# the-professor510/RSMCRT

Hardware: AMD Instinct MI355X
Metric: photon packets/sec (128^3 jmean grid, path-length deposition) (higher is better)
Workload: dtype f64

## Files before the change

include/smcrt.h:

```cpp
#ifndef SMCRT_H
#define SMCRT_H

#include <stddef.h>
#include <stdint.h>

#ifdef __cplusplus
extern "C" {
#endif

#define SMCRT_ABI_VERSION 5

typedef enum smcrt_status {
  SMCRT_OK = 0,
  SMCRT_ERR_INVALID_ARG = -1,
  SMCRT_ERR_HIP = -2,
  SMCRT_ERR_RCCL = -3,
  SMCRT_ERR_DEVICE_FAULT = -4,
  SMCRT_ERR_NO_DEVICE = -5,
  SMCRT_ERR_OOM = -6,
  SMCRT_ERR_UNSUPPORTED = -7
} smcrt_status;

typedef enum smcrt_sdf_kind {
  SMCRT_SDF_SPHERE = 1,
// ... 236 lines not shown
  const double* mua;
  const double* hgg;
  const double* n;
  const double* flux;
} smcrt_spectral;

typedef enum smcrt_spectral_mode {
  SMCRT_SPECTRAL_INIT = 0,
  SMCRT_SPECTRAL_UPDATE = 1,
  SMCRT_SPECTRAL_INIT_AS_WRITTEN = 2
} smcrt_spectral_mode;

typedef struct smcrt_optprops {
  double mus, mua, hgg, g2, n, kappa, albedo;
  double wavelength;
  int32_t node_flags;
  int32_t reserved;
} smcrt_optprops;

int smcrt_spectral_sample(const smcrt_spectral* sp, int32_t mode, uint64_t seed, uint64_t* draw,
                          smcrt_optprops* out);

int smcrt_scene_set_spectral(smcrt_scene* scene, int32_t top_index, const smcrt_spectral* sp, int32_t mode,
                             uint64_t seed, uint64_t* draw, smcrt_optprops* out);

int smcrt_run(smcrt_scene* scene, const smcrt_source* src, const smcrt_run_config* cfg,
              smcrt_tallies* io);

typedef struct smcrt_path_config {
  uint64_t range_first, range_count;
  int32_t max_vertices;
  int32_t reserved;
  int64_t max_paths;
} smcrt_path_config;

typedef struct smcrt_path {
  uint64_t photon;
  int32_t detector;
  uint32_t hit;
  uint32_t n_vertices;
  uint32_t n_stored;
  uint32_t status;
  int32_t layer;
  int64_t offset;
  double start[3], dir[3], point_sep, weight;
} smcrt_path;

int smcrt_scene_set_path_tracking(smcrt_scene* scene, const smcrt_path_config* cfg);
int smcrt_scene_path_counts(smcrt_scene* scene, int64_t* n_paths, int64_t* n_vertices, int64_t* n_dropped,
                            int64_t* n_truncated);
int smcrt_scene_read_paths(smcrt_scene* scene, smcrt_path* paths, double* vertices );

#define SMCRT_PPATH_MAX_MEDIA 16

typedef struct smcrt_ppath_config {
  uint64_t range_first, range_count;
  int64_t max_records;
  int64_t reserved;
} smcrt_ppath_config;

typedef struct smcrt_ppath {
  uint64_t photon;
  int32_t detector;
  uint32_t hit;
  uint32_t status;
  int32_t layer;
  uint32_t nscatt;
  int32_t reserved;
  double start[3], dir[3], point_sep, weight;
} smcrt_ppath;

int smcrt_scene_set_partial_paths(smcrt_scene* scene, const smcrt_ppath_config* cfg);
int smcrt_scene_partial_path_counts(smcrt_scene* scene, int64_t* n_records, int64_t* n_dropped);
int smcrt_scene_read_partial_paths(smcrt_scene* scene, smcrt_ppath* headers, double* lengths);

typedef struct smcrt_phasor_config {
  int32_t fixed_k;
  int32_t reserved;
  double wavenumber;
} smcrt_phasor_config;
#define SMCRT_PHASOR_OPTICAL_PATH 1

int smcrt_scene_set_phasor(smcrt_scene* scene, const smcrt_phasor_config* cfg);
int smcrt_scene_read_phasor(smcrt_scene* scene, double* out);
int smcrt_scene_reset_phasor(smcrt_scene* scene);

typedef struct smcrt_screen {
  double origin[3];
  double eu[3], ev[3];
  int32_t nu, nv;
  int32_t sides;
  int32_t reserved;
} smcrt_screen;

int smcrt_scene_set_screens(smcrt_scene* scene, const smcrt_screen* screens, int32_t n);
int smcrt_scene_screen_info(const smcrt_scene* scene, int32_t* n, int64_t* n_doubles);
int smcrt_scene_read_screens(smcrt_scene* scene, double* out);
int smcrt_scene_reset_screens(smcrt_scene* scene);
int smcrt_screen_hit(const smcrt_screen* screen, const double start[3], const double dir[3], double sep,
                     double* t, int32_t* pixel);


int smcrt_scene_set_volume_source(smcrt_scene* scene, const double* weights);
int smcrt_scene_volume_source_info(const smcrt_scene* scene, int64_t* n_positive, int64_t* n_reachable, double* total);
int smcrt_volume_sample(const double* weights, const smcrt_grid* g, uint64_t seed, uint64_t first, int64_t n,
                        double* pos, double* dir, int64_t* voxel);
int smcrt_volume_pick(const double* weights, int64_t nvox, const double* u, int64_t m, int64_t* voxel);

typedef struct smcrt_device_tallies {
  double* jmean;
  double* absorb;
  double* emission;
  double* det_bins;
  double* nscatt;
  double* moments;
  uint64_t* counters;
  smcrt_photon_record* records;
} smcrt_device_tallies;

int smcrt_run_device(smcrt_scene* scene, const smcrt_source* src, const smcrt_run_config* cfg,
                     smcrt_device_tallies* dev, void* stream);

int smcrt_run_origins(smcrt_scene* scene, const smcrt_source* src, const double* origins, int64_t n_origins,
                      const smcrt_run_config* cfg, double* det_totals, smcrt_tallies* io);

int smcrt_scene_classify(smcrt_scene* scene, const double* points, int64_t n, int32_t* layer, double* kappa);

int smcrt_scene_fence(smcrt_scene* scene, void* stream);

int smcrt_scene_check(smcrt_scene* scene);

typedef struct smcrt_kernel_times {
  double transport_ms;
  double deposit_ms;
  int64_t launches;
  int64_t lean_launches;
  int64_t far_steps;
  double fold_cu_ms;
  int64_t lean_hazards;
} smcrt_kernel_times;

int smcrt_scene_set_timing(smcrt_scene* scene, int32_t enable);
int smcrt_scene_kernel_times(smcrt_scene* scene, smcrt_kernel_times* out);

enum {
  SMCRT_DEPOSIT_ATOMIC = 0,
  SMCRT_DEPOSIT_SORTED = 1,
  SMCRT_DEPOSIT_BUCKETS = 2
};
int smcrt_scene_deposit_regime(const smcrt_scene* scene, int32_t* regime);

int smcrt_scene_invoxel_segments(smcrt_scene* scene, int64_t* out);

int smcrt_normalise_fluence(float* grid, const smcrt_grid* g, uint64_t nphotons);

typedef enum smcrt_symmetry {
  SMCRT_SYM_NONE = 0,
  SMCRT_SYM_PRISM = 1,
  SMCRT_SYM_FLIPPED = 2,
  SMCRT_SYM_UNIFORM_SLAB = 3,
  SMCRT_SYM_NONE_ROTATIONAL = 4,
  SMCRT_SYM_ROTATIONAL_360 = 5
} smcrt_symmetry;

typedef struct smcrt_escape_config {
  int32_t symmetry;
  int32_t n[3];
  double max[3];
  double pos[3];
  double dir[3];
  double rotation;
} smcrt_escape_config;

int smcrt_escape_sym_dims(const smcrt_escape_config* cfg, int32_t dims[3]);

int smcrt_escape_cells(const smcrt_escape_config* cfg, int64_t* n_cells, int32_t* cells, double* positions);

int smcrt_escape_map(const smcrt_escape_config* cfg, const smcrt_grid* grid, int32_t n_dets, const float* escape_sym,
                     float* escape);

int smcrt_escape_run(smcrt_scene* scene, const smcrt_source* src, const smcrt_escape_config* cfg,
                     const smcrt_run_config* run, float* escape_sym, float* escape, smcrt_tallies* io);

enum {
  SMCRT_INVERSE_FIND_MUS = 1u << 0,
  SMCRT_INVERSE_FIND_MUA = 1u << 1,
  SMCRT_INVERSE_FIND_G = 1u << 2,
  SMCRT_INVERSE_FIND_N = 1u << 3,
  SMCRT_INVERSE_APPLY_TRIAL = 1u << 4
};

typedef struct smcrt_inverse_config {
  int32_t layer;
  int32_t flags;
  int32_t max_steps;
  int32_t reserved;
  double max_step_size, grad_step_size, accuracy;
  uint64_t seed;
} smcrt_inverse_config;

int smcrt_scene_get_optprops(const smcrt_scene* scene, int32_t top_index, int32_t* layer, double* mus, double* mua,
                             double* hgg, double* n);

int smcrt_inverse_run(smcrt_scene* scene, const smcrt_source* src, const smcrt_inverse_config* cfg,
                      const smcrt_run_config* run, const double* targets, double* steps, smcrt_tallies* io);

enum {
  SMCRT_PACK_JMEAN = 1u << 0,
  SMCRT_PACK_ABSORB = 1u << 1,
  SMCRT_PACK_EMISSION = 1u << 2,
  SMCRT_PACK_DET_BINS = 1u << 3
};
typedef struct smcrt_pack_layout {
  int64_t n_voxels;
  int64_t n_det_bins;
  uint32_t fields;
  int32_t reserved;
} smcrt_pack_layout;

int smcrt_pack_size(const smcrt_pack_layout* layout, int64_t* n_doubles);
int smcrt_pack_host(const smcrt_pack_layout* layout, const smcrt_tallies* t, double* buf);
int smcrt_unpack_host(const smcrt_pack_layout* layout, const double* buf, smcrt_tallies* t);

#define SMCRT_UNIQUE_ID_BYTES 128
typedef struct smcrt_comm smcrt_comm;
int smcrt_comm_unique_id(uint8_t* id );
int smcrt_comm_init_rank(const uint8_t* id, int32_t n_ranks, int32_t rank, int32_t device, smcrt_comm** out);
void smcrt_comm_destroy(smcrt_comm* comm);
int smcrt_comm_info(const smcrt_comm* comm, int32_t* n_ranks, int32_t* rank, int32_t* device);
int smcrt_reduce_device_tallies(smcrt_scene* scene, smcrt_comm* comm, smcrt_device_tallies* dev, int32_t root,
                                void* stream);

typedef struct smcrt_multi smcrt_multi;
int smcrt_multi_create(const smcrt_sdf_node* nodes, int32_t n_nodes, const int32_t* top, int32_t n_top,
                       const smcrt_grid* grid, const smcrt_detector* dets, int32_t n_dets,
                       const int32_t* devices, int32_t n_devices, smcrt_multi** out);
int smcrt_multi_info(const smcrt_multi* multi, int32_t* n_devices);
smcrt_scene* smcrt_multi_scene(smcrt_multi* multi, int32_t i);
int smcrt_multi_run(smcrt_multi* multi, const smcrt_source* src, const smcrt_run_config* cfg, smcrt_tallies* io);
int smcrt_multi_accumulate(smcrt_multi* multi, const smcrt_source* src, const smcrt_run_config* cfg);
int smcrt_multi_collect(smcrt_multi* multi, smcrt_tallies* io);
int smcrt_multi_device_photons(const smcrt_multi* multi, uint64_t* photons);
void smcrt_multi_destroy(smcrt_multi* multi);


int smcrt_write_data_f32(const char* filename, const float* array, int32_t nx, int32_t ny, int32_t nz,
                         const char* metadata, const char* dect_id, int32_t overwrite,
                         char* written_path, int32_t path_cap);
int smcrt_write_data_f64(const char* filename, const double* array, int32_t nx, int32_t ny, int32_t nz,
                         const char* metadata, const char* dect_id, int32_t overwrite,
                         char* written_path, int32_t path_cap);

int smcrt_write_detector(const char* filename, const smcrt_detector* d, const double* data,
                         const char* id, int64_t nphotons);

int smcrt_write_paths(const char* filename, const smcrt_path* paths, int64_t n_paths, const double* vertices);

int smcrt_write_checkpoint(const char* filename, const char* toml_filename, int64_t photons_run,
                           const float* jmean, const smcrt_grid* g, int32_t overwrite,
                           char* written_path, int32_t path_cap);

typedef struct smcrt_job smcrt_job;

typedef struct smcrt_job_desc {
  int64_t n_photons;
  int64_t seed;
  int32_t flags;
  int32_t n_nodes, n_top, n_dets;
  int32_t overwrite;
  smcrt_grid grid;
  smcrt_source source;
  char experiment[64];
  char source_name[32];
} smcrt_job_desc;

int smcrt_job_load(const char* toml_path, smcrt_job** out);
enum { SMCRT_JOB_DEFAULT = 0, SMCRT_JOB_ESCAPE = 1, SMCRT_JOB_INVERSE = 2 };
int smcrt_job_load_mode(const char* toml_path, int32_t mode, smcrt_job** out);
void smcrt_job_destroy(smcrt_job* job);
int smcrt_job_info(const smcrt_job* job, smcrt_job_desc* desc);
int smcrt_job_scene(const smcrt_job* job, smcrt_sdf_node* nodes, int32_t* top, smcrt_detector* dets);
int smcrt_job_metadata(const smcrt_job* job, char* buf, int32_t cap);
int smcrt_job_history_filename(const smcrt_job* job, char* buf, int32_t cap);
#define SMCRT_ALL_DEVICES (-1)
int smcrt_job_run(smcrt_job* job, int32_t device, const char* outdir, double* nscatt);
int smcrt_job_run_devices(smcrt_job* job, const int32_t* devices, int32_t n_devices, const char* outdir,
                          double* nscatt);

int smcrt_job_escape_config(const smcrt_job* job, smcrt_escape_config* out);
int smcrt_job_inverse_config(const smcrt_job* job, smcrt_inverse_config* out);
int smcrt_job_targets(const smcrt_job* job, double* targets);
int smcrt_job_run_escape(smcrt_job* job, int32_t device, const char* outdir);
int smcrt_job_run_inverse(smcrt_job* job, int32_t device, int32_t apply_trial, double* steps);

#ifdef __cplusplus
}
#endif
#endif
```

rsmcrt_amd/abi.py:

```python
import ctypes as C

SMCRT_ABI_VERSION = 5

OK = 0
ERR_INVALID_ARG = -1
ERR_HIP = -2
ERR_RCCL = -3
ERR_DEVICE_FAULT = -4
ERR_NO_DEVICE = -5
ERR_OOM = -6
ERR_UNSUPPORTED = -7

STATUS_NAMES = {
    OK: "OK", ERR_INVALID_ARG: "INVALID_ARG", ERR_HIP: "HIP_ERROR", ERR_RCCL: "RCCL_ERROR",
    ERR_DEVICE_FAULT: "DEVICE_FAULT", ERR_NO_DEVICE: "NO_DEVICE", ERR_OOM: "OUT_OF_MEMORY",
    ERR_UNSUPPORTED: "UNSUPPORTED",
}

SDF_SPHERE, SDF_BOX, SDF_TORUS, SDF_CYLINDER, SDF_TRIPRISM = 1, 2, 3, 4, 5
SDF_SEGMENT, SDF_CAPSULE, SDF_CONE, SDF_EGG, SDF_PLANE, SDF_MODEL = 6, 7, 8, 9, 10, 11
SDF_REVOLUTION, SDF_EXTRUDE, SDF_ONION, SDF_TWIST, SDF_BEND, SDF_ELONGATE, SDF_DISPLACEMENT = 12, 13, 14, 15, 16, 17, 18
DISP_SINE, DISP_EXPR = 1, 2

OP_UNION, OP_SMOOTH_UNION, OP_SUBTRACTION, OP_INTERSECTION = 0, 1, 2, 3
# ... 99 lines not shown


class Detector(C.Structure):
    _fields_ = [
        ("kind", C.c_int32), ("nbins", C.c_int32), ("layer", C.c_int32), ("reserved", C.c_int32),
        ("pos", C.c_double * 3), ("dir", C.c_double * 3), ("e1", C.c_double * 3), ("e2", C.c_double * 3),
        ("radius", C.c_double), ("r1", C.c_double), ("r2", C.c_double),
        ("width", C.c_double), ("height", C.c_double),
        ("bin_wid", C.c_double), ("bin_wid_y", C.c_double), ("fibre", C.c_double * 11),
    ]


class RunConfig(C.Structure):
    _fields_ = [("n_photons", C.c_uint64), ("first_photon", C.c_uint64), ("seed", C.c_uint64),
                ("flags", C.c_uint32), ("reserved", C.c_int32)]


class PhotonRecord(C.Structure):
    _fields_ = [("pos", C.c_double * 3), ("dir", C.c_double * 3), ("weight", C.c_double),
                ("cell", C.c_int32 * 3), ("layer", C.c_int32), ("nscatt", C.c_uint32),
                ("bounces", C.c_uint32), ("draws", C.c_uint32), ("status", C.c_uint32)]


class Tallies(C.Structure):
    _fields_ = [
        ("jmean", C.POINTER(C.c_float)), ("absorb", C.POINTER(C.c_float)),
        ("emission", C.POINTER(C.c_float)),
        ("jmean_f64", C.POINTER(C.c_double)), ("absorb_f64", C.POINTER(C.c_double)),
        ("emission_f64", C.POINTER(C.c_double)),
        ("det_bins", C.POINTER(C.c_double)), ("nscatt", C.POINTER(C.c_double)),
        ("moments", C.POINTER(C.c_double)), ("counters", C.POINTER(C.c_uint64)),
        ("records", C.POINTER(PhotonRecord)),
    ]


class DeviceTallies(C.Structure):
    _fields_ = [
        ("jmean", C.c_void_p), ("absorb", C.c_void_p), ("emission", C.c_void_p),
        ("det_bins", C.c_void_p), ("nscatt", C.c_void_p), ("moments", C.c_void_p),
        ("counters", C.c_void_p), ("records", C.c_void_p),
    ]


class PathConfig(C.Structure):
    _fields_ = [("range_first", C.c_uint64), ("range_count", C.c_uint64), ("max_vertices", C.c_int32),
                ("reserved", C.c_int32), ("max_paths", C.c_int64)]


class Path(C.Structure):
    _fields_ = [("photon", C.c_uint64), ("detector", C.c_int32), ("hit", C.c_uint32), ("n_vertices", C.c_uint32),
                ("n_stored", C.c_uint32), ("status", C.c_uint32), ("layer", C.c_int32), ("offset", C.c_int64),
                ("start", C.c_double * 3), ("dir", C.c_double * 3), ("point_sep", C.c_double), ("weight", C.c_double)]


class PPathConfig(C.Structure):
    _fields_ = [("range_first", C.c_uint64), ("range_count", C.c_uint64), ("max_records", C.c_int64),
                ("reserved", C.c_int64)]


class PPath(C.Structure):
    _fields_ = [("photon", C.c_uint64), ("detector", C.c_int32), ("hit", C.c_uint32), ("status", C.c_uint32),
                ("layer", C.c_int32), ("nscatt", C.c_uint32), ("reserved", C.c_int32),
                ("start", C.c_double * 3), ("dir", C.c_double * 3), ("point_sep", C.c_double), ("weight", C.c_double)]


class PhasorConfig(C.Structure):
    _fields_ = [("fixed_k", C.c_int32), ("reserved", C.c_int32), ("wavenumber", C.c_double)]


class Screen(C.Structure):
    _fields_ = [("origin", C.c_double * 3), ("eu", C.c_double * 3), ("ev", C.c_double * 3),
                ("nu", C.c_int32), ("nv", C.c_int32), ("sides", C.c_int32), ("reserved", C.c_int32)]


def path_dtype():
    import numpy as np
    return np.dtype([("photon", "<u8"), ("detector", "<i4"), ("hit", "<u4"), ("n_vertices", "<u4"),
                     ("n_stored", "<u4"), ("status", "<u4"), ("layer", "<i4"), ("offset", "<i8"),
                     ("start", "<f8", 3), ("dir", "<f8", 3), ("point_sep", "<f8"), ("weight", "<f8")])


def ppath_dtype():
    import numpy as np
    return np.dtype([("photon", "<u8"), ("detector", "<i4"), ("hit", "<u4"), ("status", "<u4"), ("layer", "<i4"),
                     ("nscatt", "<u4"), ("reserved", "<i4"), ("start", "<f8", 3), ("dir", "<f8", 3),
                     ("point_sep", "<f8"), ("weight", "<f8")])


def record_dtype():
    import numpy as np
    return np.dtype([("pos", "<f8", 3), ("dir", "<f8", 3), ("weight", "<f8"), ("cell", "<i4", 3),
                     ("layer", "<i4"), ("nscatt", "<u4"), ("bounces", "<u4"), ("draws", "<u4"),
                     ("status", "<u4")])


SYM_NONE, SYM_PRISM, SYM_FLIPPED, SYM_UNIFORM_SLAB, SYM_NONE_ROTATIONAL, SYM_ROTATIONAL_360 = 0, 1, 2, 3, 4, 5
SYMMETRY_KINDS = {"none": SYM_NONE, "prism": SYM_PRISM, "flipped": SYM_FLIPPED, "uniformSlab": SYM_UNIFORM_SLAB,
                  "noneRotational": SYM_NONE_ROTATIONAL, "360rotational": SYM_ROTATIONAL_360}


class EscapeConfig(C.Structure):
    _fields_ = [("symmetry", C.c_int32), ("n", C.c_int32 * 3), ("max", C.c_double * 3), ("pos", C.c_double * 3),
                ("dir", C.c_double * 3), ("rotation", C.c_double)]


INVERSE_FIND_MUS, INVERSE_FIND_MUA, INVERSE_FIND_G, INVERSE_FIND_N, INVERSE_APPLY_TRIAL = 1, 2, 4, 8, 16


class InverseConfig(C.Structure):
    _fields_ = [("layer", C.c_int32), ("flags", C.c_int32), ("max_steps", C.c_int32), ("reserved", C.c_int32),
                ("max_step_size", C.c_double), ("grad_step_size", C.c_double), ("accuracy", C.c_double),
                ("seed", C.c_uint64)]


JOB_DEFAULT, JOB_ESCAPE, JOB_INVERSE = 0, 1, 2


class JobDesc(C.Structure):
    _fields_ = [("n_photons", C.c_int64), ("seed", C.c_int64), ("flags", C.c_int32), ("n_nodes", C.c_int32),
                ("n_top", C.c_int32), ("n_dets", C.c_int32), ("overwrite", C.c_int32), ("grid", Grid),
                ("source", Source), ("experiment", C.c_char * 64), ("source_name", C.c_char * 32)]


PACK_JMEAN, PACK_ABSORB, PACK_EMISSION, PACK_DET_BINS = 1, 2, 4, 8
UNIQUE_ID_BYTES = 128
ALL_DEVICES = -1


class PackLayout(C.Structure):
    _fields_ = [("n_voxels", C.c_int64), ("n_det_bins", C.c_int64), ("fields", C.c_uint32), ("reserved", C.c_int32)]


class KernelTimes(C.Structure):
    _fields_ = [("transport_ms", C.c_double), ("deposit_ms", C.c_double), ("launches", C.c_int64),
                ("lean_launches", C.c_int64), ("far_steps", C.c_int64), ("fold_cu_ms", C.c_double),
                ("lean_hazards", C.c_int64)]


EXPORTED_SYMBOLS = [
    "smcrt_abi_version", "smcrt_device_count", "smcrt_last_error", "smcrt_scene_create",
    "smcrt_scene_destroy", "smcrt_scene_det_bins", "smcrt_scene_set_optprops", "smcrt_run",
    "smcrt_run_device", "smcrt_normalise_fluence", "smcrt_scene_set_timing", "smcrt_scene_kernel_times",
    "smcrt_write_data_f32", "smcrt_write_data_f64", "smcrt_write_detector", "smcrt_write_checkpoint",
    "smcrt_job_load", "smcrt_job_destroy", "smcrt_job_info", "smcrt_job_scene", "smcrt_job_metadata", "smcrt_job_run",
    "smcrt_scene_info", "smcrt_run_origins", "smcrt_scene_classify", "smcrt_escape_sym_dims", "smcrt_escape_cells",
    "smcrt_escape_map", "smcrt_escape_run", "smcrt_scene_get_optprops", "smcrt_inverse_run", "smcrt_job_load_mode",
    "smcrt_job_escape_config", "smcrt_job_inverse_config", "smcrt_job_targets", "smcrt_job_run_escape",
    "smcrt_job_run_inverse", "smcrt_scene_fence",
    "smcrt_pack_size", "smcrt_pack_host", "smcrt_unpack_host", "smcrt_comm_unique_id", "smcrt_comm_init_rank",
    "smcrt_comm_info", "smcrt_comm_destroy", "smcrt_reduce_device_tallies", "smcrt_multi_create", "smcrt_multi_info",
    "smcrt_multi_scene", "smcrt_multi_run", "smcrt_multi_accumulate", "smcrt_multi_collect",
    "smcrt_multi_device_photons", "smcrt_multi_destroy", "smcrt_job_run_devices",
    "smcrt_spectral_sample", "smcrt_scene_set_spectral", "smcrt_scene_check",
    "smcrt_scene_invoxel_segments",
    "smcrt_scene_set_path_tracking", "smcrt_scene_path_counts", "smcrt_scene_read_paths", "smcrt_write_paths",
    "smcrt_job_history_filename",
    "smcrt_scene_set_phasor", "smcrt_scene_read_phasor", "smcrt_scene_reset_phasor",
    "smcrt_scene_set_screens", "smcrt_scene_screen_info", "smcrt_scene_read_screens", "smcrt_scene_reset_screens",
    "smcrt_screen_hit",
    "smcrt_scene_set_volume_source", "smcrt_scene_volume_source_info", "smcrt_volume_sample", "smcrt_volume_pick",
    "smcrt_displacement_compile", "smcrt_displacement_eval", "smcrt_displacement_describe",
    "smcrt_voxel_scene_create", "smcrt_scene_deposit_regime",
    "smcrt_mesh_scene_create",
    "smcrt_scene_set_partial_paths", "smcrt_scene_partial_path_counts", "smcrt_scene_read_partial_paths",
]
```

rsmcrt_amd/csrc/sceneplan.cpp:

```cpp
#include "sceneplan.h"

#include <algorithm>
#include <cmath>
#include <cstdlib>
#include <cstring>
#include <functional>
#include <string>

#include "dispexpr.h"
#include "hosterr.h"

namespace smcrt {
namespace {

int fail(int code, const std::string& msg) { return set_error(code, msg); }
bool is(const char* v, const char* s) { return v && std::strcmp(v, s) == 0; }

}

Knobs read_knobs() {
  Knobs k;
  auto num = [](const char* v, double d) { return v ? std::atof(v) : d; };
  if (const char* cm = std::getenv("SMCRT_COOP_MIN_TOPS")) k.coop_min_tops = std::max(1, std::atoi(cm));
  if (const char* cl = std::getenv("SMCRT_COOP_LANES")) k.coop_lanes = std::max(1, std::min(64, std::atoi(cl)));
  k.coop_tab = !is(std::getenv("SMCRT_COOP_TAB"), "0");
  k.cull = !is(std::getenv("SMCRT_CULL"), "0");
  k.cull_grid.cells_per_top = num(std::getenv("SMCRT_CULL_CPT"), 512.0);
  k.cull_grid.max_cells = num(std::getenv("SMCRT_CULL_MAX_CELLS"), 1 << 18);
  k.cull_grid.max_list = (int32_t)num(std::getenv("SMCRT_CULL_MAX_LIST"), 64);
  k.cull_grid.k_nearest = (int32_t)num(std::getenv("SMCRT_CULL_K"), 8);
  k.cull_grid.u_frac = num(std::getenv("SMCRT_CULL_UFRAC"), 1.0);
  k.cull_log = std::getenv("SMCRT_CULL_LOG") != nullptr;
  k.far_march = !is(std::getenv("SMCRT_FAR_MARCH"), "0");
  const char* dm = std::getenv("SMCRT_DEPOSIT");
  k.deposit_atomic = is(dm, "atomic");
  k.deposit_sorted = is(dm, "sorted");
  if (const char* pc = std::getenv("SMCRT_POOL_CAP"))
    k.pool_cap_chunks = std::max<uint64_t>(1, std::strtoull(pc, nullptr, 10) / CHUNK_RECORDS);
  const char* fp = std::getenv("SMCRT_FOLD_PRIO");
  k.fold_prio = !(fp && fp[0] == '0');
  k.fused_hist = !is(std::getenv("SMCRT_FUSED_HIST"), "0");
  const char* wsl = std::getenv("SMCRT_WS_SLOTS");
  k.ws_two_slots = wsl && wsl[0] == '2';
  const char* wi = std::getenv("SMCRT_WS_INVOXEL");
  k.ws_invoxel = wi ? (is(wi, "0") ? 0 : 1) : -1;
  const char* le = std::getenv("SMCRT_LEAN");
  k.lean_mode = le ? (is(le, "0") ? 0 : 1) : -1;
  const char* lm = std::getenv("SMCRT_DEBUG_LEAN_MARGIN");
  k.lean_debug = is(lm, "all") ? 2u : (is(lm, "0") ? 1u : 0u);
  k.verbose = std::getenv("SMCRT_VERBOSE") != nullptr;
  return k;
}

LaunchKnobs read_launch_knobs() {
  LaunchKnobs k;
#ifdef SMCRT_DIAG
  const char* dd = std::getenv("SMCRT_DIAG_DONE");
  k.diag_done = dd && dd[0] == '1';
#endif
  if (const char* wm = std::getenv("SMCRT_WATCHDOG_MS")) k.watchdog_ms = std::strtod(wm, nullptr);
  if (const char* cd = std::getenv("SMCRT_DEBUG_CLAIM_DELAY")) k.claim_delay = (uint32_t)std::strtoul(cd, nullptr, 10);
  const char* de = std::getenv("SMCRT_DEBUG_DROP_EVENT");
  k.drop_event = de && de[0] == '1';
  if (const char* pv = std::getenv("SMCRT_PATH_VERTICES")) k.path_vertices = (int32_t)std::strtol(pv, nullptr, 10);
  if (const char* pm = std::getenv("SMCRT_PATH_MAX")) k.path_max = (int64_t)std::strtoll(pm, nullptr, 10);
  return k;
}

void job_path_knobs(int32_t* max_vertices, int64_t* max_paths) {
  const LaunchKnobs k = read_launch_knobs();
  *max_vertices = k.path_vertices;
  *max_paths = k.path_max;
}

PoolKnobs read_pool_knobs() {
  PoolKnobs k;
  if (const char* ns = std::getenv("SMCRT_SLOTS")) k.slots = std::max(2, std::min(MAX_SLOTS, std::atoi(ns)));
  if (const char* dg = std::getenv("SMCRT_DEEP_SLOT_GIB")) {
    k.deep_set = true;
    k.deep_bytes = (uint64_t)std::strtoull(dg, nullptr, 10) << 30;
  }
  return k;
}

bool pool_log_knob() {
  static const bool on = std::getenv("SMCRT_POOL_LOG") != nullptr;
  return on;
}

TopProps make_props(const smcrt_sdf_node& nd) {
  TopProps p;
  p.kappa = nd.mus + nd.mua;
  if (nd.flags & SMCRT_NODE_ALBEDO_UNGUARDED) p.albedo = nd.mus / p.kappa;
  else p.albedo = (nd.mua < 1e-9) ? 1.0 : nd.mus / p.kappa;
  p.hgg = nd.hgg;
  p.n = nd.n;
  return p;
}

namespace {

int validate(const smcrt_sdf_node* nodes, int32_t n_nodes, const int32_t* top, int32_t n_top, const smcrt_grid* grid,
             const smcrt_detector* dets, int32_t n_dets) {
  if (!nodes || n_nodes < 1 || !top || n_top < 1 || !grid || n_dets < 0 || (n_dets > 0 && !dets))
    return fail(SMCRT_ERR_INVALID_ARG, "bad scene arguments");
  if (grid->nx < 1 || grid->ny < 1 || grid->nz < 1 || !(grid->xmax > 0) || !(grid->ymax > 0) ||
      !(grid->zmax > 0))
    return fail(SMCRT_ERR_INVALID_ARG, "grid dimensions must be positive");
  if ((uint64_t)grid->nx * (uint64_t)grid->ny * (uint64_t)grid->nz >= (1ull << 32))
    return fail(SMCRT_ERR_UNSUPPORTED, "grids of 2^32 or more voxels are not supported");
  for (int32_t i = 0; i < n_nodes; ++i) {
    const smcrt_sdf_node& nd = nodes[i];
    if (nd.kind < SMCRT_SDF_SPHERE || nd.kind > SMCRT_SDF_DISPLACEMENT)
      return fail(SMCRT_ERR_INVALID_ARG, "node " + std::to_string(i) + ": unknown SDF kind");
    if (nd.kind == SMCRT_SDF_MODEL) {
      if (nd.n_children < 1 || nd.first_child < 0 || nd.first_child + nd.n_children > n_nodes)
        return fail(SMCRT_ERR_INVALID_ARG, "model node " + std::to_string(i) + ": bad child range");
      if (nd.op < SMCRT_OP_UNION || nd.op > SMCRT_OP_INTERSECTION)
        return fail(SMCRT_ERR_INVALID_ARG, "model node " + std::to_string(i) + ": bad CSG op");
    } else if (composite_kind(nd.kind)) {
      if (nd.n_children != 1 || nd.first_child < 0 || nd.first_child >= n_nodes)
        return fail(SMCRT_ERR_INVALID_ARG, "modifier node " + std::to_string(i) + ": needs exactly one child");
      if (nd.kind == SMCRT_SDF_DISPLACEMENT && nd.param[0] == (double)SMCRT_DISP_EXPR) {
        std::string why;
        if (!disp_expr_verify(nd, &why))
          return fail(SMCRT_ERR_INVALID_ARG, "displacement node " + std::to_string(i) + ": bad expression program: " + why);
      } else if (nd.kind == SMCRT_SDF_DISPLACEMENT && nd.param[0] != (double)SMCRT_DISP_SINE) {
        return fail(SMCRT_ERR_INVALID_ARG, "displacement node " + std::to_string(i) + ": unknown function");
      }
    }
  }
  std::function<int(int32_t, int)> depth_ok = [&](int32_t idx, int lvl) -> int {
    const smcrt_sdf_node& nd = nodes[idx];
    if (!composite_kind(nd.kind)) return 1;
    if (lvl >= PROG_MAX_DEPTH) return 0;
    for (int32_t c = 0; c < nd.n_children; ++c)
      if (!depth_ok(nd.first_child + c, lvl + 1)) return 0;
    return 1;
  };
  for (int32_t i = 0; i < n_top; ++i)
    if (top[i] >= 0 && top[i] < n_nodes && !depth_ok(top[i], 0))
      return fail(SMCRT_ERR_UNSUPPORTED, "top " + std::to_string(i) + ": models/modifiers nested more than " +
                                             std::to_string(PROG_MAX_DEPTH) + " levels deep are not supported");
  for (int32_t i = 0; i < n_top; ++i)
    if (top[i] < 0 || top[i] >= n_nodes) return fail(SMCRT_ERR_INVALID_ARG, "top index out of range");
  for (int32_t i = 0; i < n_dets; ++i) {
    if (dets[i].kind < SMCRT_DET_CIRCLE || dets[i].kind > SMCRT_DET_FIBRE || dets[i].nbins < 1)
      return fail(SMCRT_ERR_INVALID_ARG, "bad detector " + std::to_string(i));
  }
  return SMCRT_OK;
}

bool translate_only(const smcrt_sdf_node& nd) {
  const double* t = nd.transform;
  return t[0] == 1.0 && t[1] == 0.0 && t[2] == 0.0 && t[4] == 0.0 && t[5] == 1.0 && t[6] == 0.0 &&
         t[8] == 0.0 && t[9] == 0.0 && t[10] == 1.0;
}

void flatten(const smcrt_sdf_node* nodes, const int32_t* top, int32_t n_top, ScenePlan& p) {
  std::vector<ProgOp>& prog = p.prog;
  p.top_first.assign((size_t)n_top + 1, 0);
  for (int32_t i = 0; i < n_top; ++i) {
    const smcrt_sdf_node& nd = nodes[top[i]];
    p.top_first[i] = (int32_t)prog.size();
    if (!composite_kind(nd.kind)) {
      prog.push_back(ProgOp{top[i], PROG_TOP, i + 1, 0, 0.0, translate_only(nd), 0});
    } else if (nd.kind != SMCRT_SDF_MODEL) {
      prog.push_back(ProgOp{top[i], PROG_TOP | PROG_SUB, i + 1, 0, 0.0, 0, 0});
    } else {
      for (int32_t c = 0; c < nd.n_children; ++c) {
        const int32_t ci = nd.first_child + c;
        const bool sub = composite_kind(nodes[ci].kind);
        prog.push_back(ProgOp{ci, (c == 0 ? PROG_CHILD_FIRST : PROG_CHILD) | (sub ? PROG_SUB : 0),
                              c == nd.n_children - 1 ? i + 1 : 0, nd.op, nd.k, sub ? 0 : translate_only(nodes[ci]), 0});
      }
    }
  }
  p.n_prog = (int)prog.size();
  p.top_first[n_top] = p.n_prog;
  for (int32_t i = 0; i <= n_top; ++i)
    prog.push_back(ProgOp{p.top_first[i], PROG_TOP, 0, 0, 0.0, 0, 0});
  for (const ProgOp& op : prog) p.nested = p.nested || (op.action & PROG_SUB) != 0;
}

void plan_far_march(const smcrt_sdf_node* nodes, const int32_t* top, int32_t n_top, const smcrt_grid* grid, bool fm,
                    ScenePlan& p) {
  double ext = grid->xmax + grid->ymax + grid->zmax + 1.0;
  double scale = 0.0;
  std::function<bool(int32_t, int, double&)> far_ok = [&](int32_t idx, int lvl, double& m) -> bool {
    const smcrt_sdf_node& nd = nodes[idx];
    if (nd.kind == SMCRT_SDF_MODEL) {
      const bool op_ok = nd.op == SMCRT_OP_UNION || nd.op == SMCRT_OP_INTERSECTION || nd.op == SMCRT_OP_SUBTRACTION ||
                         (nd.op == SMCRT_OP_SMOOTH_UNION && nd.k > 0.0 && std::isfinite(nd.k));
      if (lvl >= 4 || !op_ok || nd.n_children < 1) return false;
      if (nd.op == SMCRT_OP_SMOOTH_UNION) m = std::max(m, nd.k);
      for (int32_t c = 0; c < nd.n_children; ++c)
        if (!far_ok(nd.first_child + c, lvl + 1, m)) return false;
      return true;
    }
    const int32_t kd = nd.kind;
    if (!translate_only(nd) || !(kd == SMCRT_SDF_SPHERE || kd == SMCRT_SDF_BOX || kd == SMCRT_SDF_TORUS ||
                                 kd == SMCRT_SDF_SEGMENT || kd == SMCRT_SDF_CAPSULE))
      return false;
    double mm = std::fabs(nd.transform[3]) + std::fabs(nd.transform[7]) + std::fabs(nd.transform[11]);
    for (int r = 0; r < 8; ++r) mm += std::fabs(nd.param[r]);
    if (!std::isfinite(mm)) return false;
    m = std::max(m, mm);
    return true;
  };
  for (int32_t i = 0; fm && i < n_top; ++i) {
    double m = 0.0;
    fm = far_ok(top[i], 0, m);
    scale = std::max(scale, m);
  }
  fm = fm && std::isfinite(ext);
  if (fm) {
// ... 447 lines not shown
```

rsmcrt_amd/csrc/sceneplan.h:

```cpp
#pragma once
#include <stdint.h>

#include <algorithm>
#include <vector>

#include "../../include/smcrt.h"
#include "transport.h"
#include "cull.h"
#include "deposit.h"
#include "launchchoice.h"

namespace smcrt {

constexpr int MAX_SLOTS = 4;
#ifndef SMCRT_DEEP_SLOT_GIB
#define SMCRT_DEEP_SLOT_GIB 24
#endif
constexpr uint64_t DEEP_SLOT_BYTES = (uint64_t)SMCRT_DEEP_SLOT_GIB << 30;

enum QueueWord : int {
  Q_STREAM0 = 0,
  Q_CALLER = MAX_SLOTS,
  Q_FAR_STEPS,
  Q_FOLD_TICKS,
  Q_LEAN_HAZARDS,
  Q_WATCHDOG,
  Q_INVOXEL,
  Q_COUNT
};
constexpr int N_QUEUES = Q_CALLER + 1;

constexpr size_t LDS_BYTES = 163840;
constexpr size_t MAX_FACE_BYTES = 40960;
constexpr uint32_t MAX_FUSED_HIST_TILES = 512;
constexpr uint64_t MAX_POOL_RECORDS = (1ull << 32) - (1ull << 28);
constexpr double POOL_SLACK = 1.15;
constexpr double DEFAULT_WATCHDOG_MS = 2000.0;

struct Knobs {
  int32_t coop_min_tops = 8;
  int32_t coop_lanes = 0;
  bool coop_tab = true;
  bool cull = true;
  CullKnobs cull_grid;
  bool cull_log = false;
  bool far_march = true;
  bool deposit_atomic = false, deposit_sorted = false;
  uint64_t pool_cap_chunks = 0;
  bool fold_prio = true;
  bool fused_hist = true;
  bool ws_two_slots = false;
  int ws_invoxel = -1;
  int lean_mode = -1;
  uint32_t lean_debug = 0;
  bool verbose = false;
};
struct LaunchKnobs {
  int32_t path_vertices = 64;
  int64_t path_max = 65536;
  double watchdog_ms = DEFAULT_WATCHDOG_MS;
  uint32_t claim_delay = 0;
  bool drop_event = false;
  bool diag_done = false;
};
struct PoolKnobs {
  int slots = 0;
  bool deep_set = false;
  uint64_t deep_bytes = 0;
};
Knobs read_knobs();
LaunchKnobs read_launch_knobs();
PoolKnobs read_pool_knobs();
bool pool_log_knob();

struct PlanLimits {
  size_t ws_shared2 = 0, ws_shared3 = 0;
};

struct ScenePlan {
  int n_nodes = 0, n_top = 0, n_dets = 0;
  smcrt_grid grid{};
  int64_t det_total = 0;
  std::vector<smcrt_sdf_node> h_nodes;
  std::vector<int32_t> h_top;
  std::vector<TopProps> h_props;
  std::vector<smcrt_detector> h_dets;
  std::vector<int64_t> h_det_off;
  std::vector<double> faces;
  std::vector<ProgOp> prog;
  std::vector<int32_t> top_first;
  int n_prog = 0;
  bool nested = false;
  int coop_lanes = 0;
  std::vector<double> ctab;
  CullHost cull;
  double fm_err = 0.0, fm_step = 0.0;
  double inv2[3] = {0.0, 0.0, 0.0};
  int grid_mode = 0;
  int32_t fe[3] = {0, 0, 0};
  uint32_t n_tiles = 0;
  bool force_atomic = false;
  uint64_t pool_cap_chunks = 0;
  bool bucketed = false;
  uint32_t hist_tiles = 0;
  size_t face_bytes = 0;
  bool lds_faces = false;
  bool fresnel = false;
  int ws_slots = 3;
  int lean_mode = -1;
  uint32_t lean_debug = 0;
  int ws_invoxel = -1;
  bool lean_candidate = false;
  bool fold_prio = true, cull_log = false, verbose = false;
  bool voxel = false;
  std::vector<uint8_t> labels;
  bool mesh = false;
  int32_t mesh_ambient = 0;
  std::vector<MeshNode> mesh_nodes;
  std::vector<MeshTri> mesh_tris;
  std::vector<MeshFace> mesh_faces;
};

int plan_scene(const smcrt_sdf_node* nodes, int32_t n_nodes, const int32_t* top, int32_t n_top, const smcrt_grid* grid,
               const smcrt_detector* dets, int32_t n_dets, const Knobs& knobs, const PlanLimits& lim, ScenePlan* out);

TopProps make_props(const smcrt_sdf_node& nd);

int plan_voxel_scene(const uint8_t* labels, const smcrt_medium* media, int32_t n_media, const smcrt_grid* grid,
                     const smcrt_detector* dets, int32_t n_dets, const Knobs& knobs, ScenePlan* out);
int32_t host_vox_of(double p, int32_t n, double max);

int plan_mesh_scene(const double* verts, int32_t nv, const int32_t* tris, const uint8_t* tri_media, int32_t nt,
                    const smcrt_medium* media, int32_t n_media, int32_t ambient, const smcrt_grid* grid,
                    const smcrt_detector* dets, int32_t n_dets, const Knobs& knobs, ScenePlan* out);
int32_t mesh_medium_at(const ScenePlan& p, const double pt[3]);

int plan_screens(const smcrt_screen* screens, int32_t n, std::vector<ScreenDev>* out, int64_t* n_doubles);

int plan_volume_source(const double* w, int64_t nvox, std::vector<double>* cdf, int64_t* last, int64_t* n_positive,
                       int64_t* n_reachable);

std::vector<double> grid_faces(const smcrt_grid* grid);

inline size_t lean_lds(const ScenePlan& p) {
  return (p.lds_faces ? p.face_bytes : 0) + (size_t)2 * p.n_tiles * sizeof(uint32_t);
}
inline uint32_t dep_words(const ScenePlan& p) { return p.bucketed ? 2 * p.n_tiles : 4 * p.hist_tiles; }
inline size_t transport_lds(const ScenePlan& p, uint32_t dep_words, bool xsrc, bool hist = false, bool screens = false) {
  const bool ctab = !p.ctab.empty() && p.coop_lanes > 0;
  const bool faces = p.lds_faces && !(xsrc && p.coop_lanes > 0) && !hist;
  const size_t start_rows = screens ? 4 : p.n_dets ? 3 : 0;
  return (faces ? p.face_bytes : 0) + start_rows * 256 * sizeof(double) +
         (size_t)dep_words * sizeof(uint32_t) + (ctab ? CTAB_DOUBLES * sizeof(double) : 0);
}
inline double pool_slack_records(const ScenePlan& p, int blocks) {
  const double waves = (double)blocks * 4.0;
  return p.bucketed ? (waves / 4.0 * 2.0 * p.n_tiles + waves * BUCKET_BATCH) * BUCKET_RECORDS
                    : waves * CHUNK_RECORDS;
}
inline uint64_t pool_records_for(const ScenePlan& p, int blocks, uint64_t n, double rpp) {
  const double want = (double)n * rpp * POOL_SLACK + pool_slack_records(p, blocks);
  return (uint64_t)std::min(want, (double)MAX_POOL_RECORDS);
}
inline int slot_depth(const PoolKnobs& k, bool lean_or_far, uint64_t cap_bytes, uint64_t total_mem) {
  const int want = k.slots ? k.slots : (lean_or_far ? 2 : MAX_SLOTS);
  uint64_t deep = std::max<uint64_t>(DEEP_SLOT_BYTES, (uint64_t)(0.6 * (double)total_mem) / MAX_SLOTS);
  if (k.deep_set) deep = k.deep_bytes;
  return cap_bytes <= deep ? want : 2;
}
inline bool launch_binned(const ScenePlan& p, bool has_jmean, uint32_t flags) {
  return has_jmean && (flags & SMCRT_FLAG_PATHLENGTH) && !(flags & SMCRT_FLAG_SURVIVAL_BIAS) && p.n_tiles > 0 &&
         !p.force_atomic;
}
inline bool launch_lean(bool lean_ok, bool xsrc, uint32_t bucket_tiles, uint32_t flags) {
  return !xsrc && lean_ok && bucket_tiles && (flags & SMCRT_FLAG_PATHLENGTH) &&
         !(flags & (SMCRT_FLAG_SURVIVAL_BIAS | SMCRT_FLAG_TRACK_PATHS | SMCRT_FLAG_PHASOR));
}
inline bool ws_invoxel_on(int knob, bool xf) { return knob < 0 ? !xf : knob != 0; }
inline bool plan_xf(const ScenePlan& p) { return p.fresnel || p.n_dets > 0; }

constexpr int32_t PPL_MAX_MEDIA = SMCRT_PPATH_MAX_MEDIA;
inline size_t ppl_lds_bytes(const ScenePlan& p) { return (size_t)p.n_top * 256 * sizeof(double); }
constexpr size_t SDFLESS_STATIC_LDS = sizeof(LaneCounters);

inline LaunchChoice launch_choice(const ScenePlan& p, bool lean_ok, bool xsrc, uint32_t bucket_tiles, uint32_t flags,
                                  bool path_on, bool phasor_on, size_t n_screens, size_t ppl_lds = 0) {
  LaunchChoice c;
  c.gm = p.grid_mode;
  if (p.voxel || p.mesh) {
    c.family = p.mesh ? KF_MESH : KF_VOXEL;
    c.xsrc = xsrc;
    c.lds = p.face_bytes + (size_t)dep_words(p) * sizeof(uint32_t);
    c.ppl = (flags & SMCRT_FLAG_PARTIAL_PATHS) && ppl_lds > 0;
    if (c.ppl) c.lds += ppl_lds;
  } else if (launch_lean(lean_ok, xsrc, bucket_tiles, flags)) {
    c.family = KF_WS;
    c.lds_faces = p.lds_faces;
    c.xf = plan_xf(p);
    c.slots = p.ws_slots;
    c.iv = ws_invoxel_on(p.ws_invoxel, c.xf);
    c.tk = (flags & SMCRT_FLAG_TEST_KERNEL) != 0;
    c.lds = lean_lds(p);
  } else {
    c.xsrc = xsrc;
    c.coop = p.coop_lanes > 0;
    c.hist = (flags & SMCRT_FLAG_TRACK_PATHS) && path_on;
    c.phas = (flags & SMCRT_FLAG_PHASOR) && phasor_on && !c.hist;
    c.scr = c.phas && n_screens > 0;
    c.lds_faces = p.lds_faces && !((xsrc && c.coop) || c.hist || c.phas);
    c.lds = transport_lds(p, dep_words(p), xsrc, c.hist || c.phas, c.scr);
  }
  return c;
}
inline void lean_margins(uint32_t lean_debug, const smcrt_grid& g, double lo[3], double hi[3]) {
  const double eps = 1e-8, mf = (lean_debug & 3u) ? 0.0 : 2.0 * eps;
// ... 7 lines not shown
```

rsmcrt_amd/csrc/smcrt.hip:

```cpp
#include <hip/hip_runtime.h>

#include <algorithm>
#include <cmath>
#include <cstdio>
#include <cstring>
#include <memory>
#include <mutex>
#include <string>
#include <vector>

#define SMCRT_FOLD_KERNELS
#include "../../include/smcrt.h"
#include "scene_internal.h"
#include "transport.h"
#include "deposit.h"
#include "devmem.h"
#include "hosterr.h"
#include "hostrng.h"
#include "sceneplan.h"

using namespace smcrt;

#include "kernel_ptrs.h"

// ... 525 lines not shown
  uint64_t chunks = (records + CHUNK_RECORDS - 1) / CHUNK_RECORDS;
  if (s->pool_cap_chunks) chunks = std::min(chunks, s->pool_cap_chunks);
  if (chunks <= s->pool_chunks) return true;
  chunks = std::min<uint64_t>(chunks + chunks / 4, MAX_POOL_RECORDS / CHUNK_RECORDS);
  if (s->pool_cap_chunks) chunks = std::min(chunks, s->pool_cap_chunks);
  (void)hipDeviceSynchronize();
  (void)drain_folds(s);
  auto release = [&]() {
    s->d_sorted.reset(); s->d_pieces.reset(); s->d_order.reset();
    for (int i = 0; i < MAX_SLOTS; ++i) { s->d_pool[i].reset(); s->d_chunk_fill[i].reset(); s->d_bucket_tile[i].reset(); }
    s->pool_chunks = 0;
  };
  release();
  const uint64_t cap = chunks * CHUNK_RECORDS;
  size_t mfree = 0, mtotal = 0;
  if (hipMemGetInfo(&mfree, &mtotal) != hipSuccess) mtotal = 0;
  s->n_slots = slot_depth(read_pool_knobs(), s->lean_ok || s->fm_err > 0.0, cap * 8, mtotal);
  s->slot = 0;
  s->lturn = 0;
  s->last_slot = -1;
  const uint64_t pieces = std::min<uint64_t>(cap / MIN_PIECE_RECORDS, REDUCE_PIECES + 1) + s->n_tiles + 1;
  const uint64_t buckets = cap / BUCKET_RECORDS;
  bool ok = s->d_pieces.alloc(pieces) == hipSuccess;
  for (int i = 0; ok && i < s->n_slots; ++i) {
    ok = s->d_pool[i].alloc(cap) == hipSuccess;
    if (ok && s->bucketed)
      ok = s->d_chunk_fill[i].alloc(buckets) == hipSuccess && s->d_bucket_tile[i].alloc(buckets) == hipSuccess;
    else if (ok)
      ok = s->d_chunk_fill[i].alloc(chunks) == hipSuccess;
  }
  if (ok && s->bucketed)
    ok = s->d_order.alloc(buckets) == hipSuccess;
  else if (ok)
    ok = s->d_sorted.alloc(cap) == hipSuccess;
  if (!ok) {
    (void)hipGetLastError();
    release();
    return false;
  }
  s->pool_chunks = chunks;
  s->max_pieces = pieces;
  return true;
}


static int next_timing_events(smcrt_scene* s, Event** ev) {
  *ev = nullptr;
  if (!s->timing) return SMCRT_OK;
  if (s->tev_used == MAX_TIMED) HIPCHK(harvest_times(s));
  while (4 * (s->tev_used + 1) > s->tev.size()) {
    Event e;
    HIPCHK(hipEventCreate(e.out()));
    s->tev.push_back(std::move(e));
  }
  *ev = &s->tev[4 * s->tev_used++];
  return SMCRT_OK;
}

static int enqueue_transport(smcrt_scene* s, const KParams& K, KCold Ch, const LaunchChoice& c, hipStream_t stream,
                             int sl, int qi, Event** ev_out) {
  const bool binned = K.rec_pool != nullptr;
  if (binned && s->f_pending[sl]) HIPCHK(hipStreamWaitEvent(stream, s->ev_f[sl], 0));
  Ch.queue = s->d_queue + qi;
  Ch.lane_scratch = s->d_lscratch ? (double*)(s->d_lscratch + (size_t)qi * s->lscratch_stride) : nullptr;
  HIPCHK(hipMemsetAsync(Ch.queue, 0, sizeof(unsigned long long), stream));
  const KCold* C = s->d_cold + (size_t)qi * COLD_PER_STREAM + (s->cold_seq[qi]++ % COLD_PER_STREAM);
  HIPCHK(hipMemcpyAsync((void*)C, &Ch, sizeof(KCold), hipMemcpyHostToDevice, stream));
  if (binned) {
    HIPCHK(hipMemsetAsync(s->d_dep_ctl[sl], 0, 8 * sizeof(uint32_t), stream));
    if (K.bucket_tiles)
      HIPCHK(hipMemsetAsync(s->d_bin_counts[sl], 0, (size_t)s->n_tiles * sizeof(uint32_t), stream));
    else if (K.hist_tiles)
      HIPCHK(hipMemsetAsync(s->d_bin_counts[sl], 0, (size_t)s->n_tiles * BIN_BLOCKS * sizeof(uint32_t), stream));
  }
  if (const int st = next_timing_events(s, ev_out)) return st;
  Event* ev = *ev_out;
  if (ev) HIPCHK(hipEventRecord(ev[0], stream));
  const bool ws = c.family == KF_WS;
  const uint64_t per_block = ws ? (uint64_t)kinst_ws_photon_lanes() : 256;
  const int blocks = (int)std::min<uint64_t>((uint64_t)blocks_for(s, c),
                                             std::max<uint64_t>(1, (Ch.n_photons + per_block - 1) / per_block));
  if (ws) ++s->lean_launches;
  const smcrt_sdf_node* a_nodes = K.nodes;
  const ProgOp* a_prog = K.prog;
  const smcrt_detector* a_dets = K.dets;
  const int64_t* a_off = K.det_off;
  void* args_ws[] = {(void*)&K, (void*)&a_nodes, (void*)&a_prog, (void*)&C};
  void* args[] = {(void*)&K, (void*)&a_nodes, (void*)&a_prog, (void*)&a_dets, (void*)&a_off, (void*)&C};
  HIPCHK(hipLaunchKernel(kernel_ptr(c), dim3(blocks), dim3(kernel_threads(c)), ws ? args_ws : args, c.lds, stream));
  HIPCHK(hipGetLastError());
  if (ev) HIPCHK(hipEventRecord(ev[1], stream));
  return SMCRT_OK;
}

static int enqueue_fold(smcrt_scene* s, const KParams& K, double* jmean, hipStream_t stream, int sl, Event* ev) {
  if (!K.rec_pool) {
    if (ev) {
      HIPCHK(hipEventRecord(ev[2], stream));
      HIPCHK(hipEventRecord(ev[3], stream));
    }
    return SMCRT_OK;
  }
  hipStream_t fs = s->fstream;
  HIPCHK(hipEventRecord(s->ev_t, stream));
  HIPCHK(hipStreamWaitEvent(fs, s->ev_t, 0));
  if (ev) HIPCHK(hipEventRecord(ev[2], fs));
  const uint32_t nch = (uint32_t)s->pool_chunks;
  const uint64_t nv = (uint64_t)s->grid.nx * s->grid.ny * s->grid.nz;
  if (K.bucket_tiles) {
    hipLaunchKernelGGL(bk_scan, dim3(1), dim3(1024), 0, fs, s->d_bin_counts[sl], s->n_tiles, s->d_tile_start,
                       s->d_tile_count, s->d_pieces, s->d_dep_ctl[sl]);
    hipLaunchKernelGGL(bk_place, dim3(BIN_BLOCKS), dim3(BIN_THREADS), 0, fs, s->d_bucket_tile[sl], s->d_chunk_fill[sl],
                       s->d_dep_ctl[sl], K.n_buckets, s->n_tiles, s->d_tile_count, s->d_order);
#ifndef SMCRT_ABL_NO_FOLD
    hipLaunchKernelGGL(bk_reduce, dim3(1024), dim3(RED_THREADS), 0, fs, s->d_pool[sl], s->d_order, s->d_pieces,
                       s->d_dep_ctl[sl], nv, jmean, s->d_queue + Q_FOLD_TICKS);
#endif
  } else {
    if (!K.hist_tiles)
      hipLaunchKernelGGL(bin_hist, dim3(BIN_BLOCKS), dim3(BIN_THREADS), 0, fs, s->d_pool[sl], s->d_chunk_fill[sl],
                         s->d_dep_ctl[sl], nch, s->n_tiles, s->d_bin_counts[sl]);
    hipLaunchKernelGGL(bin_rowscan, dim3(s->n_tiles), dim3(BIN_BLOCKS), 0, fs, s->d_bin_counts[sl],
                       s->d_tile_count);
    hipLaunchKernelGGL(bin_scan, dim3(1), dim3(1024), 0, fs, s->d_tile_count, s->n_tiles, s->d_tile_start,
                       s->d_pieces, s->d_dep_ctl[sl]);
    hipLaunchKernelGGL(bin_scatter, dim3(BIN_BLOCKS), dim3(BIN_THREADS), s->scatter_lds, fs, s->d_pool[sl],
                       s->d_chunk_fill[sl], s->d_dep_ctl[sl], nch, s->n_tiles, s->d_tile_start, s->d_bin_counts[sl],
                       s->d_sorted, (uint64_t)s->pool_chunks * CHUNK_RECORDS);
    hipLaunchKernelGGL(bin_reduce, dim3(1024), dim3(1024), 0, fs, s->d_sorted, s->d_pieces, s->d_dep_ctl[sl], nv,
                       jmean);
  }
  HIPCHK(hipGetLastError());
  HIPCHK(hipMemcpyAsync(s->h_ctl + 8 * sl, s->d_dep_ctl[sl], 4 * sizeof(uint32_t), hipMemcpyDeviceToHost, fs));
  HIPCHK(hipMemcpyAsync(s->h_ctl + 8 * sl + 5, s->d_dep_ctl[sl] + 5, 2 * sizeof(uint32_t), hipMemcpyDeviceToHost, fs));
  HIPCHK(hipEventRecord(s->ctl_ev[sl], fs));
  s->ctl_pending[sl] = true;
  if (ev) HIPCHK(hipEventRecord(ev[3], fs));
  HIPCHK(hipEventRecord(s->ev_f[sl], fs));
  s->f_pending[sl] = true;
  s->last_slot = sl;
  return SMCRT_OK;
}

#ifdef SMCRT_DIAG
static int diag_report(hipStream_t stream, bool lean) {
  unsigned long long h[72], ht[9], hc[6];
  HIPCHK(hipStreamSynchronize(stream));
  kinst_diag_gather(h, ht, hc);
  if (lean) {
    const double wi = (double)std::max(1ull, h[20]), pt = (double)std::max(1ull, h[24]);
    std::fprintf(stderr, "[diag-ws] walker iters %llu: idle %.3f, busy lanes/iter %.1f, pending lanes/iter %.1f | "
                 "photon trips %llu: sleep %.3f, idle lanes %.1f, sync-waiting %.2f, slot-blocked %.2f, EVAL lanes "
                 "%.1f, pushes %.2f, P7 runs %.3f (lanes/run %.1f), event-waiting %.2f | producer waits %llu | event "
                 "iters %llu, lanes/iter %.1f | emissions waiting for a slot %llu lane-trips\n",
                 h[20], h[21] / wi, h[22] / wi, h[23] / wi, h[24], h[25] / pt, h[30] / pt, h[27] / pt, h[26] / pt,
                 h[31] / pt, h[32] / pt, h[28] / pt, (double)h[29] / (double)std::max(1ull, h[28]), h[36] / pt, h[33],
                 h[34], (double)h[35] / (double)std::max(1ull, h[34]), h[51]);
    const char* np[8] = {"fetch", "poll", "eval", "p3p4", "handout", "p5p6", "p7", "p8"};
    double tp = 0, tw = 0, te = 0;
    for (int i = 0; i < 8; ++i) tp += (double)h[37 + i];
    for (int i = 0; i < 4; ++i) tw += (double)h[45 + i];
    te = (double)h[49] + (double)h[50];
    std::fprintf(stderr, "[diag-ws-time] photon:");
    for (int i = 0; i < 8; ++i) std::fprintf(stderr, " %s=%.3f", np[i], (double)h[37 + i] / std::max(1.0, tp));
    std::fprintf(stderr, " | walker: claim=%.3f idle=%.3f walk=%.3f finish=%.3f | event: run=%.3f idle=%.3f | "
                 "ticks photon/walker/event %.3g/%.3g/%.3g\n", h[45] / std::max(1.0, tw), h[46] / std::max(1.0, tw),
                 h[47] / std::max(1.0, tw), h[48] / std::max(1.0, tw), h[49] / std::max(1.0, te),
                 h[50] / std::max(1.0, te), tp, tw, te);
  }
  unsigned long long lt = 0;
  for (int i = 0; i < 64; ++i) lt += h[i];
  std::fprintf(stderr, "[diag] waves %llu, longest wave %llu trips %llu ticks\n", h[70], h[68], h[69]);
  std::fprintf(stderr, "[diag] trips %llu dda %llu eval %llu p7 %llu | lane-trips %llu:", h[64], h[65], h[66],
               h[67], lt);
  for (int i = 0; i < 64; ++i)
    if (h[i]) std::fprintf(stderr, " %s%d=%.3f", i >= 32 ? "seg:" : "", i & 31, (double)h[i] / (double)lt);
  std::fprintf(stderr, "\n");

  double tt = 0;
  for (int i = 1; i < 9; ++i) tt += (double)ht[i];
  const char* nm_t[9] = {"", "fetch", "eval", "p3", "p4", "dda", "p5p6", "p7", "p8"};
  const char* nm_l[9] = {"", "fetch", "eval", "p3p4", "push", "walk", "p5p6", "p7", "p8"};
  const char* const* nm = lean ? nm_l : nm_t;
  std::fprintf(stderr, "[diag-time]");
  for (int i = 1; i < 9; ++i) std::fprintf(stderr, " %s=%.3f", nm[i], (double)ht[i] / tt);
  std::fprintf(stderr, "\n");

  if (hc[0] + hc[2])
    std::fprintf(stderr, "[diag-cull] culled lane-EVALs %llu, bound fallbacks %llu (%.4f), capture/outside %llu, "
                 "mean list %.1f, wave-EVALs %llu with a full fallback %.3f\n", hc[0], hc[1],
                 (double)hc[1] / (double)std::max(1ull, hc[0]), hc[2], (double)hc[3] / (double)std::max(1ull, hc[0]),
                 hc[4], (double)hc[5] / (double)std::max(1ull, hc[4]));
  return SMCRT_OK;
}
#endif

static int launch_one(smcrt_scene* s, const KParams& K, const KCold& Ch, bool xsrc, hipStream_t stream, int sl, int qi) {
  const LaunchChoice c = launch_choice(*s, s->lean_ok, xsrc, K.bucket_tiles, K.flags, s->path_on, s->phasor_on, s->screens.size(),
                                       ppl_lds_of(s));
  Event* ev = nullptr;
  int st = enqueue_transport(s, K, Ch, c, stream, sl, qi, &ev);
  if (!st) st = enqueue_fold(s, K, Ch.jmean, stream, sl, ev);
#ifdef SMCRT_DIAG
  if (!st) st = diag_report(stream, c.family == KF_WS);
#endif
  return st;
}

struct OriginRun {
  const double* d_origins;
  double* d_totals;
  uint64_t per_origin, first;
};

static int fill_params(smcrt_scene* s, const smcrt_source* src, const smcrt_run_config* cfg,
                       const smcrt_device_tallies& dt, const SrcPlan& plan, hipStream_t stream, bool diag_done_ok,
                       const LaunchChoice& run, KParams& K, KCold& Ch) {
  const LaunchKnobs knobs = read_launch_knobs();
  K.nodes = s->d_nodes;
  K.prog = s->d_prog;
  K.n_prog = s->n_prog;
  K.coop_lanes = s->coop_lanes;
  K.cull = s->d_cull;
  K.ctab = s->d_ctab;
  const bool far = s->fm_err > 0.0 && (cfg->flags & SMCRT_FLAG_PATHLENGTH);
  K.fm_err = far ? s->fm_err : 0.0;
  K.fm_step = s->fm_step;
  K.inv2x = s->inv2[0]; K.inv2y = s->inv2[1]; K.inv2z = s->inv2[2];
  K.fex = s->fe[0]; K.fey = s->fe[1]; K.fez = s->fe[2];
  K.props = s->d_props;
  K.xface = s->d_faces;
  K.yface = s->d_faces + (s->grid.nx + 1);
  K.zface = s->d_faces + (s->grid.nx + 1) + (s->grid.ny + 1);
  K.dets = s->d_dets;
  K.det_off = s->d_det_off;
  K.n_top = s->n_top;
  K.n_dets = s->n_dets;
  K.nx = s->grid.nx; K.ny = s->grid.ny; K.nz = s->grid.nz;
  K.xmax = s->grid.xmax; K.ymax = s->grid.ymax; K.zmax = s->grid.zmax;
  K.flags = cfg->flags;
  Ch.src = *src;
  Ch.plan = plan;
  K.key0 = (uint32_t)cfg->seed;
  K.key1 = (uint32_t)(cfg->seed >> 32);
  Ch.jmean = dt.jmean; Ch.absorb = dt.absorb; Ch.emission = dt.emission;
  Ch.chunk_fill = nullptr; Ch.dep_ctl = nullptr; Ch.bin_counts = nullptr;
  Ch.bucket_tile = nullptr; Ch.bucket_fill = nullptr; Ch.tile_nb = nullptr;
  Ch.det_bins = dt.det_bins; Ch.nscatt = dt.nscatt; Ch.moments = dt.moments;
  Ch.counters = (unsigned long long*)dt.counters;
  Ch.queue = nullptr;
  Ch.far_steps = s->d_queue + Q_FAR_STEPS;
  Ch.lean_hazards = s->d_queue + Q_LEAN_HAZARDS;
  Ch.invoxel_segs = s->d_queue + Q_INVOXEL;
  Ch.lane_scratch = nullptr;
  Ch.watchdog = watchdog_word(s);
  const bool hist = run.hist, phas = run.phas, scr = run.scr;
  Ch.hist_scratch = hist ? (double*)s->d_hist_scratch : nullptr;
  Ch.path_vertices = hist ? (double*)s->d_path_vertices : nullptr;
  Ch.path_headers = hist ? (smcrt_path*)s->d_path_headers : nullptr;
  Ch.path_ctl = hist ? (unsigned long long*)s->d_path_ctl : nullptr;
  Ch.hist_lanes = hist ? s->hist_lanes : 0;
  Ch.path_max = hist ? (uint64_t)s->path_cfg.max_paths : 0;
  const bool ppl = run.ppl;
  Ch.range_first = hist ? s->path_cfg.range_first : ppl ? s->ppath_cfg.range_first : 0;
  Ch.range_count = hist ? s->path_cfg.range_count : ppl ? s->ppath_cfg.range_count : 0;
  Ch.ppl_lengths = ppl ? (double*)s->d_ppl_lengths : nullptr;
  Ch.ppl_headers = ppl ? (smcrt_ppath*)s->d_ppl_headers : nullptr;
  Ch.ppl_ctl = ppl ? (unsigned long long*)s->d_ppl_ctl : nullptr;
  Ch.ppl_max = ppl ? (uint64_t)s->ppath_cfg.max_records : 0;
  Ch.ppl_lds_off = ppl ? (uint32_t)((s->face_bytes + (size_t)dep_words(*s) * sizeof(uint32_t)) / sizeof(double)) : 0u;
  Ch.ppl_n_media = ppl ? (uint32_t)s->n_top : 0u;
  Ch.hist_max_vertices = hist ? (uint32_t)s->path_cfg.max_vertices : 0;
  Ch.phasor = phas ? (double*)s->d_phasor : nullptr;
  Ch.phasor_fixed = phas && s->phasor_cfg.fixed_k ? 1u : 0u;
  Ch.phasor_k = !phas ? 0.0
                : s->phasor_cfg.fixed_k ? s->phasor_cfg.wavenumber
                                        : 6.283185307179586 / (src->spectrum ? src->spectrum->wavelength : 500.0);
  Ch.screens = scr ? (const ScreenDev*)s->d_screens : nullptr;
  Ch.screen_field = scr ? (double*)s->d_screen_field : nullptr;
  Ch.n_screens = scr ? (uint32_t)s->screens.size() : 0u;
  Ch.phasor_optical = phas && (s->phasor_cfg.reserved & SMCRT_PHASOR_OPTICAL_PATH) ? 1u : 0u;
  const bool vsrc = src->kind == SMCRT_SRC_VOLUME && s->d_vs_cdf;
  Ch.vs_cdf = vsrc ? (const double*)s->d_vs_cdf : nullptr;
  Ch.vs_xface = vsrc ? K.xface : nullptr;
  Ch.vs_yface = vsrc ? K.yface : nullptr;
  Ch.vs_zface = vsrc ? K.zface : nullptr;
  Ch.vs_total = vsrc ? s->vs_total : 0.0;
  Ch.vs_nvox = vsrc ? (uint32_t)((int64_t)s->grid.nx * s->grid.ny * s->grid.nz) : 0u;
  Ch.vs_last = vsrc ? (uint32_t)s->vs_last : 0u;
  Ch.vox_labels = s->d_labels;
  Ch.vox_n_media = s->voxel ? (uint32_t)s->n_top : 0u;
  Ch.vox_reserved = 0;
  Ch.mesh_nodes = s->d_mesh_nodes;
  Ch.mesh_tris = s->d_mesh_tris;
  Ch.mesh_faces = s->d_mesh_faces;
  Ch.mesh_n_nodes = (uint32_t)s->mesh_nodes.size();
  Ch.mesh_ambient = (uint32_t)s->mesh_ambient;
#ifdef SMCRT_DIAG
  Ch.done_time = nullptr;
  Ch.done_base = cfg->first_photon;
  if (knobs.diag_done && diag_done_ok) {
    s->n_done = cfg->n_photons;
    HIPCHK(s->d_done.alloc(s->n_done));
    HIPCHK(hipMemsetAsync(s->d_done, 0, sizeof(unsigned long long) * s->n_done, stream));
    Ch.done_time = s->d_done;
  }
#else
  (void)stream; (void)diag_done_ok;
#endif
  Ch.watchdog_ticks = knobs.watchdog_ms > 0.0 ? (uint64_t)(knobs.watchdog_ms * (double)s->wall_khz) : 0ull;
  K.rec_pool = nullptr; K.n_chunks = 0; K.hist_tiles = 0; K.bucket_tiles = 0; K.n_buckets = 0;
  K.claim_delay = knobs.claim_delay;
  K.lean_debug = s->lean_debug | (knobs.drop_event ? 4u : 0u);
  K.ws_invoxel = ws_invoxel_on(s->ws_invoxel, plan_xf(*s)) ? 1u : 0u;
  lean_margins(K.lean_debug, s->grid, K.lean_lo, K.lean_hi);
  return SMCRT_OK;
}

static int launch(smcrt_scene* s, const smcrt_source* src, const smcrt_run_config* cfg,
                  const smcrt_device_tallies& dt, hipStream_t stream, const OriginRun* orun = nullptr) {
  if (src->kind < SMCRT_SRC_POINT || src->kind > SMCRT_SRC_VOLUME) return fail(SMCRT_ERR_INVALID_ARG, "bad source kind");
  if (src->kind == SMCRT_SRC_VOLUME) {
    if (orun) return fail(SMCRT_ERR_UNSUPPORTED, "smcrt_run_origins: a volume source has no origin to batch");
    if (!s->d_vs_cdf)
      return fail(SMCRT_ERR_INVALID_ARG, "a volume source needs smcrt_scene_set_volume_source first (the scene holds no table)");
  }
  if (const int pst = ppl_flag_scene_ok(s, cfg->flags)) return pst;
  if (cfg->n_photons == 0) return SMCRT_OK;
  const bool xsrc = src_needs_plan(src) || orun || s->nested;
  SrcPlan plan;
  std::memset(&plan, 0, sizeof plan);
  if (xsrc) {
    std::vector<double> px, py, pc;
    const char* perr = "";
    const int pst = build_src_plan(src, &s->grid, &plan, px, py, pc, &perr);
    if (pst) return fail(pst, perr);
    std::vector<double> tab;
    tab.reserve(px.size() + py.size() + pc.size());
    tab.insert(tab.end(), px.begin(), px.end());
    tab.insert(tab.end(), py.begin(), py.end());
    tab.insert(tab.end(), pc.begin(), pc.end());
    if (!tab.empty()) {
      if (tab != s->h_spec) {
        HIPCHK(hipStreamSynchronize(stream));
        if (s->stream != stream) HIPCHK(hipStreamSynchronize(s->stream));
        if (tab.size() > s->spec_cap) {
          s->spec_cap = 0;
          HIPCHK(s->d_spec.alloc(tab.size()));
          s->spec_cap = tab.size();
        }
        HIPCHK(hipMemcpy(s->d_spec, tab.data(), tab.size() * sizeof(double), hipMemcpyHostToDevice));
        s->h_spec = tab;
      }
      plan.spec_x = px.empty() ? nullptr : s->d_spec;
      plan.spec_y = py.empty() ? nullptr : s->d_spec + px.size();
      plan.cdf = s->d_spec + px.size() + py.size();
    }
    if (orun) {
      plan.origins = orun->d_origins;
      plan.det_totals = orun->d_totals;
      plan.per_origin = orun->per_origin;
      plan.first = orun->first;
    }
  }
  KParams K;
  KCold Ch;
  const LaunchChoice run = launch_choice(*s, false, xsrc, 0, cfg->flags, s->path_on, s->phasor_on, s->screens.size(),
                                         ppl_lds_of(s));
  if (const int st = fill_params(s, src, cfg, dt, plan, stream, !orun, run, K, Ch)) return st;
  const bool binned = launch_binned(*s, dt.jmean != nullptr, cfg->flags);
  const bool overlap = (cfg->flags & SMCRT_FLAG_OVERLAP) != 0;
  if (overlap) {
    HIPCHK(hipEventRecord(s->ev_in, stream));
    for (int i = 0; i < MAX_SLOTS; ++i) HIPCHK(hipStreamWaitEvent(s->lstream[i], s->ev_in, 0));
  } else {
    for (int i = 0; i < MAX_SLOTS; ++i)
      if (s->lpending[i]) HIPCHK(hipStreamWaitEvent(stream, s->lev[i], 0));
  }
  for (int i = 0; i < MAX_SLOTS; ++i)
    if (s->lpending[i] && hipEventQuery(s->lev[i]) == hipSuccess) s->lpending[i] = false;
  for (uint64_t done = 0; done < cfg->n_photons;) {
    refine_rpp(s);
    uint64_t n = cfg->n_photons - done;
    K.rec_pool = nullptr; K.n_chunks = 0; K.hist_tiles = 0; K.bucket_tiles = 0; K.n_buckets = 0;
    bool calibrate = false;
    if (binned) {
      if (!s->rpp_measured && n > CALIB_PHOTONS) { n = CALIB_PHOTONS; calibrate = true; }
      const uint64_t want = pool_records_for(*s, transport_blocks(s), n, s->rpp_est);
      if (!ensure_pool(s, want)) (void)ensure_pool(s, want / 4);
      if (s->pool_chunks) {
        const double usable = (double)(s->pool_chunks * CHUNK_RECORDS) - pool_slack_records(*s, transport_blocks(s));
        n = std::min<uint64_t>(n, (uint64_t)std::max(65536.0, usable / (s->rpp_est * POOL_SLACK)));
        K.rec_pool = s->d_pool[s->slot];
        Ch.chunk_fill = s->d_chunk_fill[s->slot];
        Ch.dep_ctl = s->d_dep_ctl[s->slot];
        Ch.bin_counts = s->d_bin_counts[s->slot];
        K.n_chunks = (uint32_t)s->pool_chunks;
        K.hist_tiles = s->hist_tiles;
        if (s->bucketed) {
          Ch.bucket_fill = s->d_chunk_fill[s->slot];
          Ch.bucket_tile = s->d_bucket_tile[s->slot];
          Ch.tile_nb = s->d_bin_counts[s->slot];
          K.bucket_tiles = s->n_tiles;
          K.n_buckets = (uint32_t)(s->pool_chunks * (CHUNK_RECORDS / BUCKET_RECORDS));
        }
      }
    }
    Ch.n_photons = n;
    Ch.first_photon = orun ? done : cfg->first_photon + done;
    Ch.records = dt.records ? dt.records + done : nullptr;
    const int sl = s->slot;
    if (K.rec_pool) {
      if (s->ctl_pending[sl]) { HIPCHK(hipEventSynchronize(s->ctl_ev[sl])); refine_rpp(s); }
      s->h_ctl[8 * sl + 4] = (uint32_t)std::min<uint64_t>(n, 0xFFFFFFFFull);
    }
    int st;
    if (overlap) {
      const int q = s->lturn;
      s->lturn = (s->lturn + 1) % s->n_slots;
      st = launch_one(s, K, Ch, xsrc, s->lstream[q], sl, q);
      if (!st && hipEventRecord(s->lev[q], s->lstream[q]) != hipSuccess) st = fail(SMCRT_ERR_HIP, "event record failed");
      s->lpending[q] = true;
    } else {
      st = launch_one(s, K, Ch, xsrc, stream, sl, Q_CALLER);
    }
    if (st) return st;
    if (K.rec_pool) s->slot = (s->slot + 1) % s->n_slots;
    if (calibrate && K.rec_pool) {
      HIPCHK(hipEventSynchronize(s->ctl_ev[sl]));
      refine_rpp(s);
    }
    done += n;
  }
  if (!(cfg->flags & (SMCRT_FLAG_ASYNC_FOLD | SMCRT_FLAG_OVERLAP)) && s->last_slot >= 0 && s->f_pending[s->last_slot])
    HIPCHK(hipStreamWaitEvent(stream, s->ev_f[s->last_slot], 0));
  return SMCRT_OK;
}

int smcrt_run_device(smcrt_scene* s, const smcrt_source* src, const smcrt_run_config* cfg,
                     smcrt_device_tallies* dev, void* stream) {
  g_last_error.clear();
  if (!s || !src || !cfg || !dev) return fail(SMCRT_ERR_INVALID_ARG, "NULL argument");
  if (const int vst = sdfless_flags_ok(s, cfg->flags)) return vst;
  if (const int pst = ppl_flag_scene_ok(s, cfg->flags)) return pst;
  if (cfg->flags & SMCRT_FLAG_TRACK_PATHS)
    return fail(SMCRT_ERR_INVALID_ARG, "SMCRT_FLAG_TRACK_PATHS: paths are recorded by smcrt_run only");
  if (cfg->flags & SMCRT_FLAG_PHASOR)
    return fail(SMCRT_ERR_INVALID_ARG, "SMCRT_FLAG_PHASOR: the phasor grid is tallied by smcrt_run only");
  if (cfg->flags & SMCRT_FLAG_PARTIAL_PATHS)
    return fail(SMCRT_ERR_INVALID_ARG, "SMCRT_FLAG_PARTIAL_PATHS: partial path lengths are recorded by smcrt_run only");
  std::lock_guard<std::mutex> g(s->mu);
  HIPCHK(hipSetDevice(s->device));
  return launch(s, src, cfg, *dev, (hipStream_t)stream);
}

}

static int run_sync(smcrt_scene* s, const smcrt_source* src, const smcrt_run_config* cfg_in, smcrt_tallies* io,
                    const OriginRun* orun) {
  smcrt_run_config cfg_local = *cfg_in;
  cfg_local.flags &= ~(uint32_t)(SMCRT_FLAG_ASYNC_FOLD | SMCRT_FLAG_OVERLAP);
  const smcrt_run_config* cfg = &cfg_local;
  const int64_t nv = (int64_t)s->grid.nx * s->grid.ny * s->grid.nz;
  const bool want[3] = {io->jmean || io->jmean_f64, io->absorb || io->absorb_f64, io->emission || io->emission_f64};
  if (!s->d_grids && (want[0] || want[1] || want[2])) {
    int st = dalloc(s->d_grids, (size_t)nv * 3);
// ... 125 lines not shown
  unsigned long long hc[6];
  kinst_diag_gather(out, out + 72, hc);
  return SMCRT_OK;
}
int smcrt_diag_done_times(smcrt_scene* s, unsigned long long* out, uint64_t n, int32_t* khz) {
  if (!s || !out || !s->d_done || n > s->n_done) return fail(SMCRT_ERR_INVALID_ARG, "no completion times");
  HIPCHK(hipDeviceSynchronize());
  HIPCHK(hipMemcpy(out, s->d_done, sizeof(unsigned long long) * n, hipMemcpyDeviceToHost));
  if (khz) *khz = s->wall_khz;
  return SMCRT_OK;
}
#endif

int smcrt_scene_info(const smcrt_scene* s, smcrt_grid* grid, int32_t* n_top, int32_t* n_dets) {
  if (!s) return fail(SMCRT_ERR_INVALID_ARG, "scene is NULL");
  if (grid) *grid = s->grid;
  if (n_top) *n_top = s->n_top;
  if (n_dets) *n_dets = s->n_dets;
  return SMCRT_OK;
}

int smcrt_scene_classify(smcrt_scene* s, const double* points, int64_t n, int32_t* layer, double* kappa) {
  g_last_error.clear();
  if (!s || (n > 0 && (!points || !layer))) return fail(SMCRT_ERR_INVALID_ARG, "NULL argument");
  if (n <= 0) return SMCRT_OK;
  std::lock_guard<std::mutex> g(s->mu);
  if (s->voxel) {
    for (int64_t i = 0; i < n; ++i) {
      const int32_t ci = host_vox_of(points[3 * i], s->grid.nx, s->grid.xmax),
                    cj = host_vox_of(points[3 * i + 1], s->grid.ny, s->grid.ymax),
                    ck = host_vox_of(points[3 * i + 2], s->grid.nz, s->grid.zmax);
      layer[i] = (ci < 1 || cj < 1 || ck < 1)
                     ? 0
                     : 1 + (int32_t)s->labels[(size_t)(ci - 1) + (size_t)s->grid.nx * ((size_t)(cj - 1) + (size_t)s->grid.ny * (size_t)(ck - 1))];
      if (kappa) kappa[i] = layer[i] > 0 ? s->h_props[layer[i] - 1].kappa : 0.0;
    }
    return SMCRT_OK;
  }
  if (s->mesh) {
    for (int64_t i = 0; i < n; ++i) {
      const bool in = host_vox_of(points[3 * i], s->grid.nx, s->grid.xmax) >= 1 &&
                      host_vox_of(points[3 * i + 1], s->grid.ny, s->grid.ymax) >= 1 &&
                      host_vox_of(points[3 * i + 2], s->grid.nz, s->grid.zmax) >= 1;
      layer[i] = in ? 1 + mesh_medium_at(*s, points + 3 * i) : 0;
      if (kappa) kappa[i] = layer[i] > 0 ? s->h_props[layer[i] - 1].kappa : 0.0;
    }
    return SMCRT_OK;
  }
  HIPCHK(hipSetDevice(s->device));
  DevBuf<double> d_pts;
  DevBuf<int32_t> d_lay;
  int st = dalloc(d_pts, (size_t)n * 3);
  if (!st) st = dalloc(d_lay, (size_t)n);
  if (!st) {
    hipError_t e = hipMemcpy(d_pts, points, sizeof(double) * 3 * (size_t)n, hipMemcpyHostToDevice);
    if (e == hipSuccess) {
      const int blocks = (int)std::min<int64_t>((n + 255) / 256, 65535);
      hipLaunchKernelGGL(classify_kernel, dim3(blocks), dim3(256), 0, s->stream, (const smcrt_sdf_node*)s->d_nodes,
                         (const ProgOp*)s->d_prog, (int32_t)s->n_prog, (const double*)d_pts, n, d_lay);
      e = hipGetLastError();
    }
    if (e == hipSuccess) e = hipStreamSynchronize(s->stream);
    if (e == hipSuccess) e = hipMemcpy(layer, d_lay, sizeof(int32_t) * (size_t)n, hipMemcpyDeviceToHost);
    if (e != hipSuccess) st = fail(SMCRT_ERR_HIP, std::string("classify: ") + hipGetErrorString(e));
  }
  if (!st && kappa)
    for (int64_t i = 0; i < n; ++i) kappa[i] = layer[i] > 0 ? s->h_props[layer[i] - 1].kappa : 0.0;
  return st;
}

int smcrt_scene_fence(smcrt_scene* s, void* stream) {
  g_last_error.clear();
  if (!s) return fail(SMCRT_ERR_INVALID_ARG, "scene is NULL");
  std::lock_guard<std::mutex> g(s->mu);
  HIPCHK(hipSetDevice(s->device));
  for (int i = 0; i < MAX_SLOTS; ++i)
    if (s->lpending[i]) HIPCHK(hipStreamWaitEvent((hipStream_t)stream, s->lev[i], 0));
  if (s->last_slot >= 0 && s->f_pending[s->last_slot])
    HIPCHK(hipStreamWaitEvent((hipStream_t)stream, s->ev_f[s->last_slot], 0));
  return SMCRT_OK;
}

int smcrt_scene_check(smcrt_scene* s) {
  g_last_error.clear();
  if (!s) return fail(SMCRT_ERR_INVALID_ARG, "scene is NULL");
  std::lock_guard<std::mutex> g(s->mu);
  HIPCHK(hipSetDevice(s->device));
  for (int i = 0; i < MAX_SLOTS; ++i)
    if (s->lstream[i]) {
      const hipError_t e = hipStreamSynchronize(s->lstream[i]);
      if (e != hipSuccess) return fail(SMCRT_ERR_DEVICE_FAULT, std::string("transport kernel: ") + hipGetErrorString(e));
    }
  for (hipStream_t st : {(hipStream_t)s->stream, (hipStream_t)s->fstream})
    if (st) {
      const hipError_t e = hipStreamSynchronize(st);
      if (e != hipSuccess) return fail(SMCRT_ERR_DEVICE_FAULT, std::string("transport kernel: ") + hipGetErrorString(e));
    }
  return take_watchdog(s);
}

int smcrt_scene_set_timing(smcrt_scene* s, int32_t enable) {
  if (!s) return fail(SMCRT_ERR_INVALID_ARG, "scene is NULL");
  std::lock_guard<std::mutex> g(s->mu);
  s->timing = enable != 0;
  return SMCRT_OK;
}

int smcrt_scene_kernel_times(smcrt_scene* s, smcrt_kernel_times* out) {
  if (!s || !out) return fail(SMCRT_ERR_INVALID_ARG, "NULL argument");
  std::lock_guard<std::mutex> g(s->mu);
  HIPCHK(hipSetDevice(s->device));
  HIPCHK(harvest_times(s));
  out->transport_ms = s->t_transport;
  out->deposit_ms = s->t_deposit;
  out->launches = s->t_launches;
  out->lean_launches = s->lean_launches;
  s->lean_launches = 0;
  unsigned long long far = 0;
  HIPCHK(hipMemcpy(&far, s->d_queue + Q_FAR_STEPS, sizeof(far), hipMemcpyDeviceToHost));
  out->far_steps = (int64_t)(far - s->far_reported);
  s->far_reported = far;
  unsigned long long ticks = 0;
  HIPCHK(hipMemcpy(&ticks, s->d_queue + Q_FOLD_TICKS, sizeof(ticks), hipMemcpyDeviceToHost));
  out->fold_cu_ms = (double)(ticks - s->fold_ticks_reported) / (double)s->wall_khz / (double)s->n_cus;
  s->fold_ticks_reported = ticks;
  unsigned long long hz = 0;
  HIPCHK(hipMemcpy(&hz, s->d_queue + Q_LEAN_HAZARDS, sizeof(hz), hipMemcpyDeviceToHost));
  out->lean_hazards = (int64_t)(hz - s->hazards_reported);
  s->hazards_reported = hz;
  s->t_transport = s->t_deposit = 0.0;
  s->t_launches = 0;
  return SMCRT_OK;
}

int smcrt_scene_deposit_regime(const smcrt_scene* s, int32_t* regime) {
  if (!s || !regime) return fail(SMCRT_ERR_INVALID_ARG, "NULL argument");
  *regime = !launch_binned(*s, true, SMCRT_FLAG_PATHLENGTH) ? SMCRT_DEPOSIT_ATOMIC
            : s->bucketed                                   ? SMCRT_DEPOSIT_BUCKETS
                                                            : SMCRT_DEPOSIT_SORTED;
  return SMCRT_OK;
}

int smcrt_scene_invoxel_segments(smcrt_scene* s, int64_t* out) {
  if (!s || !out) return fail(SMCRT_ERR_INVALID_ARG, "NULL argument");
  if (const int vst = smcrt::scene_needs_sdf(s, "smcrt_scene_invoxel_segments")) return vst;
  std::lock_guard<std::mutex> g(s->mu);
  HIPCHK(hipSetDevice(s->device));
  unsigned long long n = 0;
  HIPCHK(hipMemcpy(&n, s->d_queue + Q_INVOXEL, sizeof(n), hipMemcpyDeviceToHost));
  *out = (int64_t)n;
  return SMCRT_OK;
}

static void release_paths(smcrt_scene* s) {
  s->path_on = false;
  s->d_hist_scratch.reset(); s->d_path_vertices.reset(); s->d_path_headers.reset(); s->d_path_ctl.reset();
  s->hist_lanes = 0;
}

int smcrt_scene_set_path_tracking(smcrt_scene* s, const smcrt_path_config* cfg) {
  g_last_error.clear();
  if (!s) return fail(SMCRT_ERR_INVALID_ARG, "scene is NULL");
  if (const int vst = smcrt::scene_needs_sdf(s, "path tracking")) return vst;
  if (cfg) {
    if (cfg->max_vertices < 2 || cfg->max_vertices > 1024)
      return fail(SMCRT_ERR_INVALID_ARG, "path tracking: max_vertices must lie in 2 .. 1024");
    if (cfg->max_paths < 1) return fail(SMCRT_ERR_INVALID_ARG, "path tracking: max_paths must be >= 1");
    if (cfg->range_count > UINT64_MAX - cfg->range_first)
      return fail(SMCRT_ERR_INVALID_ARG, "path tracking: the photon range overflows");
  }
  std::lock_guard<std::mutex> g(s->mu);
  HIPCHK(hipSetDevice(s->device));
  HIPCHK(hipStreamSynchronize(s->stream));
  release_paths(s);
  if (!cfg) return SMCRT_OK;
  int hist_blocks = 0;
  for (int x = 0; x < 2; ++x)
    hist_blocks = std::max(hist_blocks, blocks_for(s, launch_choice(*s, false, x == 1, 0, SMCRT_FLAG_TRACK_PATHS, true, false, 0)));
  const uint64_t lanes = (uint64_t)hist_blocks * 256ull;
  const uint64_t mv = (uint64_t)cfg->max_vertices, mp = (uint64_t)cfg->max_paths;
  if (mp > (1ull << 40) / mv) return fail(SMCRT_ERR_OOM, "path tracking: the arena does not fit");
  int st;
  if ((st = dalloc(s->d_hist_scratch, (size_t)(lanes * mv * 4))) || (st = dalloc(s->d_path_vertices, (size_t)(mp * mv * 4))) ||
      (st = dalloc(s->d_path_headers, (size_t)mp)) || (st = dalloc(s->d_path_ctl, 3))) {
    (void)hipGetLastError();
    release_paths(s);
    return st;
  }
  HIPCHK(hipMemset(s->d_path_ctl, 0, 3 * sizeof(unsigned long long)));
  s->path_cfg = *cfg;
  s->hist_lanes = lanes;
  s->path_on = true;
  return SMCRT_OK;
}

static int fetch_paths(smcrt_scene* s, unsigned long long ctl[3], std::vector<smcrt_path>& hdr) {
  if (!s->path_on) return fail(SMCRT_ERR_INVALID_ARG, "path tracking is not configured on this scene");
  HIPCHK(hipSetDevice(s->device));
  HIPCHK(hipStreamSynchronize(s->stream));
  HIPCHK(hipMemcpy(ctl, s->d_path_ctl, 3 * sizeof(unsigned long long), hipMemcpyDeviceToHost));
  const uint64_t n = std::min<uint64_t>(ctl[0], (uint64_t)s->path_cfg.max_paths);
  hdr.resize((size_t)n);
  if (n) HIPCHK(hipMemcpy(hdr.data(), s->d_path_headers, (size_t)n * sizeof(smcrt_path), hipMemcpyDeviceToHost));
  for (smcrt_path& p : hdr)
    p.n_stored = std::min<uint32_t>(p.n_stored, (uint32_t)s->path_cfg.max_vertices);
  return SMCRT_OK;
}

int smcrt_scene_path_counts(smcrt_scene* s, int64_t* n_paths, int64_t* n_vertices, int64_t* n_dropped,
                            int64_t* n_truncated) {
  g_last_error.clear();
  if (!s) return fail(SMCRT_ERR_INVALID_ARG, "scene is NULL");
  if (const int vst = smcrt::scene_needs_sdf(s, "path tracking")) return vst;
  std::lock_guard<std::mutex> g(s->mu);
  unsigned long long ctl[3];
  std::vector<smcrt_path> hdr;
  if (const int st = fetch_paths(s, ctl, hdr)) return st;
  int64_t nv = 0;
  for (const smcrt_path& p : hdr) nv += p.n_stored;
  if (n_paths) *n_paths = (int64_t)hdr.size();
  if (n_vertices) *n_vertices = nv;
  if (n_dropped) *n_dropped = (int64_t)ctl[1];
  if (n_truncated) *n_truncated = (int64_t)ctl[2];
  return SMCRT_OK;
}

int smcrt_scene_read_paths(smcrt_scene* s, smcrt_path* paths, double* vertices) {
  g_last_error.clear();
  if (!s) return fail(SMCRT_ERR_INVALID_ARG, "scene is NULL");
  if (const int vst = smcrt::scene_needs_sdf(s, "path tracking")) return vst;
  std::lock_guard<std::mutex> g(s->mu);
  unsigned long long ctl[3];
  std::vector<smcrt_path> hdr;
  if (const int st = fetch_paths(s, ctl, hdr)) return st;
  if (hdr.empty()) return SMCRT_OK;
  if (!paths || !vertices) return fail(SMCRT_ERR_INVALID_ARG, "NULL argument");
  std::vector<size_t> order(hdr.size());
  for (size_t i = 0; i < order.size(); ++i) order[i] = i;
  std::sort(order.begin(), order.end(), [&](size_t a, size_t b) {
    if (hdr[a].photon != hdr[b].photon) return hdr[a].photon < hdr[b].photon;
    if (hdr[a].hit != hdr[b].hit) return hdr[a].hit < hdr[b].hit;
    return a < b;
  });
  const size_t mv = (size_t)s->path_cfg.max_vertices;
  std::vector<double> arena(hdr.size() * mv * 4);
  HIPCHK(hipMemcpy(arena.data(), s->d_path_vertices, arena.size() * sizeof(double), hipMemcpyDeviceToHost));
  int64_t off = 0;
  for (size_t k = 0; k < order.size(); ++k) {
    const size_t slot = order[k];
    paths[k] = hdr[slot];
    paths[k].offset = off;
    std::memcpy(vertices + 4 * off, arena.data() + slot * mv * 4, (size_t)hdr[slot].n_stored * 4 * sizeof(double));
    off += hdr[slot].n_stored;
  }
  return SMCRT_OK;
}

static void release_ppaths(smcrt_scene* s) {
  s->ppath_on = false;
  s->d_ppl_lengths.reset(); s->d_ppl_headers.reset(); s->d_ppl_ctl.reset();
}

static int ppaths_scene_ok(const smcrt_scene* s) {
  if (s->voxel || s->mesh) return SMCRT_OK;
  return fail(SMCRT_ERR_UNSUPPORTED, "partial path lengths are not supported on SDF scenes (smcrt_scene_create): "
                                     "they are kept by voxel and mesh scenes only");
}

int smcrt_scene_set_partial_paths(smcrt_scene* s, const smcrt_ppath_config* cfg) {
  g_last_error.clear();
  if (!s) return fail(SMCRT_ERR_INVALID_ARG, "scene is NULL");
  if (const int vst = ppaths_scene_ok(s)) return vst;
  uint64_t mr = 0;
  const uint64_t nm = (uint64_t)s->n_top;
  if (cfg) {
    if (cfg->max_records < 1) return fail(SMCRT_ERR_INVALID_ARG, "partial path lengths: max_records must be >= 1");
    if (cfg->reserved != 0) return fail(SMCRT_ERR_INVALID_ARG, "partial path lengths: reserved must be 0");
    if (cfg->range_count > UINT64_MAX - cfg->range_first)
      return fail(SMCRT_ERR_INVALID_ARG, "partial path lengths: the photon range overflows");
    if (s->n_top > PPL_MAX_MEDIA)
      return fail(SMCRT_ERR_UNSUPPORTED, "partial path lengths: the scene has " + std::to_string(s->n_top) +
                                             " media, more than the cap of " + std::to_string(PPL_MAX_MEDIA) +
                                             " (SMCRT_PPATH_MAX_MEDIA: the lengths live in the kernels' LDS)");
    const size_t lds = launch_choice(*s, false, false, 0, SMCRT_FLAG_PATHLENGTH | SMCRT_FLAG_PARTIAL_PATHS, false, false, 0,
                                     ppl_lds_bytes(*s)).lds + SDFLESS_STATIC_LDS;
    if (lds > LDS_BYTES)
      return fail(SMCRT_ERR_UNSUPPORTED, "partial path lengths: a block would need " + std::to_string(lds) +
                                             " bytes of LDS, more than " + std::to_string(LDS_BYTES));
    mr = (uint64_t)cfg->max_records;
    if (mr > (1ull << 40) / (nm * sizeof(double) + sizeof(smcrt_ppath)))
      return fail(SMCRT_ERR_OOM, "partial path lengths: the arena does not fit");
  }
  std::lock_guard<std::mutex> g(s->mu);
  HIPCHK(hipSetDevice(s->device));
  HIPCHK(hipStreamSynchronize(s->stream));
  release_ppaths(s);
  if (!cfg) return SMCRT_OK;
  int st;
  if ((st = dalloc(s->d_ppl_lengths, (size_t)(mr * nm))) || (st = dalloc(s->d_ppl_headers, (size_t)mr)) ||
      (st = dalloc(s->d_ppl_ctl, 2))) {
    (void)hipGetLastError();
    release_ppaths(s);
    return st;
  }
  HIPCHK(hipMemset(s->d_ppl_ctl, 0, 2 * sizeof(unsigned long long)));
  s->ppath_cfg = *cfg;
// ... 282 lines not shown
```

rsmcrt_amd/csrc/transport.h:

```cpp
#pragma once
#include <hip/hip_runtime.h>
#include <stdint.h>

#include <type_traits>

#include "../../include/smcrt.h"
#include "detmath.h"
#include "geometry.h"
#include "srcplan.h"
#include "cull.h"
#include "meshcast.h"
#include "screen.h"
#include "volsrc.h"

namespace smcrt {

constexpr int64_t MAX_EMIT_TRIES = 100000;
constexpr int64_t MAX_HOP_ITERS = 1000000;
constexpr int64_t MAX_MARCH_ITERS = 10000000;
constexpr int64_t MAX_GLANCE_ITERS = 100000;
constexpr int64_t MAX_DDA_ITERS = 10000000;
constexpr int MAX_RENORM_ITERS = 64;
constexpr int64_t MAX_INTERACTIONS = 100000000;

#define SMCRT_DDA_PER_ITER 3
#define SMCRT_FETCH_CHUNK 64
#define SMCRT_EVENT_LANES 16

struct TopProps {
  double kappa, albedo, hgg, n;
};

struct KCold {
  smcrt_source src;
  uint64_t n_photons, first_photon;
  double* absorb;
  double* emission;
  double* det_bins;
  double* nscatt;
  double* moments;
  unsigned long long* counters;
  smcrt_photon_record* records;
  unsigned long long* queue;
  double* jmean;
  uint32_t* chunk_fill;
  uint32_t* dep_ctl;
  uint32_t* bin_counts;
  uint32_t* bucket_tile;
  uint32_t* bucket_fill;
  uint32_t* tile_nb;
  unsigned long long* far_steps;
  unsigned long long* lean_hazards;
  unsigned long long* invoxel_segs;
  double* lane_scratch;
  uint32_t* watchdog;
  uint64_t watchdog_ticks;
#ifdef SMCRT_DIAG
  unsigned long long* done_time;
  uint64_t done_base;
#endif
  SrcPlan plan;
  double* hist_scratch;
  double* path_vertices;
  smcrt_path* path_headers;
  unsigned long long* path_ctl;
  uint64_t hist_lanes;
  uint64_t path_max;
  uint64_t range_first, range_count;
  uint32_t hist_max_vertices;
  uint32_t phasor_fixed;
  double* phasor;
  double phasor_k;
  const uint8_t* vox_labels;
  uint32_t vox_n_media;
  uint32_t vox_reserved;
  const MeshNode* mesh_nodes;
  const MeshTri* mesh_tris;
  const MeshFace* mesh_faces;
  uint32_t mesh_n_nodes;
  uint32_t mesh_ambient;
  const ScreenDev* screens;
  double* screen_field;
  uint32_t n_screens;
  uint32_t phasor_optical;
  const double* vs_cdf;
  const double* vs_xface;
  const double* vs_yface;
  const double* vs_zface;
  double vs_total;
  uint32_t vs_nvox;
  uint32_t vs_last;
  double* ppl_lengths;
  smcrt_ppath* ppl_headers;
  unsigned long long* ppl_ctl;
  uint64_t ppl_max;
  uint32_t ppl_lds_off;
  uint32_t ppl_n_media;
};

enum : uint32_t {
  WDOG_PHOTON_WAVE = 1,
  WDOG_RING = 2,
  WDOG_EVENT_QUEUE = 3,
  WDOG_BUCKET = 4
};
__device__ __forceinline__ bool watchdog_expired(const KCold* __restrict__ C, uint64_t t0, uint32_t site) {
  const uint64_t budget = C->watchdog_ticks;
  if (budget == 0 || __builtin_amdgcn_s_memrealtime() - t0 <= budget) return false;
  atomicCAS(C->watchdog, 0u, site | ((blockIdx.x + 1u) << 8));
  return true;
}

struct KParams {
  const smcrt_sdf_node* __restrict__ nodes;
  const ProgOp* __restrict__ prog;
  const TopProps* __restrict__ props;
  const double* __restrict__ xface;
  const double* __restrict__ yface;
  const double* __restrict__ zface;
  const smcrt_detector* __restrict__ dets;
  const int64_t* __restrict__ det_off;
  int32_t n_prog, n_top, n_dets;
  int32_t coop_lanes;
  int32_t nx, ny, nz;
  uint32_t flags;
  double xmax, ymax, zmax;
  double inv2x, inv2y, inv2z;
  int32_t fex, fey, fez;
  uint32_t key0, key1;
  unsigned long long* rec_pool;
  uint32_t n_chunks;
  uint32_t hist_tiles;
  uint32_t bucket_tiles, n_buckets;
  uint32_t claim_delay;
  uint32_t lean_debug;
  uint32_t ws_invoxel;
  double lean_lo[3], lean_hi[3];
  const CullGrid* __restrict__ cull;
  const double* __restrict__ ctab;
  double fm_err, fm_step;
};

template <int GM>
__device__ __forceinline__ double cell_floor(double p, int32_t n, double max, double inv, int32_t fe) {
  if constexpr (GM == 2) return floor(ldexp(p, -fe));
  const double a = (double)n * p;
  return floor(GM >= 1 ? a * inv : (inv != 0.0 ? a * inv : a / (2.0 * max)));
}
__device__ __forceinline__ int32_t cvt_sat_i32(double f) {
  int32_t r;
  asm("v_cvt_i32_f64 %0, %1" : "=v"(r) : "v"(f));
  return r;
}
template <int GM>
__device__ __forceinline__ int32_t cell_of(double p, int32_t n, double max, double inv, int32_t fe) {
  const double f = cell_floor<GM>(p, n, max, inv, fe);
  if (!(f >= 0.0 && f < (double)n)) return -1;
  return (int32_t)f + 1;
}
template <int GM>
__device__ __forceinline__ int32_t vox_of(double p, int32_t n, double max, double inv, int32_t fe) {
  return cell_of<GM>(p + max, n, max, inv, fe);
}

template <int GM>
__device__ __forceinline__ double face(const double* __restrict__ f, int32_t k, int32_t ex) {
  if constexpr (GM == 2) return ldexp((double)k, ex);
  else return f[k];
}

__device__ __forceinline__ void atomic_add_nr(double* p, double v) {
  __hip_atomic_fetch_add(p, v, __ATOMIC_RELAXED, __HIP_MEMORY_SCOPE_AGENT);
}

__device__ __forceinline__ bool intersect_circle(V3 n, V3 p0, double radius, V3 l0, V3 l, double& t, double& d2) {
  t = 0.0;
  const double denom = dot(n, l);
  if (denom > 1e-6) {
    const V3 p0l0 = p0 - l0;
    double tt = dot(p0l0, n);
    tt = tt / denom;
    t = tt;
    if (tt > -1e-6) {
      const V3 p = l0 + mul(l, tt);
      const V3 v = p - p0;
      d2 = sqrt(dot(v, v));
      if (d2 <= radius) return true;
    }
  }
  return false;
}

__device__ __forceinline__ int64_t f_nint(double x) {
  if (!(fabs(x) < 4.0e18)) return x > 0 ? (int64_t)4e18 : -(int64_t)4e18;
  return (int64_t)round(x);
}
__device__ __forceinline__ int64_t f_int(double x) {
  if (!(fabs(x) < 4.0e18)) return x > 0 ? (int64_t)4e18 : -(int64_t)4e18;
  return (int64_t)x;
}

struct NoHitHook {
  __device__ __forceinline__ void operator()(int32_t, const smcrt_detector*) const {}
};
template <class OnHit = NoHitHook>
__device__ __forceinline__ uint32_t record_hits(const KParams& K, double* det_bins,
// ... 543 lines not shown
    uxx = sint * cosp; uyy = sint * sinp; uzz = -cost;
  } else {
    temp = sqrt(1.0 - nzp * nzp);
    uxx = sint * ((nxp * nzp * cosp - nyp * sinp) / temp) + nxp * cost;
    uyy = sint * ((nyp * nzp * cosp + nxp * sinp) / temp) + nyp * cost;
    uzz = -1.0 * sint * cosp * temp + nzp * cost;
  }
  temp = sqrt(uxx * uxx + uyy * uyy + uzz * uzz);
  int it = 0;
  while (fabs(temp - 1.0) > 1e-12) {
    if (++it > MAX_RENORM_ITERS) { L.fault = true; L.tflag = true; break; }
    uxx = uxx / temp; uyy = uyy / temp; uzz = uzz / temp;
    temp = sqrt(uxx * uxx + uyy * uyy + uzz * uzz);
  }
  L.dir = v3(uxx, uyy, uzz);
}

template <int GM>
__device__ __forceinline__ bool start_segment(const KParams& K, Lane& L, LaneCounters* sh, V3 p, double dlen) {
  LCTR(LC_UPD)++;
  V3 old = v3(p.x + K.xmax, p.y + K.ymax, p.z + K.zmax);
  int32_t ci = cell_of<GM>(old.x, K.nx, K.xmax, K.inv2x, K.fex), cj = cell_of<GM>(old.y, K.ny, K.ymax, K.inv2y, K.fey),
          ck = cell_of<GM>(old.z, K.nz, K.zmax, K.inv2z, K.fez);
  L.xcell = ci; L.ycell = cj; L.zcell = ck;
  if (!(K.flags & SMCRT_FLAG_PATHLENGTH)) {
    old.x = old.x + L.dir.x * dlen;
    old.y = old.y + L.dir.y * dlen;
    old.z = old.z + L.dir.z * dlen;
    ci = cell_of<GM>(old.x, K.nx, K.xmax, K.inv2x, K.fex); cj = cell_of<GM>(old.y, K.ny, K.ymax, K.inv2y, K.fey);
    ck = cell_of<GM>(old.z, K.nz, K.zmax, K.inv2z, K.fez);
    if (ci == -1 || cj == -1 || ck == -1) L.tflag = true;
    L.xcell = ci; L.ycell = cj; L.zcell = ck;
    return false;
  }
  if (ci == -1 || cj == -1 || ck == -1) { L.tflag = true; return false; }
  L.old = old; L.sd = 0.0; L.slen = dlen; L.dda_it = 0;
  L.seg = true;
  return true;
}

template <int GM, class S, class PC = NoDdaPiece>
__device__ __forceinline__ void dda_step_r(const KParams& K, S& L, const V3 dir, const V3 rcp,
                                           const double* __restrict__ xf, const double* __restrict__ yf,
                                           const double* __restrict__ zf, bool& dep, uint32_t& dep_vox,
                                           double& dep_val, double weight, PC* piece = nullptr);
template <int GM, class S, class PC = NoDdaPiece>
__device__ __forceinline__ void dda_step(const KParams& K, S& L, const V3 dir, const double* __restrict__ xf,
                                         const double* __restrict__ yf, const double* __restrict__ zf,
                                         bool& dep, uint32_t& dep_vox, double& dep_val, double weight,
                                         PC* piece = nullptr) {
  const V3 rcp = v3(ieee_rcp_f64(dir.x), ieee_rcp_f64(dir.y), ieee_rcp_f64(dir.z));
  dda_step_r<GM>(K, L, dir, rcp, xf, yf, zf, dep, dep_vox, dep_val, weight, piece);
}
template <int GM, class S, class PC>
__device__ __forceinline__ void dda_step_r(const KParams& K, S& L, const V3 dir, const V3 rcp3,
                                           const double* __restrict__ xf, const double* __restrict__ yf,
                                           const double* __restrict__ zf, bool& dep, uint32_t& dep_vox,
                                           double& dep_val, double weight, PC* piece) {
#ifdef SMCRT_ASM_MARKERS
  asm volatile("; @@DDA_BEGIN");
#endif
  const bool capped = ++L.dda_it > (uint32_t)MAX_DDA_ITERS;
  const double fx = face<GM>(xf, dir.x > 0.0 ? L.xcell : L.xcell - 1, K.fex);
  const double fy = face<GM>(yf, dir.y > 0.0 ? L.ycell : L.ycell - 1, K.fey);
  const double fz = face<GM>(zf, dir.z > 0.0 ? L.zcell : L.zcell - 1, K.fez);
  const double nx = fx - L.old.x;
  const double ny = fy - L.old.y;
  const double nz = fz - L.old.z;
  const double rx = rcp3.x, ry = rcp3.y, rz = rcp3.z;
  const double ax = nx * rx;
  const double ay = ny * ry;
  const double az = nz * rz;
  const double amin = fmin(fmin(ax, ay), az);
  const double thr = amin * (1.0 + 0x1.0p-16);
  const bool ux = ax > thr, uy = ay > thr, uz = az > thr;
  const bool two = ((ux ^ uy) ^ uz) == false && (ux || uy || uz);
  const bool fast0 = two && amin > 0.0 && fabs(dir.x) >= 0x1.0p-500 && fabs(dir.y) >= 0x1.0p-500 &&
                     fabs(dir.z) >= 0x1.0p-500;
  bool lx = !ux, ly = !uy, lz = !uz;
  const double num = lx ? nx : (ly ? ny : nz), den = lx ? dir.x : (ly ? dir.y : dir.z);
  const double rcp = lx ? rx : (ly ? ry : rz);
  const bool fast = fast0 && fabs(num) >= 0x1.0p-500;
  double dcell;
  if (fast) {
    dcell = ieee_div_tail_f64(num, den, rcp);
  } else {
    double dx = -999.0, dy = -999.0, dz = -999.0;
    if (dir.x > 0.0 || dir.x < 0.0) dx = nx / dir.x;
    else if (dir.x == 0.0) dx = 100000.0;
    if (dir.y > 0.0 || dir.y < 0.0) dy = ny / dir.y;
    else if (dir.y == 0.0) dy = 100000.0;
    if (dir.z > 0.0 || dir.z < 0.0) dz = nz / dir.z;
    else if (dir.z == 0.0) dz = 100000.0;
    dcell = dmin(dmin(dx, dy), dz);
    lx = (dcell == dx); ly = (dcell == dy); lz = (dcell == dz);
  }
  const bool neg = dcell < 0.0;
  const bool ok = !capped && !neg;
  const double sdn = L.sd + dcell;
  const bool last = sdn > L.slen;
  const double dc = last ? L.slen - L.sd : dcell;
  dep = ok;
  dep_vox = lin(K, L.xcell, L.ycell, L.zcell);
  dep_val = (double)(float)dc * weight;
  if constexpr (!std::is_empty_v<PC>) {
    piece->dc = dc;
    piece->wall = ok && !last;
  }
  const double delta = 1e-8;
  const double vx = L.old.x + dir.x * dc, vy = L.old.y + dir.y * dc, vz = L.old.z + dir.z * dc;
  const double sx = dir.x > 0.0 || dir.x < 0.0 ? fx + (dir.x > 0.0 ? delta : -delta) : L.old.x;
  const double sy = dir.y > 0.0 || dir.y < 0.0 ? fy + (dir.y > 0.0 ? delta : -delta) : L.old.y;
  const double sz = dir.z > 0.0 || dir.z < 0.0 ? fz + (dir.z > 0.0 ? delta : -delta) : L.old.z;
  const bool noaxis = !(lx || ly || lz);
  const bool snap = ok && !last && !noaxis;
  const bool snx = lx, sny = !lx && ly, snz = !lx && !ly;
  if constexpr (std::is_same_v<PC, DdaPieceAxis>) piece->axis = snap ? (snx ? 0 : (sny ? 1 : 2)) : -1;
  const double px = snx && (dir.x > 0.0 || dir.x < 0.0) ? sx : vx;
  const double py = sny && (dir.y > 0.0 || dir.y < 0.0) ? sy : vy;
  const double pz = snz && (dir.z > 0.0 || dir.z < 0.0) ? sz : vz;
  const int32_t gx = cvt_sat_i32(cell_floor<GM>(px, K.nx, K.xmax, K.inv2x, K.fex));
  const int32_t gy = cvt_sat_i32(cell_floor<GM>(py, K.ny, K.ymax, K.inv2y, K.fey));
  const int32_t gz = cvt_sat_i32(cell_floor<GM>(pz, K.nz, K.zmax, K.inv2z, K.fez));
  const bool inx = (uint32_t)gx < (uint32_t)K.nx, iny = (uint32_t)gy < (uint32_t)K.ny,
             inz = (uint32_t)gz < (uint32_t)K.nz;
  const bool left = snap && !(inx && iny && inz);
  L.old = v3(px, py, pz);
  L.sd = sdn;
  L.xcell = snap ? (inx ? gx + 1 : -1) : L.xcell;
  L.ycell = snap ? (iny ? gy + 1 : -1) : L.ycell;
  L.zcell = snap ? (inz ? gz + 1 : -1) : L.zcell;
  const bool bad = capped || neg || (ok && !last && noaxis);
  if (bad || left) {
    L.fault = L.fault || bad;
    L.tflag = true;
  }
  L.seg = !(bad || (ok && last) || left);
#ifdef SMCRT_ASM_MARKERS
  asm volatile("; @@DDA_END");
#endif
}

#ifndef SMCRT_EVAL_PAIRS
#define SMCRT_EVAL_PAIRS 1
#endif
struct EvalOut {
  double minabs, minv, va, vb;
  int32_t maxloc;
};

template <bool NEST = false, bool PAIRS = false>
__device__ __forceinline__ EvalOut eval_sdfs(const smcrt_sdf_node* __restrict__ nodes,
                                             const ProgOp* __restrict__ prog, int32_t n_prog, V3 q,
                                             bool mask_le, int32_t capi, int32_t capj) {
  EvalOut r;
  r.minabs = __builtin_inf();
  r.minv = __builtin_inf();
  r.va = 0.0; r.vb = 0.0;
  r.maxloc = 0;
  double best = -__builtin_inf();
  double acc = 0.0;
  for (int32_t ip = 0; ip < n_prog; ++ip) {
    const ProgOp op = prog[ip];
#if SMCRT_EVAL_PAIRS
    if (PAIRS && !NEST && ip + 1 < n_prog && op.action == PROG_TOP && op.top > 0) {
      const ProgOp op2 = prog[ip + 1];
      if (op2.action == PROG_TOP && op2.top > 0) {
        const smcrt_sdf_node* n1 = nodes + __builtin_amdgcn_readfirstlane(op.node);
        const smcrt_sdf_node* n2 = nodes + __builtin_amdgcn_readfirstlane(op2.node);
        const int32_t k1 = n1->kind, k2 = n2->kind;
        const bool t1 = op.translate_only != 0, t2 = op2.translate_only != 0;
        double v1 = 0.0, v2 = 0.0;
        bool pair = true;
        if (k1 == SMCRT_SDF_SPHERE && k2 == SMCRT_SDF_BOX) {
          v1 = sdf_prim_s<1>(SMCRT_SDF_SPHERE, n1->transform, n1->param, q, t1);
          v2 = sdf_prim_s<1>(SMCRT_SDF_BOX, n2->transform, n2->param, q, t2);
        } else if (k1 == SMCRT_SDF_BOX && k2 == SMCRT_SDF_BOX) {
          v1 = sdf_prim_s<1>(SMCRT_SDF_BOX, n1->transform, n1->param, q, t1);
          v2 = sdf_prim_s<1>(SMCRT_SDF_BOX, n2->transform, n2->param, q, t2);
        } else if (k1 == SMCRT_SDF_BOX && k2 == SMCRT_SDF_SPHERE) {
          v1 = sdf_prim_s<1>(SMCRT_SDF_BOX, n1->transform, n1->param, q, t1);
          v2 = sdf_prim_s<1>(SMCRT_SDF_SPHERE, n2->transform, n2->param, q, t2);
        } else if (k1 == SMCRT_SDF_SPHERE && k2 == SMCRT_SDF_SPHERE) {
          v1 = sdf_prim_s<1>(SMCRT_SDF_SPHERE, n1->transform, n1->param, q, t1);
          v2 = sdf_prim_s<1>(SMCRT_SDF_SPHERE, n2->transform, n2->param, q, t2);
        } else {
          pair = false;
        }
        if (pair) {
          const double dv[2] = {v1, v2};
          const int32_t tv[2] = {op.top, op2.top};
#pragma unroll
          for (int u = 0; u < 2; ++u) {
            const double d = dv[u];
            const int32_t i = tv[u];
            const double a = fabs(d);
            if (a < r.minabs) r.minabs = a;
            if (d < r.minv) r.minv = d;
            const bool neg = mask_le ? (d <= 0.0) : (d < 0.0);
            if (neg && (r.maxloc == 0 || d > best)) { best = d; r.maxloc = i; }
            if (i == capi) r.va = d;
            if (i == capj) r.vb = d;
          }
          ++ip;
          continue;
        }
      }
    }
#endif
    const int32_t node = __builtin_amdgcn_readfirstlane(op.node);
    const double v = prog_value<NEST>(nodes, node, op.action, op.translate_only != 0, q);
    if ((op.action & 3) == PROG_TOP) acc = v;
    else if ((op.action & 3) == PROG_CHILD_FIRST) acc = v;
    else acc = csg(op.op, acc, v, op.k);
    if (op.top > 0) {
      const double d = acc;
      const int32_t i = op.top;
      const double a = fabs(d);
      if (a < r.minabs) r.minabs = a;
      if (d < r.minv) r.minv = d;
      const bool neg = mask_le ? (d <= 0.0) : (d < 0.0);
      if (neg && (r.maxloc == 0 || d > best)) { best = d; r.maxloc = i; }
      if (i == capi) r.va = d;
      if (i == capj) r.vb = d;
    }
  }
  return r;
}

template <bool NEST = false>
__device__ __forceinline__ EvalOut eval_sdfs_coop(const smcrt_sdf_node* __restrict__ nodes,
                                                           const ProgOp* __restrict__ prog, int32_t n_prog,
                                                           int32_t n_top, V3 q, bool mask_le, int32_t capi,
                                                           int32_t capj) {
  const int32_t lane = (int32_t)(threadIdx.x & 63);
  double minabs = __builtin_inf(), minv = __builtin_inf(), best = -__builtin_inf();
  double va = 0.0, vb = 0.0;
  int32_t loc = 0;
  for (int32_t i = lane; i < n_top; i += 64) {
    const int32_t b = prog[n_prog + i].node, e = prog[n_prog + i + 1].node;
    if (b == e) continue;
    double acc = 0.0;
    for (int32_t ip = b; ip < e; ++ip) {
      const ProgOp op = prog[ip];
      const double v = prog_value<NEST>(nodes, op.node, op.action, op.translate_only != 0, q);
      if ((op.action & 3) == PROG_TOP || (op.action & 3) == PROG_CHILD_FIRST) acc = v;
      else acc = csg(op.op, acc, v, op.k);
    }
    const double d = acc;
    const int32_t t = i + 1;
    const double a = fabs(d);
    if (a < minabs) minabs = a;
    if (d < minv) minv = d;
    const bool neg = mask_le ? (d <= 0.0) : (d < 0.0);
    if (neg && (loc == 0 || d > best)) { best = d; loc = t; }
    if (t == capi) va = d;
    if (t == capj) vb = d;
  }
#pragma unroll
  for (int off = 32; off >= 1; off >>= 1) {
    const double m2 = __shfl_xor(minabs, off, 64);
    if (m2 < minabs) minabs = m2;
    const double v2 = __shfl_xor(minv, off, 64);
    if (v2 < minv) minv = v2;
    const double b2 = __shfl_xor(best, off, 64);
    const int32_t l2 = __shfl_xor(loc, off, 64);
    if (l2 != 0 && (loc == 0 || b2 > best || (b2 == best && l2 < loc))) { best = b2; loc = l2; }
  }
  EvalOut r;
  r.minabs = minabs;
  r.minv = minv;
  r.maxloc = loc;
  r.va = capi > 0 ? __shfl(va, (capi - 1) & 63, 64) : 0.0;
  r.vb = capj > 0 ? __shfl(vb, (capj - 1) & 63, 64) : 0.0;
  return r;
}

constexpr int CTAB_ROWS = 21;
constexpr int CTAB_DOUBLES = CTAB_ROWS * 64;

__device__ __forceinline__ double readlane_f64(double v, int l) {
  const uint64_t b = (uint64_t)__double_as_longlong(v);
  const uint32_t lo = (uint32_t)__builtin_amdgcn_readlane((int)(uint32_t)b, l);
  const uint32_t hi = (uint32_t)__builtin_amdgcn_readlane((int)(uint32_t)(b >> 32), l);
  return __longlong_as_double((long long)(((uint64_t)hi << 32) | lo));
}
template <int CTRL, int ROWS>
__device__ __forceinline__ double dpp_f64(double old, double v) {
  const uint64_t b = (uint64_t)__double_as_longlong(v), o = (uint64_t)__double_as_longlong(old);
  const uint32_t lo = (uint32_t)__builtin_amdgcn_update_dpp((int)(uint32_t)o, (int)(uint32_t)b, CTRL, ROWS, 0xf, false);
  const uint32_t hi =
      (uint32_t)__builtin_amdgcn_update_dpp((int)(uint32_t)(o >> 32), (int)(uint32_t)(b >> 32), CTRL, ROWS, 0xf, false);
  return __longlong_as_double((long long)(((uint64_t)hi << 32) | lo));
}
template <int CTRL, int ROWS>
__device__ __forceinline__ int32_t dpp_i32(int32_t old, int32_t v) {
  return __builtin_amdgcn_update_dpp(old, v, CTRL, ROWS, 0xf, false);
}
struct CoopAcc {
  double minabs, minv, best;
  int32_t loc;
};
__device__ __forceinline__ void coop_fold(CoopAcc& a, const CoopAcc& b) {
  if (b.minabs < a.minabs) a.minabs = b.minabs;
  if (b.minv < a.minv) a.minv = b.minv;
  if (b.loc != 0 && (a.loc == 0 || b.best > a.best || (b.best == a.best && b.loc < a.loc))) {
    a.best = b.best;
    a.loc = b.loc;
  }
}
template <int CTRL, int ROWS>
__device__ __forceinline__ void coop_step(CoopAcc& a) {
  CoopAcc b;
  b.minabs = dpp_f64<CTRL, ROWS>(__builtin_inf(), a.minabs);
  b.minv = dpp_f64<CTRL, ROWS>(__builtin_inf(), a.minv);
  b.best = dpp_f64<CTRL, ROWS>(-__builtin_inf(), a.best);
  b.loc = dpp_i32<CTRL, ROWS>(0, a.loc);
  coop_fold(a, b);
// ... 404 lines not shown
```

rsmcrt_amd/csrc/ws.h:

```cpp
#pragma once
#include <hip/hip_runtime.h>
#include <stdint.h>

#include "invoxel.h"
#include "lean.h"

namespace smcrt {

#ifndef SMCRT_WS_PHOTON_WAVES
#define SMCRT_WS_PHOTON_WAVES 8
#endif
#ifndef SMCRT_WS_EVENT_WAVES
#define SMCRT_WS_EVENT_WAVES 1
#endif
#ifndef SMCRT_WS_DDA
#define SMCRT_WS_DDA 2
#endif
#ifndef SMCRT_WS_WAVES
#define SMCRT_WS_WAVES 16
#endif
#ifndef SMCRT_WS_KBOUNDS_PLAIN
#define SMCRT_WS_KBOUNDS_PLAIN 0
#endif
#ifndef SMCRT_WS_EVAL_PAIRS
#define SMCRT_WS_EVAL_PAIRS 0
#endif
#ifndef SMCRT_WS_START_CELLS
#define SMCRT_WS_START_CELLS 1
#endif
#ifndef SMCRT_WS_INVOXEL_LDS
#define SMCRT_WS_INVOXEL_LDS 0
#endif
constexpr uint32_t WS_NO_VOX = 0xFFFFFFFFu;
constexpr int WS_WAVES = SMCRT_WS_WAVES;
constexpr int WS_THREADS = 64 * WS_WAVES;
constexpr int WS_PW = SMCRT_WS_PHOTON_WAVES;
constexpr int WS_EW = SMCRT_WS_EVENT_WAVES;
static_assert(WS_PW >= 1 && WS_EW >= 1 && WS_PW + WS_EW < WS_WAVES, "a block needs all three roles");
constexpr uint32_t WS_NPL = 64u * WS_PW;
constexpr uint32_t ws_pow2(uint32_t v) { return v <= 1 ? 1 : 2 * ws_pow2((v + 1) / 2); }
constexpr uint32_t WS_EQ = ws_pow2(WS_NPL);
constexpr uint32_t WS_CONSUMED = 1u << 12;
constexpr uint32_t WS_SEQ_MASK = 0xFFFFF000u;
__device__ __forceinline__ uint32_t ws_tick(uint32_t t) { return ((t + 1u) & 0x7FFFFu) << 13; }

enum : int { SG_OX = 0, SG_OY, SG_OZ, SG_DX, SG_DY, SG_DZ, SG_LEN, SG_N };
template <uint32_t SL>
struct WsSharedT {
  static constexpr uint32_t SLOTS = SL;
  static constexpr uint32_t RING = ws_pow2(WS_NPL * SL);
  static_assert(SL >= 1 && SL <= 4, "two slot bits in a meta word");
  static_assert(RING >= WS_NPL * SL && RING < (1u << 18), "ring bound");
  double seg[SL][SG_N][WS_NPL];
  uint32_t meta[RING];
  unsigned long long pcell[WS_NPL][SL];
  uint32_t busy[WS_NPL];
  uint32_t lu[3][WS_NPL];
  uint32_t wctr[WS_WAVES][LC_N];
#if SMCRT_WS_INVOXEL_LDS
  double iv_acc[WS_NPL];
  uint32_t iv_vox[WS_NPL];
#endif
  double ev_dir[3][WS_NPL];
  double ev_cached[WS_NPL];
  double ev_tau[WS_NPL];
  uint32_t ev_pid[2][WS_NPL];
  uint32_t ev_draws[WS_NPL];
  uint32_t ev_code[WS_NPL];
  uint32_t evq[WS_EQ];
  uint32_t head, tail;
  uint32_t ev_head, ev_tail;
  uint32_t alive;
  uint32_t abort_;
};
constexpr uint32_t WS_EV_INTERACT = 1u, WS_EV_TAU = 2u, WS_EV_EMIT = 3u, WS_EV_FRESNEL = 4u;

enum : int { WX_ENTRY = 0, WX_START = 6, WX_SSP = 9, WX_ND = 12 };
enum : int { WXI_NEWL = 0, WXI_BOUNCES, WXI_N };
__host__ __device__ constexpr size_t ws_scratch_bytes(size_t lanes) {
  return lanes * (WX_ND * sizeof(double) + WXI_N * sizeof(uint32_t));
}

template <class S>
__device__ __forceinline__ void ws_count(S* sh, int c) {
  const uint64_t m = __ballot(1);
  if ((int)(threadIdx.x & 63) == __builtin_ctzll(m)) atomicAdd(&sh->wctr[threadIdx.x >> 6][c], (uint32_t)__popcll(m));
}

template <class S>
__device__ __forceinline__ uint32_t ws_busy(S* sh, uint32_t pl) {
  return __hip_atomic_load(&sh->busy[pl], __ATOMIC_ACQUIRE, __HIP_MEMORY_SCOPE_WORKGROUP);
}

__device__ __forceinline__ uint32_t ws_load(uint32_t* p) {
  return __hip_atomic_load(p, __ATOMIC_RELAXED, __HIP_MEMORY_SCOPE_WORKGROUP);
}


#ifdef SMCRT_ASM_MARKERS
#define WS_MARK(i) asm volatile("; @@LPHASE " #i)
#else
#define WS_MARK(i) do {} while (0)
#endif
#ifdef SMCRT_DIAG
enum : int { WD_WITERS = 20, WD_WIDLE, WD_WBUSY, WD_WPEND, WD_PTRIPS, WD_PSLEEP, WD_PBLOCKED, WD_PWAIT, WD_P7,
             WD_P7LANES, WD_PIDLE, WD_ELANES, WD_PUSH, WD_PRODWAIT, WD_EITERS, WD_ELANESRUN, WD_PEVQ,
             WD_TP_FETCH, WD_TP_POLL, WD_TP_EVAL, WD_TP_P34, WD_TP_HAND, WD_TP_P56, WD_TP_P7, WD_TP_P8,
             WD_TW_CLAIM, WD_TW_IDLE, WD_TW_WALK, WD_TW_FIN, WD_TE_RUN, WD_TE_IDLE,
             WD_PEMITW,
             WD_N };
static_assert(WD_N <= 64, "g_diag[64..] belongs to transport_kernel");
#define WSDIAG(i, v) (wd[(i) - WD_WITERS] += (uint64_t)(v))
#define WST(i)                                                \
  do {                                                        \
    const uint64_t now_ = __builtin_amdgcn_s_memtime();       \
    wd[(i) - WD_WITERS] += now_ - tprev;                      \
    tprev = now_;                                             \
  } while (0)
#else
#define WSDIAG(i, v) do {} while (0)
#define WST(i) do {} while (0)
#endif

template <bool LDS_FACES, int GM, bool XF, uint32_t SL, bool IV, bool TK>
__global__ __launch_bounds__(WS_THREADS) __attribute__((amdgpu_waves_per_eu(4))) void ws_kernel(
    KParams K, const smcrt_sdf_node* __restrict__ nodes, const ProgOp* __restrict__ prog,
    const KCold* __restrict__ C) {
  using WsShared = WsSharedT<SL>;
  constexpr uint32_t WS_SLOTS = SL, WS_RING = WsShared::RING;
  __shared__ WsShared shm;
  WsShared* sh = &shm;
  const double eps = 1e-8;
  const int lane_id = threadIdx.x & 63;
  const int wv = threadIdx.x >> 6;

  extern __shared__ double sh_dyn[];
  const TopProps* props = K.props;
  const double* xf = K.xface;
  const double* yf = K.yface;
  const double* zf = K.zface;
  int dyn_off = 0;
  if constexpr (LDS_FACES) {
    const int np = 4 * K.n_top;
    const double* gp = (const double*)K.props;
    for (int i = threadIdx.x; i < np; i += blockDim.x) sh_dyn[i] = gp[i];
    const int nf = (K.nx + 1) + (K.ny + 1) + (K.nz + 2);
    double* sh_faces = sh_dyn + np;
    for (int i = threadIdx.x; i < nf; i += blockDim.x) sh_faces[i] = K.xface[i];
    props = (const TopProps*)sh_dyn;
    xf = sh_faces;
    yf = sh_faces + (K.nx + 1);
    zf = yf + (K.ny + 1);
    dyn_off = np + nf;
  }
  unsigned long long* const bstate = (unsigned long long*)(sh_dyn + dyn_off);
  init_buckets(K, C, bstate);
  for (int c = lane_id; c < LC_N; c += 64) sh->wctr[wv][c] = 0;
  for (uint32_t i = threadIdx.x; i < WS_NPL; i += WS_THREADS) {
    sh->busy[i] = 0;
    sh->lu[0][i] = sh->lu[1][i] = sh->lu[2][i] = 0;
#if SMCRT_WS_INVOXEL_LDS
    sh->iv_acc[i] = 0.0;
    sh->iv_vox[i] = WS_NO_VOX;
#endif
  }
  for (uint32_t i = threadIdx.x; i < WS_RING; i += WS_THREADS) sh->meta[i] = 0;
  for (uint32_t i = threadIdx.x; i < WS_EQ; i += WS_THREADS) sh->evq[i] = 0;
  if (threadIdx.x == 0) {
    sh->head = sh->tail = 0;
    sh->ev_head = sh->ev_tail = 0;
    sh->alive = WS_PW;
    sh->abort_ = 0;
  }
  __syncthreads();

  uint32_t w_iters = 0, w_sdf = 0, w_dep = 0, hazards = 0;
  uint32_t r_upd = 0, r_scat = 0, r_tau = 0, r_abs = 0, r_inv = 0;
#ifdef SMCRT_DIAG
  uint64_t wd[WD_N - WD_WITERS] = {};
  uint64_t tprev = __builtin_amdgcn_s_memtime();
#endif
  if (wv < WS_PW) {
    WS_MARK(1);
    const bool test_kernel = TK && (K.flags & SMCRT_FLAG_TEST_KERNEL) != 0;
    const bool records_on = (K.flags & SMCRT_FLAG_RECORD_PHOTONS) != 0 && C->records != nullptr;
    const uint32_t pl = threadIdx.x;
#define WLU(f) (sh->lu[(f)][pl])
    const double mf = (K.lean_debug & 3u) ? 0.0 : 2.0 * eps;
    const double mx0 = mf * (double)(K.nx + 2), my0 = mf * (double)(K.ny + 2), mz0 = mf * (double)(K.nz + 2);
    const double ex0 = 2.0 * K.xmax - mx0, ey0 = 2.0 * K.ymax - my0, ez0 = 2.0 * K.zmax - mz0;
    const bool defer_all = (K.lean_debug & 3u) == 2u;
    bool drop_event = (K.lean_debug & 4u) && blockIdx.x == 0 && pl == 0;
    const bool invoxel_on = IV && K.ws_invoxel != 0 && (K.flags & SMCRT_FLAG_PATHLENGTH) != 0;
#if SMCRT_WS_INVOXEL_LDS
#define WS_IV_ACC (sh->iv_acc[pl])
#define WS_IV_VOX (sh->iv_vox[pl])
#else
    double iv_acc = 0.0;
    uint32_t iv_vox = WS_NO_VOX;
#define WS_IV_ACC iv_acc
#define WS_IV_VOX iv_vox
#endif
    auto iv_flush = [&]() {
      const uint32_t av = WS_IV_VOX;
      if (av != WS_NO_VOX) {
        atomic_add_nr(C->jmean + av, WS_IV_ACC);
        WS_IV_ACC = 0.0;
        WS_IV_VOX = WS_NO_VOX;
      }
    };
    uint64_t wait_t0 = 0;
    const size_t xs = (size_t)gridDim.x * WS_NPL;
    double* const X = XF ? C->lane_scratch + (size_t)blockIdx.x * WS_NPL + pl : nullptr;
    uint32_t* const XI = XF ? (uint32_t*)(C->lane_scratch + WX_ND * xs) + (size_t)blockIdx.x * WS_NPL + pl
                                         : nullptr;
    LeanPhoton P;
    P.st = ST_FETCH; P.f = LF_CELLS;
    P.pos = P.dir = v3(0.0, 0.0, 0.0);
    P.tau = P.taurun = P.d = P.minabs = 0.0;
    P.layer = P.xcell = P.ycell = P.zcell = 0;
    P.hop = P.loopc = P.seq = 0;
    P.rng.init(0);
    uint64_t chunk_base = 0;
    uint32_t chunk_left = 0;
    bool more = true;
    auto t2_entry = [&]() {
      if constexpr (XF) {
        X[(WX_ENTRY + 0) * xs] = P.pos.x; X[(WX_ENTRY + 1) * xs] = P.pos.y; X[(WX_ENTRY + 2) * xs] = P.pos.z;
        X[(WX_ENTRY + 3) * xs] = P.dir.x; X[(WX_ENTRY + 4) * xs] = P.dir.y; X[(WX_ENTRY + 5) * xs] = P.dir.z;
        X[(WX_START + 0) * xs] = P.pos.x; X[(WX_START + 1) * xs] = P.pos.y; X[(WX_START + 2) * xs] = P.pos.z;
      }
    };

    auto p8 = [&]() {
      if (!(P.f & (LF_REQ | LF_WAIT | LF_PEND)) && P.st == ST_H0) {
        if (!(P.taurun <= P.tau)) P.st = ST_T2END;
        else if (++P.hop > (uint32_t)MAX_HOP_ITERS) { P.set(LF_FAULT | LF_TFLAG); P.st = ST_T2END; }
        else P.set(LF_PEND);
      }
    };
    for (;; ++w_iters) {
      {
        uint64_t need = __ballot(P.st == ST_FETCH);
        while (need && more) {
          if (chunk_left == 0) {
            unsigned long long base = 0;
            if (lane_id == 0) base = atomicAdd(C->queue, (unsigned long long)SMCRT_FETCH_CHUNK);
            chunk_base = __shfl(base, 0, 64);
            const uint64_t n_photons = C->n_photons;
            chunk_left = (chunk_base < n_photons)
                             ? (uint32_t)((n_photons - chunk_base) < SMCRT_FETCH_CHUNK ? (n_photons - chunk_base)
                                                                                         : SMCRT_FETCH_CHUNK)
                             : 0u;
            if (chunk_left == 0) { more = false; break; }
          }
          const uint32_t n = __popcll(need);
          const uint32_t take = n < chunk_left ? n : chunk_left;
          const uint64_t rank = __popcll(need & ((1ull << lane_id) - 1ull));
          if (P.st == ST_FETCH && rank < take) {
            if constexpr (TK) {
              P.rng.init(C->first_photon + chunk_base + rank);
              sh->ev_pid[0][pl] = P.rng.pid_lo; sh->ev_pid[1][pl] = P.rng.pid_hi;
            } else {
              const uint64_t pid = C->first_photon + chunk_base + rank;
              sh->ev_pid[0][pl] = (uint32_t)pid; sh->ev_pid[1][pl] = (uint32_t)(pid >> 32);
              sh->ev_draws[pl] = 0u;
              sh->ev_cached[pl] = 0.0;
            }
            P.st = ST_EMIT;
          }
          chunk_base += take;
          chunk_left -= take;
          need = __ballot(P.st == ST_FETCH);
        }
        if (!more && P.st == ST_FETCH) P.st = ST_IDLE;
        const uint64_t live = __ballot(P.st != ST_IDLE);
        if (live == 0) break;
      }
      WST(WD_TP_FETCH);
      if (P.has(LF_EVQ)) {
        const uint32_t code = __hip_atomic_load(&sh->ev_code[pl], __ATOMIC_ACQUIRE, __HIP_MEMORY_SCOPE_WORKGROUP);
        if (code & EV_DONE) {
          P.clr(LF_EVQ);
          if constexpr (TK) {
            P.rng.draws = sh->ev_draws[pl];
            P.rng.cached = sh->ev_cached[pl];
          }
          if (P.st == ST_EMIT) {
            P.pos = v3(sh->seg[P.seq][SG_OX][pl], sh->seg[P.seq][SG_OY][pl], sh->seg[P.seq][SG_OZ][pl]);
            P.dir = v3(sh->ev_dir[0][pl], sh->ev_dir[1][pl], sh->ev_dir[2][pl]);
            P.clr(LF_TFLAG);
            P.layer = (int32_t)(code & 0xFFFFu);
            P.xcell = vox_of<GM>(P.pos.x, K.nx, K.xmax, K.inv2x, K.fex);
            P.ycell = vox_of<GM>(P.pos.y, K.ny, K.ymax, K.inv2y, K.fey);
            P.zcell = vox_of<GM>(P.pos.z, K.nz, K.zmax, K.inv2z, K.fez);
            P.set(LF_CELLS);
            if (code & EV_RUNAWAY) { P.set(LF_FAULT); P.st = ST_DONE; }
            else { P.st = ST_LAYER; P.set(LF_PEND); }
          } else if (XF && P.st == ST_F0) {
            if (code & EV_RUNAWAY) {
              P.set(LF_FAULT | LF_TFLAG); P.st = ST_T2END;
            } else if (code & EV_FR_REFLECT) {
              X[WX_START * xs] = P.pos.x; X[(WX_START + 1) * xs] = P.pos.y; X[(WX_START + 2) * xs] = P.pos.z;
              const uint32_t nb = XI[WXI_BOUNCES * xs] + 1u;
              XI[WXI_BOUNCES * xs] = nb;
              if (nb > 1000u) {
                ws_count(sh, LC_BABORT);
                P.pos = v3(X[WX_ENTRY * xs], X[(WX_ENTRY + 1) * xs], X[(WX_ENTRY + 2) * xs]);
                P.dir = v3(X[(WX_ENTRY + 3) * xs], X[(WX_ENTRY + 4) * xs], X[(WX_ENTRY + 5) * xs]);
                P.st = ST_INTERACT;
              } else {
                P.dir = v3(sh->ev_dir[0][pl], sh->ev_dir[1][pl], sh->ev_dir[2][pl]);
                P.st = ST_H0;
                p8();
              }
            } else {
              X[WX_SSP * xs] = sh->seg[P.seq][SG_DX][pl];
              X[(WX_SSP + 1) * xs] = sh->seg[P.seq][SG_DY][pl];
              X[(WX_SSP + 2) * xs] = sh->seg[P.seq][SG_DZ][pl];
              P.dir = v3(sh->ev_dir[0][pl], sh->ev_dir[1][pl], sh->ev_dir[2][pl]);
              P.layer = (int32_t)XI[WXI_NEWL * xs];
              P.st = ST_X1;
              P.set(LF_REQ | LF_SSP);
            }
          } else if (code & EV_ABSORB) {
            P.set(LF_TFLAG);
            P.st = ST_ABSORB;
          } else {
            if (code & EV_RUNAWAY) P.set(LF_FAULT | LF_TFLAG);
            P.dir = v3(sh->ev_dir[0][pl], sh->ev_dir[1][pl], sh->ev_dir[2][pl]);
            P.tau = sh->ev_tau[pl];
            P.taurun = 0.0;
            P.hop = 0;
            P.st = ST_H0;
            t2_entry();
            p8();
          }
        }
      }
      WSDIAG(WD_PTRIPS, 1);
      WSDIAG(WD_PIDLE, __popcll(__ballot(P.st == ST_IDLE)));
      WSDIAG(WD_PWAIT, __popcll(__ballot(P.has(LF_WAIT))));
      WSDIAG(WD_PEVQ, __popcll(__ballot(P.has(LF_EVQ))));
      WSDIAG(WD_PEMITW, __popcll(__ballot(!TK && P.st == ST_EMIT && !P.has(LF_EVQ) && (ws_busy(sh, pl) & (1u << P.seq)))));

      WST(WD_TP_POLL);
      const bool have = (P.f & (LF_PEND | LF_REQ | LF_WAIT)) == LF_PEND;
      EvalOut R;
      R.minabs = R.minv = R.va = R.vb = 0.0; R.maxloc = 0;
      if (__ballot(have)) {
        const bool mask_le = test_kernel && P.st == ST_LAYER;
        const V3 q = (P.st == ST_H1 || P.st == ST_G0) ? P.pos + smul(P.d, P.dir) : P.pos;
        R = eval_sdfs<false, SMCRT_WS_EVAL_PAIRS != 0>(nodes, prog, K.n_prog, q, mask_le, 0, 0);
        const bool counted = P.st == ST_H0 || P.st == ST_H1 || P.st == ST_H3 || P.st == ST_M1 || P.st == ST_G0;
        w_sdf += __popcll(__ballot(have && counted)) * (uint32_t)K.n_top;
        WSDIAG(WD_ELANES, __popcll(__ballot(have)));
        if (have) P.clr(LF_PEND);
      }

      WST(WD_TP_EVAL);
      if (have && (P.st == ST_H0 || P.st == ST_H3 || P.st == ST_M1)) {
        const uint32_t st0 = P.st;
        P.minabs = R.minabs;
        const bool small = st0 == ST_H0 && R.minabs < eps;
        const bool out = st0 != ST_H0 && R.minv > 0.0;
        if (out) P.set(LF_TFLAG);
        if (st0 == ST_H0) P.loopc = 0;
        const bool done = P.taurun >= P.tau || P.has(LF_TFLAG);
        P.d = small ? R.minabs + 2.0 * eps : R.minabs;
        uint32_t ns = st0 == ST_M1 ? (out ? (uint32_t)ST_B0 : (uint32_t)ST_M0) : (done ? (uint32_t)ST_T2END : (uint32_t)ST_M0);
        if (small) { ns = ST_H1; P.set(LF_PEND); }
        P.st = ns;
      } else if (have) {
        switch (P.st) {
          case ST_LAYER:
            P.layer = R.maxloc;
            if (P.layer == 0) { P.set(LF_FAULT); P.st = ST_DONE; }
            else P.st = ST_T2;
            break;
          case ST_H1: {
            const double kap = props[P.layer - 1].kappa;
            const double t = P.d * kap;
            if (R.maxloc == P.layer) {
              if (P.taurun + t < P.tau) { P.set(LF_MOVE_FWD); P.taurun = P.taurun + t; }
              else { P.d = (P.tau - P.taurun) / kap; P.taurun = P.taurun + t; }
            } else {
              if (P.taurun + t < P.tau) { P.set(LF_MOVE_BACK); P.taurun = P.taurun + t; }
              else { P.d = (P.tau - P.taurun) / kap; P.set(LF_MOVE_BACK); }
            }
            P.st = ST_H2;
            P.set(LF_REQ);
            break;
          }
          case ST_G0: {
            const int32_t new_layer = R.maxloc;
            if (new_layer == P.layer && R.minabs < eps) {
              if (++P.loopc > (uint32_t)MAX_GLANCE_ITERS) { P.set(LF_FAULT | LF_TFLAG); P.st = ST_T2END; break; }
              P.d = P.d + eps;
              P.set(LF_PEND);
              break;
            }
            if (new_layer == 0) { P.set(LF_TFLAG); P.st = ST_T2END; break; }
            if (XF && props[P.layer - 1].n != props[new_layer - 1].n) {
              XI[WXI_NEWL * xs] = (uint32_t)new_layer;
              P.st = ST_F0;
              break;
            }
            P.layer = new_layer;
            P.st = ST_X1;
            P.set(LF_REQ);
            break;
          }
          default:
            break;
        }
      }

      if (!(P.f & (LF_REQ | LF_WAIT)) && P.st == ST_M0) {
        if (!(P.d >= eps)) {
          P.st = ST_B0;
        } else if (++P.loopc > (uint32_t)MAX_MARCH_ITERS) {
          P.set(LF_FAULT | LF_TFLAG); P.st = ST_B0;
        } else {
          const double kap = props[P.layer - 1].kappa;
          const double t = P.d * kap;
          if (P.taurun + t < P.tau) {
            P.taurun = P.taurun + t;
            P.st = ST_M1; P.set(LF_PEND);
          } else {
            P.d = (P.tau - P.taurun) / kap;
            P.taurun = P.tau;
            P.st = ST_B0;
          }
          P.set(LF_REQ | LF_MOVE_FWD);
        }
      }

      WST(WD_TP_P34);
      if (__ballot(P.has(LF_REQ))) {
        bool push = false, sync = false;
        V3 old = v3(0.0, 0.0, 0.0);
        const uint32_t slot = P.seq;
        bool inv = false;
        int32_t ci = -1, cj = -1, ck = -1;
        if constexpr (IV) {
          if (P.has(LF_REQ)) {
            old = v3(P.pos.x + K.xmax, P.pos.y + K.ymax, P.pos.z + K.zmax);
            ci = cell_of<GM>(old.x, K.nx, K.xmax, K.inv2x, K.fex);
            cj = cell_of<GM>(old.y, K.ny, K.ymax, K.inv2y, K.fey);
            ck = cell_of<GM>(old.z, K.nz, K.zmax, K.inv2z, K.fez);
            if (invoxel_on && ci != -1 && cj != -1 && ck != -1)
              inv = invoxel_segment(old.x, old.y, old.z, P.dir.x, P.dir.y, P.dir.z, P.d,
                                    face<GM>(xf, P.dir.x > 0.0 ? ci : ci - 1, K.fex),
                                    face<GM>(yf, P.dir.y > 0.0 ? cj : cj - 1, K.fey),
                                    face<GM>(zf, P.dir.z > 0.0 ? ck : ck - 1, K.fez));
          }
        }
        if (inv) {
          ++r_upd;
          ++r_inv;
          const uint32_t vox = lin(K, ci, cj, ck);
          if (WS_IV_VOX != vox) {
            iv_flush();
            WS_IV_VOX = vox;
          }
          WS_IV_ACC = WS_IV_ACC + (double)(float)P.d;
          if (P.has(LF_MOVE_FWD)) P.pos = P.pos + smul(P.d, P.dir);
          else if (P.has(LF_MOVE_BACK)) P.pos = P.pos - smul(P.d, P.dir);
          P.clr(LF_REQ | LF_MOVE_FWD | LF_MOVE_BACK);
          P.xcell = ci; P.ycell = cj; P.zcell = ck;
          P.set(LF_CELLS);
        } else if (P.has(LF_REQ) && !(ws_busy(sh, pl) & (1u << slot))) {
          ++r_upd;
          if constexpr (!IV) {
            old = v3(P.pos.x + K.xmax, P.pos.y + K.ymax, P.pos.z + K.zmax);
            ci = cell_of<GM>(old.x, K.nx, K.xmax, K.inv2x, K.fex);
            cj = cell_of<GM>(old.y, K.ny, K.ymax, K.inv2y, K.fey);
            ck = cell_of<GM>(old.z, K.nz, K.zmax, K.inv2z, K.fez);
          }
          if (P.has(LF_MOVE_FWD)) P.pos = P.pos + smul(P.d, P.dir);
          else if (P.has(LF_MOVE_BACK)) P.pos = P.pos - smul(P.d, P.dir);
          P.clr(LF_REQ | LF_MOVE_FWD | LF_MOVE_BACK);
          if (ci == -1 || cj == -1 || ck == -1) {
            P.set(LF_TFLAG | LF_CELLS);
            P.xcell = ci; P.ycell = cj; P.zcell = ck;
          } else {
            const double len = P.d;
            const V3 e = v3(old.x + P.dir.x * len, old.y + P.dir.y * len, old.z + P.dir.z * len);
            constexpr bool KB = XF || SMCRT_WS_KBOUNDS_PLAIN;
            const double mx = KB ? K.lean_lo[0] : mx0, my = KB ? K.lean_lo[1] : my0, mz = KB ? K.lean_lo[2] : mz0;
            const double ex = KB ? K.lean_hi[0] : ex0, ey = KB ? K.lean_hi[1] : ey0, ez = KB ? K.lean_hi[2] : ez0;
            const bool inside = old.x >= mx && old.x <= ex && old.y >= my && old.y <= ey && old.z >= mz &&
                                old.z <= ez && e.x >= mx && e.x <= ex && e.y >= my && e.y <= ey && e.z >= mz &&
                                e.z <= ez;
            push = true;
            sync = !inside && !defer_all;
#if SMCRT_WS_START_CELLS
            sh->pcell[pl][slot] = lean_pack(ci, cj, ck);
#endif
            if constexpr (GM != 2) {
              const bool in_cell = face<GM>(xf, ci - 1, K.fex) <= old.x && old.x <= face<GM>(xf, ci, K.fex) &&
                                   face<GM>(yf, cj - 1, K.fey) <= old.y && old.y <= face<GM>(yf, cj, K.fey) &&
                                   face<GM>(zf, ck - 1, K.fez) <= old.z && old.z <= face<GM>(zf, ck, K.fez);
              if (!in_cell) sync = true;
            }
          }
        }
        const uint64_t pm = __ballot(push);
        WSDIAG(WD_PUSH, __popcll(pm));
        WSDIAG(WD_PBLOCKED, __popcll(__ballot(P.has(LF_REQ))));
        if (pm) {
          const int first = __builtin_ctzll(pm);
          uint32_t base = 0;
          if (lane_id == first) base = atomicAdd(&sh->tail, (uint32_t)__popcll(pm));
          base = __builtin_amdgcn_readlane(base, first);
          if (push) {
            const uint32_t rank = __builtin_amdgcn_mbcnt_hi((uint32_t)(pm >> 32), __builtin_amdgcn_mbcnt_lo((uint32_t)pm, 0u));
            const uint32_t t = base + rank;
            const uint32_t ix = t & (WS_RING - 1);
            double* const sg = &sh->seg[slot][0][pl];
            sg[SG_OX * WS_NPL] = old.x; sg[SG_OY * WS_NPL] = old.y; sg[SG_OZ * WS_NPL] = old.z;
            sg[SG_DX * WS_NPL] = P.dir.x; sg[SG_DY * WS_NPL] = P.dir.y; sg[SG_DZ * WS_NPL] = P.dir.z;
            sg[SG_LEN * WS_NPL] = P.d;
            atomicOr(&sh->busy[pl], 1u << slot);
            const uint32_t prev = t < WS_RING ? 0u : (ws_tick(t - WS_RING) | WS_CONSUMED);
            uint64_t t0 = 0;
            while (__hip_atomic_load(&sh->meta[ix], __ATOMIC_RELAXED, __HIP_MEMORY_SCOPE_WORKGROUP) != prev) {
              WSDIAG(WD_PRODWAIT, 1);
              __builtin_amdgcn_s_sleep(1);
              if (!t0) t0 = __builtin_amdgcn_s_memrealtime();
              else if (watchdog_expired(C, t0, WDOG_RING)) break;
            }
            __hip_atomic_store(&sh->meta[ix], pl | (slot << 9) | (sync ? (1u << 11) : 0u) | ws_tick(t),
                               __ATOMIC_RELEASE, __HIP_MEMORY_SCOPE_WORKGROUP);
            P.seq = P.seq + 1 == WS_SLOTS ? 0u : P.seq + 1;
            P.clr(LF_CELLS);
            if (sync) P.set(LF_WAIT);
          }
        }
      }

      WST(WD_TP_HAND);
      if (P.has(LF_WAIT) && !(ws_busy(sh, pl) & (1u << ((P.seq + WS_SLOTS - 1) % WS_SLOTS)))) {
        const unsigned long long w = sh->pcell[pl][(P.seq + WS_SLOTS - 1) % WS_SLOTS];
        P.xcell = lean_cell(w, 0); P.ycell = lean_cell(w, 1); P.zcell = lean_cell(w, 2);
        P.set(LF_CELLS);
        if (w & LEAN_TFLAG) P.set(LF_TFLAG);
        if (w & LEAN_FAULT) P.set(LF_FAULT);
        P.clr(LF_WAIT);
      }
      const bool free_ = !(P.f & (LF_REQ | LF_WAIT));
      if (free_ && (P.st == ST_H2 || P.st == ST_B0 || P.st == ST_X1)) {
        if (P.st == ST_X1) {
          P.taurun = P.taurun + P.d * props[P.layer - 1].kappa;
          if (XF && P.has(LF_SSP)) P.pos = v3(X[WX_SSP * xs], X[(WX_SSP + 1) * xs], X[(WX_SSP + 2) * xs]);
          else P.pos = P.pos + smul(P.d, P.dir);
          P.clr(LF_SSP);
        }
        if (XF && K.n_dets) {
          const V3 st = v3(X[WX_START * xs], X[(WX_START + 1) * xs], X[(WX_START + 2) * xs]);
          const double sep = pointsep(P.pos, st);
          X[WX_START * xs] = P.pos.x; X[(WX_START + 1) * xs] = P.pos.y; X[(WX_START + 2) * xs] = P.pos.z;
          const uint32_t hits = record_hits(K, C->det_bins, K.dets, K.det_off, st, P.dir, sep, P.layer, 1.0);
          if (hits) atomicAdd(&sh->wctr[wv][LC_HITS], hits);
        }
        if (P.st == ST_H2) {
          P.st = ST_H3; P.set(LF_PEND);
        } else if (P.st == ST_X1) {
          P.st = P.has(LF_TFLAG) ? ST_T2END : ST_H0;
        } else if (P.taurun >= P.tau || P.has(LF_TFLAG)) {
          P.st = ST_T2END;
        } else {
          P.d = P.minabs + 2.0 * eps;
          P.loopc = 0;
          P.st = ST_G0; P.set(LF_PEND);
        }
      }

      if (free_ && P.st == ST_T2END) {
        if (fabs(P.pos.x) > K.xmax) P.set(LF_TFLAG);
        if (fabs(P.pos.y) > K.ymax) P.set(LF_TFLAG);
        if (fabs(P.pos.z) > K.zmax) P.set(LF_TFLAG);
        P.st = ST_INTERACT;
      }
      if (!P.has(LF_CELLS) && (P.st == ST_ABSORB || (records_on && P.st == ST_DONE)) && ws_busy(sh, pl) == 0) {
        const unsigned long long w = sh->pcell[pl][(P.seq + WS_SLOTS - 1) % WS_SLOTS];
        P.xcell = lean_cell(w, 0); P.ycell = lean_cell(w, 1); P.zcell = lean_cell(w, 2);
        P.set(LF_CELLS);
      }
      if (P.st == ST_ABSORB && P.has(LF_CELLS)) {
        if (P.xcell < 1 || P.xcell > K.nx || P.ycell < 1 || P.ycell > K.ny || P.zcell < 1 || P.zcell > K.nz)
          P.set(LF_FAULT);
        else if (C->absorb) atomic_add_nr(C->absorb + lin(K, P.xcell, P.ycell, P.zcell), 1.0);
        P.st = ST_DONE;
      }

      WST(WD_TP_P56);
      {
        bool qev = free_ && !P.has(LF_EVQ) &&
                   ((!test_kernel && ((P.st == ST_INTERACT && !(P.f & (LF_TFLAG | LF_FAULT)) &&
                                     WLU(LL_INTER) + 1u <= (uint32_t)MAX_INTERACTIONS) ||
                                    P.st == ST_T2 || (P.st == ST_EMIT && !(ws_busy(sh, pl) & (1u << P.seq))))) ||
                    (XF && P.st == ST_F0 && !(ws_busy(sh, pl) & (1u << P.seq))));
        if (drop_event && qev) {
          drop_event = qev = false;
          __hip_atomic_store(&sh->ev_code[pl], 0u, __ATOMIC_RELAXED, __HIP_MEMORY_SCOPE_WORKGROUP);
          P.set(LF_EVQ);
        }
        const uint64_t qm = __ballot(qev);
        if (qm) {
          const int first = __builtin_ctzll(qm);
          uint32_t base = 0;
          if (lane_id == first) base = atomicAdd(&sh->ev_tail, (uint32_t)__popcll(qm));
          base = __builtin_amdgcn_readlane(base, first);
          if (qev) {
            const uint32_t t = base + __builtin_amdgcn_mbcnt_hi((uint32_t)(qm >> 32), __builtin_amdgcn_mbcnt_lo((uint32_t)qm, 0u));
            const uint32_t ix = t & (WS_EQ - 1);
            const uint32_t prev = t < WS_EQ ? 0u : (ws_tick(t - WS_EQ) | WS_CONSUMED);
            uint64_t t0 = 0;
            while (__hip_atomic_load(&sh->evq[ix], __ATOMIC_ACQUIRE, __HIP_MEMORY_SCOPE_WORKGROUP) != prev) {
              __builtin_amdgcn_s_sleep(1);
              if (!t0) t0 = __builtin_amdgcn_s_memrealtime();
              else if (watchdog_expired(C, t0, WDOG_EVENT_QUEUE)) break;
            }
            sh->ev_dir[0][pl] = P.dir.x; sh->ev_dir[1][pl] = P.dir.y; sh->ev_dir[2][pl] = P.dir.z;
            if constexpr (TK) {
              sh->ev_cached[pl] = P.rng.cached;
              sh->ev_draws[pl] = P.rng.draws;
            }
            if (XF && P.st == ST_F0) {
              sh->seg[P.seq][SG_OX][pl] = P.pos.x; sh->seg[P.seq][SG_OY][pl] = P.pos.y;
              sh->seg[P.seq][SG_OZ][pl] = P.pos.z; sh->seg[P.seq][SG_LEN][pl] = P.d;
              sh->ev_tau[pl] = (double)XI[WXI_NEWL * xs];
            }
            if (P.st == ST_EMIT) {
              P.clr(LF_FAULT); P.layer = 0;
              WLU(LL_STATUS) = 0; WLU(LL_NSCATT) = 0; WLU(LL_INTER) = 0;
              if constexpr (XF) XI[WXI_BOUNCES * xs] = 0;
            }
            sh->ev_code[pl] = (uint32_t)P.layer |
                              ((P.st == ST_INTERACT ? WS_EV_INTERACT
                                : (P.st == ST_T2 ? WS_EV_TAU : (P.st == ST_EMIT ? WS_EV_EMIT : WS_EV_FRESNEL))) << 16) |
                              (P.seq << 19);
            __hip_atomic_store(&sh->evq[ix], pl | ws_tick(t), __ATOMIC_RELEASE, __HIP_MEMORY_SCOPE_WORKGROUP);
            P.set(LF_EVQ);
          }
        }
      }
      {
        const bool ev = free_ && !P.has(LF_EVQ) &&
                        (P.st == ST_INTERACT || P.st == ST_DONE || (TK && (P.st == ST_T2 || P.st == ST_EMIT)));
        const uint64_t evm = __ballot(ev);
        const uint64_t busy = __ballot(P.st != ST_IDLE && P.st != ST_FETCH && !P.has(LF_EVQ) &&
                                       (TK || P.st != ST_EMIT));
        const uint32_t nev = __popcll(evm);
        const uint32_t batch = test_kernel ? (uint32_t)SMCRT_LEAN_EVENT_LANES : 4u;
        const bool run_ev = nev && (nev >= batch || evm == busy);
        WSDIAG(WD_P7, run_ev ? 1 : 0);
        WSDIAG(WD_P7LANES, run_ev ? nev : 0);
        if (run_ev) {
          if (ev && P.st == ST_INTERACT) {
            if (P.f & (LF_TFLAG | LF_FAULT)) {
              P.st = ST_DONE;
            } else if (WLU(LL_INTER) + 1u > (uint32_t)MAX_INTERACTIONS) {
              ++WLU(LL_INTER);
              P.set(LF_FAULT); P.st = ST_DONE;
            } else if constexpr (TK) {
              const double ran = P.rng.next(K.key0, K.key1);
              const TopProps pr = props[P.layer - 1];
              const bool sc = ran < pr.albedo;
              ++WLU(LL_INTER);
              if (!sc) {
                P.set(LF_TFLAG); WLU(LL_STATUS) = 1; ++r_abs;
                P.st = test_kernel ? ST_DONE : ST_ABSORB;
              } else {
                Lane L;
                L.dir = P.dir; L.rng = P.rng; L.fault = false; L.tflag = false;
                scatter(K, L, pr.hgg);
                P.dir = L.dir; P.rng = L.rng;
                if (L.fault) P.set(LF_FAULT | LF_TFLAG);
                const uint32_t st = ++WLU(LL_NSCATT);
                ++r_scat;
                if (test_kernel) {
                  if (st >= 1 && st <= 4) {
                    double* const moments = C->moments;
                    if (moments) {
                      double* m = moments + 3 * (st - 1);
                      double* m2 = moments + 12 + 3 * (st - 1);
                      atomic_add_nr(m + 0, P.pos.x); atomic_add_nr(m + 1, P.pos.y); atomic_add_nr(m + 2, P.pos.z);
                      atomic_add_nr(m2 + 0, P.pos.x * P.pos.x);
                      atomic_add_nr(m2 + 1, P.pos.y * P.pos.y);
                      atomic_add_nr(m2 + 2, P.pos.z * P.pos.z);
                    }
                  } else if (K.flags & SMCRT_FLAG_END_EARLY) {
                    P.set(LF_TFLAG);
                    WLU(LL_STATUS) = 4;
                  }
                }
                P.st = ST_T2;
              }
            }
          }
          if (TK && ev && P.st == ST_T2) {
            ++r_tau;
            t2_entry();
            P.tau = -det_log(P.rng.next(K.key0, K.key1));
            P.taurun = 0.0;
            P.hop = 0;
            P.st = ST_H0;
          }
          if (TK && ev && P.st == ST_EMIT) {
            P.clr(LF_FAULT); P.layer = 0;
            WLU(LL_STATUS) = 0; WLU(LL_NSCATT) = 0; WLU(LL_INTER) = 0;
            if constexpr (XF) XI[WXI_BOUNCES * xs] = 0;
            Lane L;
            L.rng = P.rng; L.xcell = L.ycell = L.zcell = 0; L.layer = 0; L.tflag = false;
            emit<GM, false>(K, C, L, 0u);
            if (!test_kernel) {
              int64_t tries = 0;
              while (cell_out(K, L)) {
                if (++tries > MAX_EMIT_TRIES) { P.set(LF_FAULT); break; }
                ws_count(sh, LC_RETRIES);
                emit<GM, false>(K, C, L, 0u);
              }
            }
            P.pos = L.pos; P.dir = L.dir; P.rng = L.rng; P.clr(LF_TFLAG);
            P.layer = L.layer;
            P.xcell = L.xcell; P.ycell = L.ycell; P.zcell = L.zcell;
            P.set(LF_CELLS);
            if (!test_kernel && !P.has(LF_FAULT) && (K.flags & SMCRT_FLAG_RENDER_SOURCE) && C->emission)
              atomic_add_nr(C->emission + lin(K, P.xcell, P.ycell, P.zcell), 1.0);
            if (P.has(LF_FAULT)) P.st = ST_DONE;
            else { P.st = ST_LAYER; P.set(LF_PEND); }
          }
          if (ev && P.st == ST_DONE && (P.has(LF_CELLS) || !records_on)) {
            if (P.has(LF_FAULT)) { WLU(LL_STATUS) = 3; ws_count(sh, LC_FAULTS); }
            else if (WLU(LL_STATUS) == 0) { WLU(LL_STATUS) = 2; ws_count(sh, LC_ESCAPED); }
            ws_count(sh, LC_PHOTONS);
            const uint32_t draws = TK ? P.rng.draws : sh->ev_draws[pl];
            atomicAdd(&sh->wctr[wv][LC_DRAWS], draws);
            iv_flush();
#ifdef SMCRT_DIAG
            if (C->done_time) {
              const uint64_t dp = TK ? ((uint64_t)P.rng.pid_hi << 32) | P.rng.pid_lo
                                     : ((uint64_t)sh->ev_pid[1][pl] << 32) | sh->ev_pid[0][pl];
              C->done_time[dp - C->done_base] = __builtin_amdgcn_s_memrealtime();
            }
#endif
            if (records_on) {
              const uint64_t pid = TK ? ((uint64_t)P.rng.pid_hi << 32) | P.rng.pid_lo
                                      : ((uint64_t)sh->ev_pid[1][pl] << 32) | sh->ev_pid[0][pl];
              smcrt_photon_record* r = C->records + (pid - C->first_photon);
              r->pos[0] = P.pos.x; r->pos[1] = P.pos.y; r->pos[2] = P.pos.z;
              r->dir[0] = P.dir.x; r->dir[1] = P.dir.y; r->dir[2] = P.dir.z;
              r->weight = 1.0;
              r->cell[0] = P.xcell; r->cell[1] = P.ycell; r->cell[2] = P.zcell;
              r->layer = P.layer;
              r->nscatt = WLU(LL_NSCATT);
              r->bounces = XF ? XI[WXI_BOUNCES * xs] : 0u;
              r->draws = draws;
              r->status = WLU(LL_STATUS);
            }
            P.clr(LF_TFLAG | LF_FAULT);
            P.st = ST_FETCH;
          }
        }
      }

      WST(WD_TP_P7);
      p8();
      if (__ballot(P.st != ST_IDLE && !(P.has(LF_WAIT) || P.has(LF_REQ) || P.has(LF_EVQ) ||
                                        (P.st == ST_ABSORB && !P.has(LF_CELLS)) || (!TK && P.st == ST_EMIT))) == 0) {
        WSDIAG(WD_PSLEEP, 1);
        __builtin_amdgcn_s_sleep(1);
        if (!wait_t0) {
          wait_t0 = __builtin_amdgcn_s_memrealtime();
        } else if (ws_load(&sh->abort_) || watchdog_expired(C, wait_t0, WDOG_PHOTON_WAVE)) {
          if (lane_id == 0) __hip_atomic_store(&sh->abort_, 1u, __ATOMIC_RELAXED, __HIP_MEMORY_SCOPE_WORKGROUP);
          break;
        }
      } else {
        wait_t0 = 0;
      }
      WST(WD_TP_P8);
    }
    iv_flush();
#undef WS_IV_ACC
#undef WS_IV_VOX
#undef WLU
    if (lane_id == 0) atomicSub(&sh->alive, 1u);
  } else if (wv < WS_PW + WS_EW) {
    WS_MARK(2);
    __builtin_amdgcn_s_setprio(3);
    bool pend = false;
    uint32_t tk = 0;
    for (;; ++w_iters) {
// ... 89 lines not shown
            const V3 N = v3(nn.x / ln, nn.y / ln, nn.z / ln);
            const double n1 = props[layer - 1].n, n2 = props[new_layer - 1].n;
            ws_count(sh, LC_FRES);
            const double Rf = fresnel(dir0, N, n1, n2);
            V3 dn;
            if (rg.next(K.key0, K.key1) <= Rf) {
              dn = reflect_dir(dir0, N);
              ws_count(sh, LC_REFL);
              res = EV_FR_REFLECT;
            } else {
              sh->seg[es][SG_DX][o] = ssp.x; sh->seg[es][SG_DY][o] = ssp.y; sh->seg[es][SG_DZ][o] = ssp.z;
              dn = refract_dir(dir0, N, n1, n2);
            }
            sh->ev_dir[0][o] = dn.x; sh->ev_dir[1][o] = dn.y; sh->ev_dir[2][o] = dn.z;
          }
        } else if (kind == WS_EV_INTERACT) {
          const TopProps pr = props[layer - 1];
          const double ran = rg.next(K.key0, K.key1);
          ++sh->lu[LL_INTER][o];
          if (!(ran < pr.albedo)) {
            sh->lu[LL_STATUS][o] = 1;
            ++r_abs;
            res = EV_ABSORB;
          } else {
            Lane L;
            L.dir = v3(sh->ev_dir[0][o], sh->ev_dir[1][o], sh->ev_dir[2][o]);
            L.rng = rg; L.fault = false; L.tflag = false;
            scatter(K, L, pr.hgg);
            rg = L.rng;
            if (L.fault) res = EV_RUNAWAY;
            ++sh->lu[LL_NSCATT][o];
            ++r_scat;
            sh->ev_dir[0][o] = L.dir.x; sh->ev_dir[1][o] = L.dir.y; sh->ev_dir[2][o] = L.dir.z;
            tau_entry = true;
          }
        }
        if (tau_entry) {
          ++r_tau;
          sh->ev_tau[o] = -det_log(rg.next(K.key0, K.key1));
        }
        sh->ev_draws[o] = rg.draws;
        sh->ev_cached[o] = rg.cached;
        __hip_atomic_store(&sh->ev_code[o], res | EV_DONE, __ATOMIC_RELEASE, __HIP_MEMORY_SCOPE_WORKGROUP);
      }
      WST(WD_TE_RUN);
    }
  } else {
    WS_MARK(10);
    WalkSeg W;
    W.old = v3(0.0, 0.0, 0.0);
    W.sd = W.slen = 0.0;
    W.xcell = W.ycell = W.zcell = 0;
    W.dda_it = 0;
    W.seg = W.tflag = W.fault = false;
    V3 wdir = v3(0.0, 0.0, 0.0);
    V3 wrcp = v3(0.0, 0.0, 0.0);
    uint32_t wmeta = 0;
    BucketLog WB;
    WB.next = WB.end = 0;
    uint32_t overflow = 0;
    bool pend = false;
    uint32_t tk = 0;
    for (;; ++w_iters) {
      WS_MARK(11);
      const uint64_t cm = __ballot(!W.seg && !pend);
      if (cm) {
        const int first = __builtin_ctzll(cm);
        uint32_t base = 0;
        if (lane_id == first) base = atomicAdd(&sh->head, (uint32_t)__popcll(cm));
        base = __builtin_amdgcn_readlane(base, first);
        if (!W.seg && !pend) {
          tk = base + __builtin_amdgcn_mbcnt_hi((uint32_t)(cm >> 32), __builtin_amdgcn_mbcnt_lo((uint32_t)cm, 0u));
          pend = true;
        }
      }
      if (pend) {
        const uint32_t ix = tk & (WS_RING - 1);
        const uint32_t m = __hip_atomic_load(&sh->meta[ix], __ATOMIC_ACQUIRE, __HIP_MEMORY_SCOPE_WORKGROUP);
        if ((m & WS_SEQ_MASK) == ws_tick(tk)) {
          __hip_atomic_store(&sh->meta[ix], ws_tick(tk) | WS_CONSUMED, __ATOMIC_RELAXED, __HIP_MEMORY_SCOPE_WORKGROUP);
          const double* const sg = &sh->seg[(m >> 9) & 3u][0][m & 511u];
          const V3 o = v3(sg[SG_OX * WS_NPL], sg[SG_OY * WS_NPL], sg[SG_OZ * WS_NPL]);
          const V3 dd = v3(sg[SG_DX * WS_NPL], sg[SG_DY * WS_NPL], sg[SG_DZ * WS_NPL]);
          const double l = sg[SG_LEN * WS_NPL];
          W.old = o;
          wdir = dd;
          wrcp = v3(ieee_rcp_f64(dd.x), ieee_rcp_f64(dd.y), ieee_rcp_f64(dd.z));
          W.slen = l;
          wmeta = m;
#if SMCRT_WS_START_CELLS
          {
            const unsigned long long cw = sh->pcell[m & 511u][(m >> 9) & 3u];
            W.xcell = lean_cell(cw, 0); W.ycell = lean_cell(cw, 1); W.zcell = lean_cell(cw, 2);
          }
#else
          W.xcell = cell_of<GM>(W.old.x, K.nx, K.xmax, K.inv2x, K.fex);
          W.ycell = cell_of<GM>(W.old.y, K.ny, K.ymax, K.inv2y, K.fey);
          W.zcell = cell_of<GM>(W.old.z, K.nz, K.zmax, K.inv2z, K.fez);
#endif
          W.sd = 0.0; W.dda_it = 0;
          W.seg = true; W.tflag = false; W.fault = false;
          pend = false;
        }
      }
      const uint64_t am = __ballot(W.seg);
      WSDIAG(WD_WITERS, 1);
      WSDIAG(WD_WIDLE, am ? 0 : 1);
      WSDIAG(WD_WBUSY, __popcll(am));
      WSDIAG(WD_WPEND, __popcll(__ballot(pend)));
      WST(WD_TW_CLAIM);
      if (!am) {
        if (ws_load(&sh->abort_)) break;
        if (ws_load(&sh->alive) == 0) {
          const uint32_t T = ws_load(&sh->tail);
          if (pend && (int32_t)(tk - T) >= 0) pend = false;
          if (!__ballot(pend) && (int32_t)(ws_load(&sh->head) - T) >= 0) break;
        }
        __builtin_amdgcn_s_sleep(2);
        WST(WD_TW_IDLE);
        continue;
      }
      WS_MARK(12);
#pragma unroll
      for (int k = 0; k < SMCRT_WS_DDA; ++k) {
        if (k > 0 && !__ballot(W.seg)) break;
        bool dep = false;
        uint32_t vox = 0;
        double val = 0.0;
        if (W.seg) dda_step_r<GM>(K, W, wdir, wrcp, xf, yf, zf, dep, vox, val, 1.0);
        w_dep += __popcll(__ballot(dep));
        WS_MARK(13);
        emit_bucketed(K, C, WB, dep, vox, val, overflow, bstate);
      }
      WS_MARK(14);
      WST(WD_TW_WALK);
      if ((am >> lane_id & 1ull) && !W.seg) {
        const uint32_t owner = wmeta & 511u, slot = (wmeta >> 9) & 3u;
        const bool sync = (wmeta & (1u << 11)) != 0;
        if (!sync && (W.tflag || W.fault)) ++hazards;
        sh->pcell[owner][slot] = lean_pack(W.xcell, W.ycell, W.zcell) | (W.tflag ? LEAN_TFLAG : 0ull) |
                                 (W.fault ? LEAN_FAULT : 0ull);
        __hip_atomic_fetch_and(&sh->busy[owner], ~(1u << slot), __ATOMIC_RELEASE, __HIP_MEMORY_SCOPE_WORKGROUP);
      }
      WST(WD_TW_FIN);
    }
    WS_MARK(15);
    close_buckets(K, C, WB, w_dep - overflow, overflow);
  }
  WS_MARK(16);
  {
    unsigned long long* const counters = C->counters;
    const uint32_t hz = wave_sum_u32(hazards);
    const uint32_t n_upd = wave_sum_u32(r_upd), n_scat = wave_sum_u32(r_scat), n_tau = wave_sum_u32(r_tau),
                   n_abs = wave_sum_u32(r_abs), n_inv = wave_sum_u32(r_inv);
    if (lane_id == 0) {
      if (hz) {
        atomicAdd(C->dep_ctl + 5, hz);
        atomicAdd(C->lean_hazards, (unsigned long long)hz);
      }
      if (C->dep_ctl && n_upd) atomicAdd(C->dep_ctl + 6, n_upd);
      if (n_inv) atomicAdd(C->invoxel_segs, (unsigned long long)n_inv);
      if (counters) {
        const uint32_t* c = sh->wctr[wv];
        const uint32_t v[SMCRT_NCOUNTERS] = {c[LC_PHOTONS], c[LC_RETRIES], n_scat,        n_abs,          w_sdf,
                                             w_dep + n_inv, n_upd,         n_tau,          c[LC_FRES],     c[LC_REFL],
                                             c[LC_BABORT],  c[LC_FAULTS] + hz, c[LC_DRAWS], c[LC_HITS],   c[LC_ESCAPED],
                                             w_iters};
        for (int i = 0; i < SMCRT_NCOUNTERS; ++i)
          if (v[i]) atomicAdd(counters + i, (unsigned long long)v[i]);
      }
      double* const nscatt = C->nscatt;
      if (nscatt && n_scat) atomic_add_nr(nscatt, (double)n_scat);
    }
  }
#ifdef SMCRT_DIAG
  if (lane_id == 0)
    for (int i = 0; i < WD_N - WD_WITERS; ++i)
      if (wd[i]) atomicAdd(&::g_diag[WD_WITERS + i], (unsigned long long)wd[i]);
#endif
  __syncthreads();
  close_block_buckets(K, C, bstate);
}

}
```

rsmcrt_amd/engine.py:

```python
from __future__ import annotations

import ctypes as C
import os
import threading

import numpy as np

from . import abi
from .scene import MeshScene, Mono, VoxelScene, detector_array
from .tallies import Result

LIB_PATH = os.environ.get("SMCRT_LIB") or os.path.join(os.path.dirname(os.path.abspath(__file__)), "libsmcrt.so")
_lock = threading.Lock()
_lib = None


class SmcrtError(RuntimeError):
    pass


def load_library(path: str = LIB_PATH):
    global _lib
    with _lock:
        if _lib is not None:
# ... 252 lines not shown
        m = cfg.max_steps
        out = np.zeros((5, m))
        tg = np.ascontiguousarray(targets, dtype=np.float64)
        rc = self.config(n_photons, seed, flags, 0)
        t = result.tallies() if result is not None else None
        _check(load_library().smcrt_inverse_run(self._h, C.byref(source), C.byref(cfg), C.byref(rc),
                                                tg.ctypes.data_as(C.POINTER(C.c_double)),
                                                out.ctypes.data_as(C.POINTER(C.c_double)),
                                                C.byref(t) if t is not None else None))
        return out.T.copy()

    def run_device(self, source, cfg: abi.RunConfig, dev: abi.DeviceTallies, stream: int = 0):
        _check(load_library().smcrt_run_device(self._h, C.byref(source), C.byref(cfg), C.byref(dev),
                                               C.c_void_p(stream)))

    def reduce_device_tallies(self, comm: "Comm", dev: abi.DeviceTallies, root: int = -1, stream: int = 0):
        _check(load_library().smcrt_reduce_device_tallies(self._h, comm._h, C.byref(dev), int(root),
                                                          C.c_void_p(stream)))

    def fence(self, stream: int = 0):
        _check(load_library().smcrt_scene_fence(self._h, C.c_void_p(stream)))

    def check(self):
        _check(load_library().smcrt_scene_check(self._h))

    def set_timing(self, enable: bool = True):
        _check(load_library().smcrt_scene_set_timing(self._h, 1 if enable else 0))

    def kernel_times(self) -> dict:
        t = abi.KernelTimes()
        _check(load_library().smcrt_scene_kernel_times(self._h, C.byref(t)))
        return {"transport_ms": t.transport_ms, "deposit_ms": t.deposit_ms, "launches": t.launches,
                "lean_launches": t.lean_launches, "far_steps": t.far_steps,
                "fold_cu_ms": t.fold_cu_ms, "lean_hazards": t.lean_hazards}

    def deposit_regime(self) -> str:
        r = C.c_int32()
        _check(load_library().smcrt_scene_deposit_regime(self._h, C.byref(r)))
        return abi.DEPOSIT_REGIMES[r.value]

    def set_path_tracking(self, range_first=0, range_count=0, max_vertices=64, max_paths=65536):
        if range_first is None:
            _check(load_library().smcrt_scene_set_path_tracking(self._h, None))
            return
        cfg = abi.PathConfig()
        cfg.range_first, cfg.range_count = int(range_first), int(range_count)
        cfg.max_vertices, cfg.max_paths = int(max_vertices), int(max_paths)
        _check(load_library().smcrt_scene_set_path_tracking(self._h, C.byref(cfg)))

    def paths(self):
        L = load_library()
        c = [C.c_int64() for _ in range(4)]
        _check(L.smcrt_scene_path_counts(self._h, *[C.byref(x) for x in c]))
        counts = dict(zip(("n_paths", "n_vertices", "n_dropped", "n_truncated"), (x.value for x in c)))
        hdr = np.zeros(counts["n_paths"], dtype=abi.path_dtype())
        vtx = np.zeros((counts["n_vertices"], 4))
        if len(hdr):
            _check(L.smcrt_scene_read_paths(self._h, hdr.ctypes.data_as(C.c_void_p),
                                            vtx.ctypes.data_as(C.POINTER(C.c_double))))
        return hdr, vtx, counts

    def set_partial_paths(self, range_first=0, range_count=0, max_records=65536):
        if range_first is None:
            _check(load_library().smcrt_scene_set_partial_paths(self._h, None))
            return
        cfg = abi.PPathConfig()
        cfg.range_first, cfg.range_count, cfg.max_records = int(range_first), int(range_count), int(max_records)
        _check(load_library().smcrt_scene_set_partial_paths(self._h, C.byref(cfg)))

    def partial_paths(self):
        L = load_library()
        c = [C.c_int64() for _ in range(2)]
        _check(L.smcrt_scene_partial_path_counts(self._h, *[C.byref(x) for x in c]))
        counts = dict(zip(("n_records", "n_dropped"), (x.value for x in c)))
        hdr = np.zeros(counts["n_records"], dtype=abi.ppath_dtype())
        lens = np.zeros((counts["n_records"], self.scene.n_media))
        if len(hdr):
            _check(L.smcrt_scene_read_partial_paths(self._h, hdr.ctypes.data_as(C.c_void_p),
                                                    lens.ctypes.data_as(C.POINTER(C.c_double))))
        return hdr, lens, counts

    def set_phasor(self, wavenumber="sampled", optical_path=False):
        L = load_library()
        if wavenumber is None:
            _check(L.smcrt_scene_set_phasor(self._h, None))
            return
        cfg = abi.PhasorConfig()
        if not (isinstance(wavenumber, str) and wavenumber == "sampled"):
            cfg.fixed_k, cfg.wavenumber = 1, float(wavenumber)
        cfg.reserved = abi.PHASOR_OPTICAL_PATH if optical_path else 0
        _check(L.smcrt_scene_set_phasor(self._h, C.byref(cfg)))

    def phasor(self) -> np.ndarray:
        g = self.grid
        out = np.zeros((g.nz, g.ny, g.nx), dtype=np.complex128)
        _check(load_library().smcrt_scene_read_phasor(self._h, out.ctypes.data_as(C.POINTER(C.c_double))))
        return out

    def reset_phasor(self):
        _check(load_library().smcrt_scene_reset_phasor(self._h))

    def set_screens(self, screens):
        L = load_library()
        screens = list(screens) if screens is not None else []
        if not screens:
            _check(L.smcrt_scene_set_screens(self._h, None, 0))
            self._screen_dims = []
            return
        arr = (abi.Screen * len(screens))(*screens)
        _check(L.smcrt_scene_set_screens(self._h, arr, len(screens)))
        self._screen_dims = [(int(s.nv), int(s.nu)) for s in screens]

    def screens(self):
        L = load_library()
        n, nd = C.c_int32(), C.c_int64()
        _check(L.smcrt_scene_screen_info(self._h, C.byref(n), C.byref(nd)))
        flat = np.zeros(max(nd.value, 2), dtype=np.float64)
        _check(L.smcrt_scene_read_screens(self._h, flat.ctypes.data_as(C.POINTER(C.c_double))))
        out, off = [], 0
        for nv, nu in getattr(self, "_screen_dims", []):
            out.append(flat[off:off + 2 * nu * nv].view(np.complex128).reshape(nv, nu).copy())
            off += 2 * nu * nv
        assert len(out) == n.value and off == nd.value
        return out

    def reset_screens(self):
        _check(load_library().smcrt_scene_reset_screens(self._h))

    def set_volume_source(self, weights):
        L = load_library()
        if weights is None:
            _check(L.smcrt_scene_set_volume_source(self._h, None))
            return
        g = self.grid
        w = np.asarray(weights, dtype=np.float64)
        if w.shape != (g.nz * g.ny * g.nx,) and w.shape != (g.nz, g.ny, g.nx):
            raise ValueError(f"weights of shape {w.shape}: expected ({g.nz * g.ny * g.nx},) or ({g.nz}, {g.ny}, {g.nx})")
        w = np.ascontiguousarray(w).reshape(-1)
        _check(L.smcrt_scene_set_volume_source(self._h, w.ctypes.data_as(C.POINTER(C.c_double))))

    def volume_source_info(self) -> dict:
        a, b, t = C.c_int64(), C.c_int64(), C.c_double()
        _check(load_library().smcrt_scene_volume_source_info(self._h, C.byref(a), C.byref(b), C.byref(t)))
        return {"n_positive": a.value, "n_reachable": b.value, "total": t.value}

    def invoxel_segments(self) -> int:
        fn = load_library().smcrt_scene_invoxel_segments
        fn.argtypes = [C.c_void_p, C.POINTER(C.c_int64)]
        n = C.c_int64()
        _check(fn(self._h, C.byref(n)))
        return n.value


def pack_layout(grid, n_det_bins: int, fields: int) -> abi.PackLayout:
    lay = abi.PackLayout()
    lay.n_voxels, lay.n_det_bins, lay.fields = grid.nx * grid.ny * grid.nz, int(n_det_bins), int(fields)
    return lay


def pack_result(res: Result, fields: int) -> np.ndarray:
    L = load_library()
    lay = pack_layout(res.grid, sum(res.det_sizes), fields)
    n = C.c_int64()
    _check(L.smcrt_pack_size(C.byref(lay), C.byref(n)))
    buf = np.zeros(n.value)
    t = res.tallies()
    _check(L.smcrt_pack_host(C.byref(lay), C.byref(t), buf.ctypes.data_as(C.POINTER(C.c_double))))
    return buf


def unpack_into(res: Result, buf: np.ndarray, fields: int) -> Result:
    L = load_library()
    lay = pack_layout(res.grid, sum(res.det_sizes), fields)
    b = np.ascontiguousarray(buf, dtype=np.float64)
    t = res.tallies()
    _check(L.smcrt_unpack_host(C.byref(lay), b.ctypes.data_as(C.POINTER(C.c_double)), C.byref(t)))
    return res


class Comm:

    @staticmethod
    def unique_id() -> bytes:
        buf = (C.c_uint8 * abi.UNIQUE_ID_BYTES)()
        _check(load_library().smcrt_comm_unique_id(buf))
        return bytes(buf)

    def __init__(self, uid: bytes, n_ranks: int, rank: int, device: int):
        buf = (C.c_uint8 * abi.UNIQUE_ID_BYTES).from_buffer_copy(uid)
        h = C.c_void_p()
        _check(load_library().smcrt_comm_init_rank(buf, int(n_ranks), int(rank), int(device), C.byref(h)))
        self._h = h

    def info(self) -> dict:
        n, r, d = C.c_int32(), C.c_int32(), C.c_int32()
        _check(load_library().smcrt_comm_info(self._h, C.byref(n), C.byref(r), C.byref(d)))
        return {"n_ranks": n.value, "rank": r.value, "device": d.value}

    @property
    def n_ranks(self) -> int:
        return self.info()["n_ranks"]

    def close(self):
        if getattr(self, "_h", None):
            load_library().smcrt_comm_destroy(self._h)
            self._h = None

    def __del__(self):
        try:
            self.close()
        except Exception:
            pass


class MultiEngine:

    def __init__(self, scene, grid, dets=(), devices=None):
        L = load_library()
        self.scene, self.grid, self.dets = scene, grid, list(dets)
        self._nodes = scene.node_array()
        self._top = scene.top_array()
        self._darr = detector_array(self.dets)
        devs = None if devices is None else (C.c_int32 * len(devices))(*devices)
        h = C.c_void_p()
        _check(L.smcrt_multi_create(self._nodes, len(scene.nodes), self._top, scene.n_top, C.byref(grid),
                                    self._darr, len(self.dets), devs, len(devices) if devices else 0, C.byref(h)))
        self._h = h
        n = C.c_int32()
        _check(L.smcrt_multi_info(h, C.byref(n)))
        self.n_devices = n.value
        self._pending = 0

    def close(self):
        if getattr(self, "_h", None):
            load_library().smcrt_multi_destroy(self._h)
            self._h = None

    def __del__(self):
        try:
            self.close()
        except Exception:
            pass

    def __enter__(self):
        return self

    def __exit__(self, *exc):
        self.close()

    def run(self, source, n_photons, seed=123456789, flags=abi.FLAG_PATHLENGTH, first_photon=0,
            result: Result | None = None) -> Result:
        res = result if result is not None else Result(self.grid, self.dets, n_photons)
        res.n_photons += int(n_photons) + self._pending
        self._pending = 0
        cfg = Engine.config(n_photons, seed, flags, first_photon)
        t = res.tallies()
        _check(load_library().smcrt_multi_run(self._h, C.byref(source), C.byref(cfg), C.byref(t)))
        return res

    def accumulate(self, source, n_photons, seed=123456789, flags=abi.FLAG_PATHLENGTH, first_photon=0):
        cfg = Engine.config(n_photons, seed, flags, first_photon)
        try:
            _check(load_library().smcrt_multi_accumulate(self._h, C.byref(source), C.byref(cfg)))
        except SmcrtError:
            self._pending = 0
            raise
        self._pending += int(n_photons)

    def device_photons(self):
        out = (C.c_uint64 * self.n_devices)()
        _check(load_library().smcrt_multi_device_photons(self._h, out))
        return list(out)

    def collect(self, result: Result | None = None) -> Result:
        res = result if result is not None else Result(self.grid, self.dets, 0)
        held = sum(self.device_photons())
        if held != self._pending:
            raise SmcrtError(f"multi-device photon count mismatch: the devices hold {held} photons, "
                             f"{self._pending} were accumulated since the last collect")
        res.n_photons += held
        self._pending = 0
        t = res.tallies()
        _check(load_library().smcrt_multi_collect(self._h, C.byref(t)))
        return res
```

Baseline: 286.2 million.

## Let photon lanes hand segments to any free slot instead of strict round-robin

The work-stealing walker used to hand each deposit segment to the next slot in a fixed ring and stalled when that slot was busy. It now picks the lowest free slot, tracking the last pushed slot and the emission slot together in P.seq, and waits on the last slot used. It also turns on K-bounds and paired SDF evaluation by default for GM==2 through a traits struct, and adds an out-of-order hand-out counter, a debug switch that disables pairs, and an optional wave-priority setting. The aim is fewer photon lanes stuck behind busy slots, at the cost of more bookkeeping and ordering that is harder to reason about.

```diff
diff --git a/include/smcrt.h b/include/smcrt.h
--- a/include/smcrt.h
+++ b/include/smcrt.h
@@ -412,6 +412,8 @@
 
 int smcrt_scene_invoxel_segments(smcrt_scene* scene, int64_t* out);
 
+int smcrt_scene_out_of_order_handouts(smcrt_scene* scene, int64_t* out);
+
 int smcrt_normalise_fluence(float* grid, const smcrt_grid* g, uint64_t nphotons);
 
 typedef enum smcrt_symmetry {
diff --git a/rsmcrt_amd/abi.py b/rsmcrt_amd/abi.py
--- a/rsmcrt_amd/abi.py
+++ b/rsmcrt_amd/abi.py
@@ -275,7 +275,7 @@
     "smcrt_multi_scene", "smcrt_multi_run", "smcrt_multi_accumulate", "smcrt_multi_collect",
     "smcrt_multi_device_photons", "smcrt_multi_destroy", "smcrt_job_run_devices",
     "smcrt_spectral_sample", "smcrt_scene_set_spectral", "smcrt_scene_check",
-    "smcrt_scene_invoxel_segments",
+    "smcrt_scene_invoxel_segments", "smcrt_scene_out_of_order_handouts",
     "smcrt_scene_set_path_tracking", "smcrt_scene_path_counts", "smcrt_scene_read_paths", "smcrt_write_paths",
     "smcrt_job_history_filename",
     "smcrt_scene_set_phasor", "smcrt_scene_read_phasor", "smcrt_scene_reset_phasor",
diff --git a/rsmcrt_amd/csrc/sceneplan.cpp b/rsmcrt_amd/csrc/sceneplan.cpp
--- a/rsmcrt_amd/csrc/sceneplan.cpp
+++ b/rsmcrt_amd/csrc/sceneplan.cpp
@@ -62,6 +62,8 @@
   if (const char* cd = std::getenv("SMCRT_DEBUG_CLAIM_DELAY")) k.claim_delay = (uint32_t)std::strtoul(cd, nullptr, 10);
   const char* de = std::getenv("SMCRT_DEBUG_DROP_EVENT");
   k.drop_event = de && de[0] == '1';
+  const char* el = std::getenv("SMCRT_DEBUG_EVAL_LOOP");
+  k.eval_loop = el && el[0] == '1';
   if (const char* pv = std::getenv("SMCRT_PATH_VERTICES")) k.path_vertices = (int32_t)std::strtol(pv, nullptr, 10);
   if (const char* pm = std::getenv("SMCRT_PATH_MAX")) k.path_max = (int64_t)std::strtoll(pm, nullptr, 10);
   return k;
diff --git a/rsmcrt_amd/csrc/sceneplan.h b/rsmcrt_amd/csrc/sceneplan.h
--- a/rsmcrt_amd/csrc/sceneplan.h
+++ b/rsmcrt_amd/csrc/sceneplan.h
@@ -26,6 +26,7 @@
   Q_LEAN_HAZARDS,
   Q_WATCHDOG,
   Q_INVOXEL,
+  Q_OOO_HANDOUTS,
   Q_COUNT
 };
 constexpr int N_QUEUES = Q_CALLER + 1;
@@ -61,6 +62,7 @@
   double watchdog_ms = DEFAULT_WATCHDOG_MS;
   uint32_t claim_delay = 0;
   bool drop_event = false;
+  bool eval_loop = false;
   bool diag_done = false;
 };
 struct PoolKnobs {
diff --git a/rsmcrt_amd/csrc/smcrt.hip b/rsmcrt_amd/csrc/smcrt.hip
--- a/rsmcrt_amd/csrc/smcrt.hip
+++ b/rsmcrt_amd/csrc/smcrt.hip
@@ -701,10 +701,12 @@
     std::fprintf(stderr, "[diag-ws] walker iters %llu: idle %.3f, busy lanes/iter %.1f, pending lanes/iter %.1f | "
                  "photon trips %llu: sleep %.3f, idle lanes %.1f, sync-waiting %.2f, slot-blocked %.2f, EVAL lanes "
                  "%.1f, pushes %.2f, P7 runs %.3f (lanes/run %.1f), event-waiting %.2f | producer waits %llu | event "
-                 "iters %llu, lanes/iter %.1f | emissions waiting for a slot %llu lane-trips\n",
+                 "iters %llu, lanes/iter %.1f | emissions waiting for a slot %llu lane-trips | out-of-order hand-outs "
+                 "%llu (%.3f of the pushes)\n",
                  h[20], h[21] / wi, h[22] / wi, h[23] / wi, h[24], h[25] / pt, h[30] / pt, h[27] / pt, h[26] / pt,
                  h[31] / pt, h[32] / pt, h[28] / pt, (double)h[29] / (double)std::max(1ull, h[28]), h[36] / pt, h[33],
-                 h[34], (double)h[35] / (double)std::max(1ull, h[34]), h[51]);
+                 h[34], (double)h[35] / (double)std::max(1ull, h[34]), h[51], h[52],
+                 (double)h[52] / (double)std::max(1ull, h[32]));
     const char* np[8] = {"fetch", "poll", "eval", "p3p4", "handout", "p5p6", "p7", "p8"};
     double tp = 0, tw = 0, te = 0;
     for (int i = 0; i < 8; ++i) tp += (double)h[37 + i];
@@ -801,6 +803,7 @@
   Ch.far_steps = s->d_queue + Q_FAR_STEPS;
   Ch.lean_hazards = s->d_queue + Q_LEAN_HAZARDS;
   Ch.invoxel_segs = s->d_queue + Q_INVOXEL;
+  Ch.ooo_handouts = s->d_queue + Q_OOO_HANDOUTS;
   Ch.lane_scratch = nullptr;
   Ch.watchdog = watchdog_word(s);
   const bool hist = run.hist, phas = run.phas, scr = run.scr;
@@ -860,7 +863,7 @@
   Ch.watchdog_ticks = knobs.watchdog_ms > 0.0 ? (uint64_t)(knobs.watchdog_ms * (double)s->wall_khz) : 0ull;
   K.rec_pool = nullptr; K.n_chunks = 0; K.hist_tiles = 0; K.bucket_tiles = 0; K.n_buckets = 0;
   K.claim_delay = knobs.claim_delay;
-  K.lean_debug = s->lean_debug | (knobs.drop_event ? 4u : 0u);
+  K.lean_debug = s->lean_debug | (knobs.drop_event ? 4u : 0u) | (knobs.eval_loop ? 8u : 0u);
   K.ws_invoxel = ws_invoxel_on(s->ws_invoxel, plan_xf(*s)) ? 1u : 0u;
   lean_margins(K.lean_debug, s->grid, K.lean_lo, K.lean_hi);
   return SMCRT_OK;
@@ -1292,6 +1295,17 @@
   return SMCRT_OK;
 }
 
+int smcrt_scene_out_of_order_handouts(smcrt_scene* s, int64_t* out) {
+  if (!s || !out) return fail(SMCRT_ERR_INVALID_ARG, "NULL argument");
+  if (const int vst = smcrt::scene_needs_sdf(s, "smcrt_scene_out_of_order_handouts")) return vst;
+  std::lock_guard<std::mutex> g(s->mu);
+  HIPCHK(hipSetDevice(s->device));
+  unsigned long long n = 0;
+  HIPCHK(hipMemcpy(&n, s->d_queue + Q_OOO_HANDOUTS, sizeof(n), hipMemcpyDeviceToHost));
+  *out = (int64_t)n;
+  return SMCRT_OK;
+}
+
 static void release_paths(smcrt_scene* s) {
   s->path_on = false;
   s->d_hist_scratch.reset(); s->d_path_vertices.reset(); s->d_path_headers.reset(); s->d_path_ctl.reset();
diff --git a/rsmcrt_amd/csrc/transport.h b/rsmcrt_amd/csrc/transport.h
--- a/rsmcrt_amd/csrc/transport.h
+++ b/rsmcrt_amd/csrc/transport.h
@@ -52,6 +52,7 @@
   unsigned long long* far_steps;
   unsigned long long* lean_hazards;
   unsigned long long* invoxel_segs;
+  unsigned long long* ooo_handouts;
   double* lane_scratch;
   uint32_t* watchdog;
   uint64_t watchdog_ticks;
@@ -901,7 +902,7 @@
 template <bool NEST = false, bool PAIRS = false>
 __device__ __forceinline__ EvalOut eval_sdfs(const smcrt_sdf_node* __restrict__ nodes,
                                              const ProgOp* __restrict__ prog, int32_t n_prog, V3 q,
-                                             bool mask_le, int32_t capi, int32_t capj) {
+                                             bool mask_le, int32_t capi, int32_t capj, bool pairs_on = true) {
   EvalOut r;
   r.minabs = __builtin_inf();
   r.minv = __builtin_inf();
@@ -912,7 +913,7 @@
   for (int32_t ip = 0; ip < n_prog; ++ip) {
     const ProgOp op = prog[ip];
 #if SMCRT_EVAL_PAIRS
-    if (PAIRS && !NEST && ip + 1 < n_prog && op.action == PROG_TOP && op.top > 0) {
+    if (PAIRS && !NEST && pairs_on && ip + 1 < n_prog && op.action == PROG_TOP && op.top > 0) {
       const ProgOp op2 = prog[ip + 1];
       if (op2.action == PROG_TOP && op2.top > 0) {
         const smcrt_sdf_node* n1 = nodes + __builtin_amdgcn_readfirstlane(op.node);
diff --git a/rsmcrt_amd/csrc/ws.h b/rsmcrt_amd/csrc/ws.h
--- a/rsmcrt_amd/csrc/ws.h
+++ b/rsmcrt_amd/csrc/ws.h
@@ -19,14 +19,27 @@
 #ifndef SMCRT_WS_WAVES
 #define SMCRT_WS_WAVES 16
 #endif
-#ifndef SMCRT_WS_KBOUNDS_PLAIN
-#define SMCRT_WS_KBOUNDS_PLAIN 0
-#endif
-#ifndef SMCRT_WS_EVAL_PAIRS
-#define SMCRT_WS_EVAL_PAIRS 0
-#endif
 #ifndef SMCRT_WS_START_CELLS
 #define SMCRT_WS_START_CELLS 1
+#endif
+template <int GM, bool XF>
+struct WsTraits {
+#ifdef SMCRT_WS_KBOUNDS_PLAIN
+  static constexpr bool KBOUNDS = XF || SMCRT_WS_KBOUNDS_PLAIN != 0;
+#else
+  static constexpr bool KBOUNDS = XF || GM == 2;
+#endif
+#ifdef SMCRT_WS_EVAL_PAIRS
+  static constexpr bool EVAL_PAIRS = SMCRT_WS_EVAL_PAIRS != 0;
+#else
+  static constexpr bool EVAL_PAIRS = GM == 2 && !XF;
+#endif
+};
+#ifndef SMCRT_WS_ANY_SLOT
+#define SMCRT_WS_ANY_SLOT 1
+#endif
+#ifndef SMCRT_WS_PHOTON_PRIO
+#define SMCRT_WS_PHOTON_PRIO 0
 #endif
 #ifndef SMCRT_WS_INVOXEL_LDS
 #define SMCRT_WS_INVOXEL_LDS 0
@@ -92,6 +105,18 @@
   return __hip_atomic_load(&sh->busy[pl], __ATOMIC_ACQUIRE, __HIP_MEMORY_SCOPE_WORKGROUP);
 }
 
+template <uint32_t SL>
+__device__ __forceinline__ uint32_t ws_next(uint32_t last) { return last + 1u == SL ? 0u : last + 1u; }
+template <uint32_t SL>
+__device__ __forceinline__ uint32_t ws_pick(uint32_t busy, uint32_t last) {
+#if SMCRT_WS_ANY_SLOT
+  return (uint32_t)__builtin_ctz(~busy | (1u << SL));
+#else
+  const uint32_t s = ws_next<SL>(last);
+  return (busy >> s & 1u) ? SL : s;
+#endif
+}
+
 __device__ __forceinline__ uint32_t ws_load(uint32_t* p) {
   return __hip_atomic_load(p, __ATOMIC_RELAXED, __HIP_MEMORY_SCOPE_WORKGROUP);
 }
@@ -108,6 +133,7 @@
              WD_TP_FETCH, WD_TP_POLL, WD_TP_EVAL, WD_TP_P34, WD_TP_HAND, WD_TP_P56, WD_TP_P7, WD_TP_P8,
              WD_TW_CLAIM, WD_TW_IDLE, WD_TW_WALK, WD_TW_FIN, WD_TE_RUN, WD_TE_IDLE,
              WD_PEMITW,
+             WD_POOO,
              WD_N };
 static_assert(WD_N <= 64, "g_diag[64..] belongs to transport_kernel");
 #define WSDIAG(i, v) (wd[(i) - WD_WITERS] += (uint64_t)(v))
@@ -175,7 +201,7 @@
   __syncthreads();
 
   uint32_t w_iters = 0, w_sdf = 0, w_dep = 0, hazards = 0;
-  uint32_t r_upd = 0, r_scat = 0, r_tau = 0, r_abs = 0, r_inv = 0;
+  uint32_t r_upd = 0, r_scat = 0, r_tau = 0, r_abs = 0, r_inv = 0, r_ooo = 0;
 #ifdef SMCRT_DIAG
   uint64_t wd[WD_N - WD_WITERS] = {};
   uint64_t tprev = __builtin_amdgcn_s_memtime();
@@ -185,6 +211,7 @@
     const bool test_kernel = TK && (K.flags & SMCRT_FLAG_TEST_KERNEL) != 0;
     const bool records_on = (K.flags & SMCRT_FLAG_RECORD_PHOTONS) != 0 && C->records != nullptr;
     const uint32_t pl = threadIdx.x;
+    if constexpr (SMCRT_WS_PHOTON_PRIO != 0) __builtin_amdgcn_s_setprio(SMCRT_WS_PHOTON_PRIO);
 #define WLU(f) (sh->lu[(f)][pl])
     const double mf = (K.lean_debug & 3u) ? 0.0 : 2.0 * eps;
     const double mx0 = mf * (double)(K.nx + 2), my0 = mf * (double)(K.ny + 2), mz0 = mf * (double)(K.nz + 2);
@@ -219,7 +246,8 @@
     P.pos = P.dir = v3(0.0, 0.0, 0.0);
     P.tau = P.taurun = P.d = P.minabs = 0.0;
     P.layer = P.xcell = P.ycell = P.zcell = 0;
-    P.hop = P.loopc = P.seq = 0;
+    P.hop = P.loopc = 0;
+    P.seq = WS_SLOTS - 1u;
     P.rng.init(0);
     uint64_t chunk_base = 0;
     uint32_t chunk_left = 0;
@@ -287,7 +315,8 @@
             P.rng.cached = sh->ev_cached[pl];
           }
           if (P.st == ST_EMIT) {
-            P.pos = v3(sh->seg[P.seq][SG_OX][pl], sh->seg[P.seq][SG_OY][pl], sh->seg[P.seq][SG_OZ][pl]);
+            const uint32_t es = P.seq >> 2;
+            P.pos = v3(sh->seg[es][SG_OX][pl], sh->seg[es][SG_OY][pl], sh->seg[es][SG_OZ][pl]);
             P.dir = v3(sh->ev_dir[0][pl], sh->ev_dir[1][pl], sh->ev_dir[2][pl]);
             P.clr(LF_TFLAG);
             P.layer = (int32_t)(code & 0xFFFFu);
@@ -315,9 +344,10 @@
                 p8();
               }
             } else {
-              X[WX_SSP * xs] = sh->seg[P.seq][SG_DX][pl];
-              X[(WX_SSP + 1) * xs] = sh->seg[P.seq][SG_DY][pl];
-              X[(WX_SSP + 2) * xs] = sh->seg[P.seq][SG_DZ][pl];
+              const uint32_t es = P.seq >> 2;
+              X[WX_SSP * xs] = sh->seg[es][SG_DX][pl];
+              X[(WX_SSP + 1) * xs] = sh->seg[es][SG_DY][pl];
+              X[(WX_SSP + 2) * xs] = sh->seg[es][SG_DZ][pl];
               P.dir = v3(sh->ev_dir[0][pl], sh->ev_dir[1][pl], sh->ev_dir[2][pl]);
               P.layer = (int32_t)XI[WXI_NEWL * xs];
               P.st = ST_X1;
@@ -342,7 +372,7 @@
       WSDIAG(WD_PIDLE, __popcll(__ballot(P.st == ST_IDLE)));
       WSDIAG(WD_PWAIT, __popcll(__ballot(P.has(LF_WAIT))));
       WSDIAG(WD_PEVQ, __popcll(__ballot(P.has(LF_EVQ))));
-      WSDIAG(WD_PEMITW, __popcll(__ballot(!TK && P.st == ST_EMIT && !P.has(LF_EVQ) && (ws_busy(sh, pl) & (1u << P.seq)))));
+      WSDIAG(WD_PEMITW, __popcll(__ballot(!TK && P.st == ST_EMIT && !P.has(LF_EVQ) && ws_pick<WS_SLOTS>(ws_busy(sh, pl), P.seq & 3u) == WS_SLOTS)));
 
       WST(WD_TP_POLL);
       const bool have = (P.f & (LF_PEND | LF_REQ | LF_WAIT)) == LF_PEND;
@@ -351,7 +381,7 @@
       if (__ballot(have)) {
         const bool mask_le = test_kernel && P.st == ST_LAYER;
         const V3 q = (P.st == ST_H1 || P.st == ST_G0) ? P.pos + smul(P.d, P.dir) : P.pos;
-        R = eval_sdfs<false, SMCRT_WS_EVAL_PAIRS != 0>(nodes, prog, K.n_prog, q, mask_le, 0, 0);
+        R = eval_sdfs<false, WsTraits<GM, XF>::EVAL_PAIRS>(nodes, prog, K.n_prog, q, mask_le, 0, 0, !(K.lean_debug & 8u));
         const bool counted = P.st == ST_H0 || P.st == ST_H1 || P.st == ST_H3 || P.st == ST_M1 || P.st == ST_G0;
         w_sdf += __popcll(__ballot(have && counted)) * (uint32_t)K.n_top;
         WSDIAG(WD_ELANES, __popcll(__ballot(have)));
@@ -440,7 +470,7 @@
       if (__ballot(P.has(LF_REQ))) {
         bool push = false, sync = false;
         V3 old = v3(0.0, 0.0, 0.0);
-        const uint32_t slot = P.seq;
+        uint32_t slot = WS_SLOTS;
         bool inv = false;
         int32_t ci = -1, cj = -1, ck = -1;
         if constexpr (IV) {
@@ -470,7 +500,8 @@
           P.clr(LF_REQ | LF_MOVE_FWD | LF_MOVE_BACK);
           P.xcell = ci; P.ycell = cj; P.zcell = ck;
           P.set(LF_CELLS);
-        } else if (P.has(LF_REQ) && !(ws_busy(sh, pl) & (1u << slot))) {
+        } else if (P.has(LF_REQ) &&
+                   (slot = ws_pick<WS_SLOTS>(ws_busy(sh, pl), P.seq & 3u)) < WS_SLOTS) {
           ++r_upd;
           if constexpr (!IV) {
             old = v3(P.pos.x + K.xmax, P.pos.y + K.ymax, P.pos.z + K.zmax);
@@ -487,7 +518,7 @@
           } else {
             const double len = P.d;
             const V3 e = v3(old.x + P.dir.x * len, old.y + P.dir.y * len, old.z + P.dir.z * len);
-            constexpr bool KB = XF || SMCRT_WS_KBOUNDS_PLAIN;
+            constexpr bool KB = WsTraits<GM, XF>::KBOUNDS;
             const double mx = KB ? K.lean_lo[0] : mx0, my = KB ? K.lean_lo[1] : my0, mz = KB ? K.lean_lo[2] : mz0;
             const double ex = KB ? K.lean_hi[0] : ex0, ey = KB ? K.lean_hi[1] : ey0, ez = KB ? K.lean_hi[2] : ez0;
             const bool inside = old.x >= mx && old.x <= ex && old.y >= my && old.y <= ey && old.z >= mz &&
@@ -508,6 +539,7 @@
         }
         const uint64_t pm = __ballot(push);
         WSDIAG(WD_PUSH, __popcll(pm));
+        WSDIAG(WD_POOO, __popcll(__ballot(push && slot != ws_next<WS_SLOTS>(P.seq & 3u))));
         WSDIAG(WD_PBLOCKED, __popcll(__ballot(P.has(LF_REQ))));
         if (pm) {
           const int first = __builtin_ctzll(pm);
@@ -533,7 +565,8 @@
             }
             __hip_atomic_store(&sh->meta[ix], pl | (slot << 9) | (sync ? (1u << 11) : 0u) | ws_tick(t),
                                __ATOMIC_RELEASE, __HIP_MEMORY_SCOPE_WORKGROUP);
-            P.seq = P.seq + 1 == WS_SLOTS ? 0u : P.seq + 1;
+            if (slot != ws_next<WS_SLOTS>(P.seq & 3u)) ++r_ooo;
+            P.seq = slot;
             P.clr(LF_CELLS);
             if (sync) P.set(LF_WAIT);
           }
@@ -541,8 +574,8 @@
       }
 
       WST(WD_TP_HAND);
-      if (P.has(LF_WAIT) && !(ws_busy(sh, pl) & (1u << ((P.seq + WS_SLOTS - 1) % WS_SLOTS)))) {
-        const unsigned long long w = sh->pcell[pl][(P.seq + WS_SLOTS - 1) % WS_SLOTS];
+      if (P.has(LF_WAIT) && !(ws_busy(sh, pl) & (1u << (P.seq & 3u)))) {
+        const unsigned long long w = sh->pcell[pl][P.seq & 3u];
         P.xcell = lean_cell(w, 0); P.ycell = lean_cell(w, 1); P.zcell = lean_cell(w, 2);
         P.set(LF_CELLS);
         if (w & LEAN_TFLAG) P.set(LF_TFLAG);
@@ -584,7 +617,7 @@
         P.st = ST_INTERACT;
       }
       if (!P.has(LF_CELLS) && (P.st == ST_ABSORB || (records_on && P.st == ST_DONE)) && ws_busy(sh, pl) == 0) {
-        const unsigned long long w = sh->pcell[pl][(P.seq + WS_SLOTS - 1) % WS_SLOTS];
+        const unsigned long long w = sh->pcell[pl][P.seq & 3u];
         P.xcell = lean_cell(w, 0); P.ycell = lean_cell(w, 1); P.zcell = lean_cell(w, 2);
         P.set(LF_CELLS);
       }
@@ -597,11 +630,14 @@
 
       WST(WD_TP_P56);
       {
+        uint32_t es = 0;
+        const bool need_slot = (!test_kernel && P.st == ST_EMIT) || (XF && P.st == ST_F0);
+        if (need_slot && free_ && !P.has(LF_EVQ)) es = ws_pick<WS_SLOTS>(ws_busy(sh, pl), P.seq & 3u);
         bool qev = free_ && !P.has(LF_EVQ) &&
                    ((!test_kernel && ((P.st == ST_INTERACT && !(P.f & (LF_TFLAG | LF_FAULT)) &&
                                      WLU(LL_INTER) + 1u <= (uint32_t)MAX_INTERACTIONS) ||
-                                    P.st == ST_T2 || (P.st == ST_EMIT && !(ws_busy(sh, pl) & (1u << P.seq))))) ||
-                    (XF && P.st == ST_F0 && !(ws_busy(sh, pl) & (1u << P.seq))));
+                                    P.st == ST_T2 || (P.st == ST_EMIT && es < WS_SLOTS))) ||
+                    (XF && P.st == ST_F0 && es < WS_SLOTS));
         if (drop_event && qev) {
           drop_event = qev = false;
           __hip_atomic_store(&sh->ev_code[pl], 0u, __ATOMIC_RELAXED, __HIP_MEMORY_SCOPE_WORKGROUP);
@@ -629,8 +665,8 @@
               sh->ev_draws[pl] = P.rng.draws;
             }
             if (XF && P.st == ST_F0) {
-              sh->seg[P.seq][SG_OX][pl] = P.pos.x; sh->seg[P.seq][SG_OY][pl] = P.pos.y;
-              sh->seg[P.seq][SG_OZ][pl] = P.pos.z; sh->seg[P.seq][SG_LEN][pl] = P.d;
+              sh->seg[es][SG_OX][pl] = P.pos.x; sh->seg[es][SG_OY][pl] = P.pos.y;
+              sh->seg[es][SG_OZ][pl] = P.pos.z; sh->seg[es][SG_LEN][pl] = P.d;
               sh->ev_tau[pl] = (double)XI[WXI_NEWL * xs];
             }
             if (P.st == ST_EMIT) {
@@ -641,7 +677,8 @@
             sh->ev_code[pl] = (uint32_t)P.layer |
                               ((P.st == ST_INTERACT ? WS_EV_INTERACT
                                 : (P.st == ST_T2 ? WS_EV_TAU : (P.st == ST_EMIT ? WS_EV_EMIT : WS_EV_FRESNEL))) << 16) |
-                              (P.seq << 19);
+                              (es << 19);
+            P.seq = (P.seq & 3u) | (es << 2);
             __hip_atomic_store(&sh->evq[ix], pl | ws_tick(t), __ATOMIC_RELEASE, __HIP_MEMORY_SCOPE_WORKGROUP);
             P.set(LF_EVQ);
           }
@@ -1037,7 +1074,7 @@
     unsigned long long* const counters = C->counters;
     const uint32_t hz = wave_sum_u32(hazards);
     const uint32_t n_upd = wave_sum_u32(r_upd), n_scat = wave_sum_u32(r_scat), n_tau = wave_sum_u32(r_tau),
-                   n_abs = wave_sum_u32(r_abs), n_inv = wave_sum_u32(r_inv);
+                   n_abs = wave_sum_u32(r_abs), n_inv = wave_sum_u32(r_inv), n_ooo = wave_sum_u32(r_ooo);
     if (lane_id == 0) {
       if (hz) {
         atomicAdd(C->dep_ctl + 5, hz);
@@ -1045,6 +1082,7 @@
       }
       if (C->dep_ctl && n_upd) atomicAdd(C->dep_ctl + 6, n_upd);
       if (n_inv) atomicAdd(C->invoxel_segs, (unsigned long long)n_inv);
+      if (n_ooo) atomicAdd(C->ooo_handouts, (unsigned long long)n_ooo);
       if (counters) {
         const uint32_t* c = sh->wctr[wv];
         const uint32_t v[SMCRT_NCOUNTERS] = {c[LC_PHOTONS], c[LC_RETRIES], n_scat,        n_abs,          w_sdf,
diff --git a/rsmcrt_amd/engine.py b/rsmcrt_amd/engine.py
--- a/rsmcrt_amd/engine.py
+++ b/rsmcrt_amd/engine.py
@@ -428,6 +428,14 @@
         return n.value
 
 
+    def out_of_order_handouts(self) -> int:
+        fn = load_library().smcrt_scene_out_of_order_handouts
+        fn.argtypes = [C.c_void_p, C.POINTER(C.c_int64)]
+        n = C.c_int64()
+        _check(fn(self._h, C.byref(n)))
+        return n.value
+
+
 def pack_layout(grid, n_det_bins: int, fields: int) -> abi.PackLayout:
     lay = abi.PackLayout()
     lay.n_voxels, lay.n_det_bins, lay.fields = grid.nx * grid.ny * grid.nz, int(n_det_bins), int(fields)
```

After: 303.5 million, median of 6. +6.0%, better.
